# fakerlove1/HPFG

Hardware: AMD Instinct MI355X
Metric: labeled+unlabeled images/sec/node, U-Net 224x224 ACDC-shaped (Mean-Teacher step) (higher is better)
Workload: dtype bf16x3 (fp32 storage; products as split-bf16 MFMA hi*hi+hi*lo+lo*hi, fp32 accumulate); 1 GPU; mean_teacher_unet_224x224 (BASELINE configs[1]): U-Net 1ch->4cls, 8 labelled + 8 unlabelled per GPU, student fwd+bwd + train-mode teacher fwd + CE/Dice/MSE + SGD + EMA; size=224, hipgraph=True, sync_bn=False, parallelism=dp1, math=bf16x3

## Files before the change

hpfg_amd/_lib.py:

```python
from __future__ import annotations

import ctypes as C
import os
import threading

_HERE = os.path.dirname(os.path.abspath(__file__))
LIB_PATH = os.path.join(_HERE, "lib", "libhpfg_hip.so")

BN_MEAN, BN_RSTD, BN_SCALE, BN_SHIFT, BN_K1, BN_K2, BN_K3, BN_SPARE, BN_ROWS = range(9)
ACT_NONE, ACT_PLAIN, ACT_STRIDED, ACT_BNACT, ACT_BNACT_POOL, ACT_UP2X, ACT_DZ, ACT_SPLIT16, ACT_UPBWD = range(9)
OPT_CONV_THIN, OPT_FIRST_MFMA, OPT_FIRST_WGRAD, OPT_NARROW_DEEP = 0, 1, 2, 3
LOSS_NSUM = 32
LOSS_MAX_CLASSES = 16
ACC_MAX_SHARDS = 8
VERSION = 139
RESIZE_TAPS = 36
SURFACE_SEGS = 32
MATH_F32, MATH_BF16X3 = 0, 1


class HipLibraryError(RuntimeError):
    pass


class Act(C.Structure):
    _fields_ = [("z", C.c_void_p), ("bn", C.c_void_p), ("aux", C.c_void_p), ("mode", C.c_int32), ("C", C.c_int32),
                ("Hs", C.c_int32), ("Ws", C.c_int32), ("pstride", C.c_int32), ("aux_pstride", C.c_int32),
                ("bn_stride", C.c_int32), ("bn_coff", C.c_int32), ("sn", C.c_int32), ("sc", C.c_int32), ("sy", C.c_int32),
                ("sx", C.c_int32), ("drop_p", C.c_float), ("drop_seed", C.c_uint32), ("drop_mask", C.c_void_p), ("seed_dev", C.c_void_p),
                ("bn_acc", C.c_void_p), ("bn_gamma", C.c_void_p), ("bn_beta", C.c_void_p), ("bn_count", C.c_float), ("bn_eps", C.c_float),
                ("bn_shards", C.c_int32), ("reserved1", C.c_int32)]


class ConvArgs(C.Structure):
    _fields_ = [("a0", Act), ("a1", Act), ("wpk", C.c_void_p), ("bias", C.c_void_p), ("out", C.c_void_p),
                ("stat_partials", C.c_void_p), ("out_pstride", C.c_int32), ("Cout", C.c_int32), ("CoutPad", C.c_int32),
                ("N", C.c_int32), ("H", C.c_int32), ("W", C.c_int32), ("taps", C.c_int32), ("math", C.c_int32),
                ("bwd_stats", C.c_int32), ("bwd_of", Act), ("out2", C.c_void_p), ("out_split", C.c_int32), ("out2_pstride", C.c_int32),
                ("stat_acc", C.c_void_p), ("stat_shards", C.c_int32), ("reserved2", C.c_int32), ("stage_out", C.c_void_p), ("side_sums", C.c_void_p)]


class WgradArgs(C.Structure):
    _fields_ = [("a0", Act), ("a1", Act), ("g", Act), ("slab", C.c_void_p), ("dw_oihw", C.c_void_p), ("Cin", C.c_int32),
                ("CinPad", C.c_int32), ("Cout", C.c_int32), ("CoutPad", C.c_int32), ("N", C.c_int32), ("H", C.c_int32),
                ("W", C.c_int32), ("taps", C.c_int32), ("S", C.c_int32), ("math", C.c_int32), ("defer_reduce", C.c_int32)]


class PeerX(C.Structure):
    _fields_ = [("mbox", C.c_void_p * 8), ("epoch", C.c_void_p), ("err", C.c_void_p), ("world", C.c_int32), ("rank", C.c_int32),
                ("slot", C.c_int32), ("cap", C.c_int32), ("slot_bytes", C.c_int64)]


class PeerBuf(C.Structure):
    _fields_ = [("win", C.c_void_p * 8), ("epoch", C.c_void_p), ("err", C.c_void_p), ("world", C.c_int32), ("rank", C.c_int32),
                ("slice", C.c_int64), ("n", C.c_int64), ("stride", C.c_int64)]


class FusedBwdArgs(C.Structure):
    _fields_ = [("d", ConvArgs), ("xa0", Act), ("xa1", Act), ("slab", C.c_void_p), ("Cin", C.c_int32), ("CinPad", C.c_int32),
                ("Cout", C.c_int32), ("CoutPad", C.c_int32)]


class AugSample(C.Structure):
    _fields_ = [("img_off", C.c_int64), ("lab_off", C.c_int64), ("h", C.c_int32), ("w", C.c_int32), ("mode", C.c_int32), ("k", C.c_int32),
                ("axis", C.c_int32), ("tab_off", C.c_int32), ("m00", C.c_double), ("m01", C.c_double), ("m10", C.c_double),
                ("m11", C.c_double), ("off_y", C.c_double), ("off_x", C.c_double)]


class BnAccDesc(C.Structure):
    _fields_ = [("acc", C.c_void_p), ("gamma", C.c_void_p), ("beta", C.c_void_p), ("running_mean", C.c_void_p), ("running_var", C.c_void_p),
                ("bn", C.c_void_p), ("C", C.c_int32), ("count", C.c_float), ("shards", C.c_int32), ("reserved", C.c_int32)]


class BnAccBwdDesc(C.Structure):
    _fields_ = [("acc", C.c_void_p), ("gamma", C.c_void_p), ("bn", C.c_void_p), ("dgamma", C.c_void_p), ("dbeta", C.c_void_p),
                ("C", C.c_int32), ("count", C.c_float), ("shards", C.c_int32), ("reserved", C.c_int32)]


class SlabDesc(C.Structure):
    _fields_ = [("slab", C.c_void_p), ("dw_oihw", C.c_void_p), ("S", C.c_int32), ("taps", C.c_int32), ("Cin", C.c_int32),
                ("CinPad", C.c_int32), ("Cout", C.c_int32), ("CoutPad", C.c_int32)]


class PackDesc(C.Structure):
    _fields_ = [("w_oihw", C.c_void_p), ("b", C.c_void_p), ("wpk_fwd", C.c_void_p), ("wpk_dgrad", C.c_void_p),
                ("bias_pad", C.c_void_p), ("wpk16_fwd", C.c_void_p), ("wpk16_dgrad", C.c_void_p), ("Cout", C.c_int32), ("Cin", C.c_int32),
                ("CoutPad", C.c_int32), ("CinPad", C.c_int32), ("taps", C.c_int32), ("kc", C.c_int32)]


class LossArgs(C.Structure):
    _fields_ = [("logits", C.c_void_p), ("t_logits", C.c_void_p), ("labels0", C.c_void_p), ("labels1", C.c_void_p),
                ("coef", C.c_void_p), ("partials", C.c_void_p), ("sums", C.c_void_p), ("out", C.c_void_p),
                ("dlogits", C.c_void_p), ("N", C.c_int32), ("n_lab", C.c_int32), ("H", C.c_int32), ("W", C.c_int32),
                ("C", C.c_int32), ("world", C.c_int32), ("input_is_prob", C.c_int32), ("teacher_is_prob", C.c_int32),
                ("t_unlab_only", C.c_int32), ("reserved0", C.c_int32), ("cons_mask", C.c_void_p)]


class PredBlocks(C.Structure):
    _fields_ = [("p", C.c_void_p * 8), ("n_blocks", C.c_int32), ("per_block", C.c_int32)]


_i, _l, _f, _d, _p, _u32 = C.c_int, C.c_long, C.c_float, C.c_double, C.c_void_p, C.c_uint32

PROTOTYPES = {
    "hpfg_version": (_i, []),
    "hpfg_last_error": (C.c_char_p, []),
    "hpfg_set_option": (_i, [_i, _i]),
    "hpfg_conv3x3_first_fwd": (_i, [C.POINTER(Act), _p, _p, _p, _p, _i, _i, _i, _i, _i, _p]),
    "hpfg_conv_fwd": (_i, [C.POINTER(ConvArgs), _p]),
    "hpfg_conv_stat_blocks": (_i, [_i, _i, _i]),
    "hpfg_conv_stat_rows": (_i, [C.POINTER(ConvArgs)]),
    "hpfg_bn_fwd_finalize": (_i, [_p, _i, _p, _d, _p, _p, _p, _p, _f, _f, _p, _i, _p]),
    "hpfg_reduce_partials": (_i, [_p, _i, _i, _p, _p]),
    "hpfg_conv_kc": (_i, [_i, _i, _i]),
    "hpfg_wpk16_elems": (_l, [_i, _i, _i, _i]),
    "hpfg_pack_weights": (_i, [_p, C.POINTER(PackDesc), _i, _p]),
    "hpfg_pack_weights_bump": (_i, [_p, C.POINTER(PackDesc), _i, _p, _i, _p, _i, _p, _l, _p]),
    "hpfg_conv3x3_first_fwd_acc": (_i, [C.POINTER(Act), _p, _p, _p, _p, _p, _i, _i, _i, _i, _i, _i, _p]),
    "hpfg_bn_acc_finalize": (_i, [_p, C.POINTER(BnAccDesc), _i, _f, _f, _p]),
    "hpfg_bn_acc_bwd_finalize": (_i, [_p, C.POINTER(BnAccBwdDesc), _i, _p]),
    "hpfg_bn_bwd_reduce_acc": (_i, [C.POINTER(Act), _i, _i, _i, _p, _i, _p]),
    "hpfg_bn_bwd_reduce_pool_acc": (_i, [C.POINTER(Act), _p, _i, _i, _i, _i, _p, _i, _p]),
    "hpfg_act_materialize": (_i, [C.POINTER(Act), C.POINTER(Act), _i, _i, _i, _p, _p]),
    "hpfg_dropout_mask": (_i, [_p, _l, _f, _u32, _p, _p]),
    "hpfg_bn_eval_table": (_i, [_p, _p, _p, _p, _f, _p, _i, _p]),
    "hpfg_bn_bwd_reduce": (_i, [C.POINTER(Act), _i, _i, _i, _p, _p]),
    "hpfg_bn_bwd_reduce_pool": (_i, [C.POINTER(Act), _p, _i, _i, _i, _i, _p, _p]),
    "hpfg_bn_bwd_pool_blocks": (_i, [_i, _i, _i, _i]),
    "hpfg_bn_bwd_blocks": (_i, [_i, _i, _i, _i]),
    "hpfg_bn_bwd_finalize": (_i, [_p, _i, _p, _d, _p, _p, _p, _p, _i, _f, _p]),
    "hpfg_wgrad": (_i, [C.POINTER(WgradArgs), _p]),
    "hpfg_fused_bwd": (_i, [C.POINTER(FusedBwdArgs), _p]),
    "hpfg_fused_bwd_grid": (_i, [C.POINTER(FusedBwdArgs)]),
    "hpfg_peer_slot_bytes": (_l, [_i, _i]),
    "hpfg_peer_alloc": (_i, [C.c_size_t, C.POINTER(C.c_void_p)]),
    "hpfg_peer_free": (_i, [_p]),
    "hpfg_peer_handle": (_i, [_p, C.c_char_p]),
    "hpfg_peer_open": (_i, [C.c_char_p, C.POINTER(C.c_void_p)]),
    "hpfg_peer_close": (_i, [_p]),
    "hpfg_word_add": (_i, [_p, _i, _p]),
    "hpfg_peer_buf_slice": (_l, [_i, _l]),
    "hpfg_peer_buf_bytes": (_l, [_i, _l]),
    "hpfg_peer_allreduce_f32": (_i, [C.POINTER(PeerBuf), _p, _p]),
    "hpfg_bn_fwd_finalize_x": (_i, [_p, _i, C.POINTER(PeerX), _d, _p, _p, _p, _p, _f, _f, _p, _i, _p]),
    "hpfg_bn_bwd_finalize_x": (_i, [_p, _i, C.POINTER(PeerX), _d, _p, _p, _p, _p, _i, _f, _p]),
    "hpfg_seg_loss_partials_x": (_i, [C.POINTER(LossArgs), C.POINTER(PeerX), _p]),
    "hpfg_slab_reduce_multi": (_i, [_p, C.POINTER(SlabDesc), _i, _p]),
    "hpfg_wgrad_splits": (_i, [_i, _i, _i, _i, _i, _i]),
    "hpfg_wgrad_slab_floats": (_l, [_i, _i, _i, _i, _i, _i]),
    "hpfg_channel_sum": (_i, [_p, _i, _l, _i, _p, _p, _p]),
    "hpfg_channel_sum_partials": (_i, [_p, _i, _l, _i, _p, _p]),
    "hpfg_channel_sum_blocks": (_i, [_l, _i]),
    "hpfg_conv_first_rows": (_i, [_i, _i, _i]),
    "hpfg_confusion_counts": (_i, [_p, _p, _l, _i, _p, _p]),
    "hpfg_resize_cubic": (_i, [_p, _i, _i, _i, _p, _i, _i, _p, _p, _p, _l, _p]),
    "hpfg_resize_cubic_scratch_bytes": (_l, [_i, _i, _i, _i, _i]),
    "hpfg_surface_counts": (_i, [_p, _p, _i, _i, _i, _i, _i, _p, _p]),
    "hpfg_surface_distances": (_i, [_p, _p, _i, _i, _i, _i, _i, _p, _p, _l, _p]),
    "hpfg_surface_workspace_bytes": (_l, [_i, _l]),
    "hpfg_surface_sums": (_i, [_p, _l, _i, _p, _p, _p]),
    "hpfg_box_masks": (_i, [_p, _i, _i, _i, _i, _i, _p, _p]),
    "hpfg_augment_batch": (_i, [_p, _p, _p, _p, _i, _i, _i, _p, _p, _p]),
    "hpfg_timestamp": (_i, [_p, _p]),
    "hpfg_ln_fwd": (_i, [_p, _p, _p, _p, _p, _p, _l, _i, _p]),
    "hpfg_ln_bwd": (_i, [_p, _p, _p, _p, _p, _p, _p, _p, _p, _l, _i, _p]),
    "hpfg_ln_bwd_blocks": (_i, [_l]),
    "hpfg_attn_fwd": (_i, [_p, _p, _p, _i, _i, _i, _i, _f, _p]),
    "hpfg_attn_bwd": (_i, [_p, _p, _p, _p, _p, _p, _i, _i, _i, _i, _f, _p]),
    "hpfg_dwgelu_fwd": (_i, [_p, _p, _p, _p, _i, _i, _i, _i, _p]),
    "hpfg_dwgelu_bwd": (_i, [_p, _p, _p, _p, _p, _p, _p, _p, _p, _i, _i, _i, _i, _p]),
    "hpfg_dwgelu_bwd_blocks": (_i, [_i, _i, _i]),
    "hpfg_resize_bilinear_fwd": (_i, [_p, _p, _i, _i, _i, _i, _i, _i, _p]),
    "hpfg_resize_sum_fwd": (_i, [_p, C.POINTER(C.c_void_p), C.POINTER(C.c_int), C.POINTER(C.c_int), _i, _p, _i, _i, _i, _i, _p]),
    "hpfg_resize_bilinear_bwd": (_i, [_p, _p, _i, _i, _i, _i, _i, _i, _p]),
    "hpfg_residual_scale": (_i, [_p, _p, _p, _p, _i, _l, _p]),
    "hpfg_scale_rows": (_i, [_p, _p, _p, _i, _l, _p]),
    "hpfg_im2col_nhwc": (_i, [_p, _p, _i, _i, _i, _i, _i, _i, _p]),
    "hpfg_col2im_nhwc": (_i, [_p, _p, _i, _i, _i, _i, _i, _i, _p]),
    "hpfg_linear_wgrad": (_i, [_p, _p, _p, _p, _l, _i, _i, _p]),
    "hpfg_linear_wgrad_splits": (_i, [_l, _i, _i]),
    "hpfg_tok_col_stats": (_i, [_p, _l, _i, _p, _p, _p]),
    "hpfg_tok_stat_blocks": (_i, [_l]),
    "hpfg_bnrelu_apply": (_i, [_p, _p, _p, _p, _p, _p, _f, _l, _p, _l, _i, _p]),
    "hpfg_bnrelu_bwd": (_i, [_p, _p, _p, _p, _p, _p, _p, _f, _l, _p, _p, _p, _l, _i, _p]),
    "hpfg_noise_add": (_i, [_p, _p, _p, _l, _l, _f, _f, _f, _p]),
    "hpfg_uncertainty_mask": (_i, [C.POINTER(PredBlocks), _i, _i, _i, _i, _i, _p, _p, _p, _p]),
    "hpfg_mix_samples": (_i, [_p, _p, _p, _p, _i, _l, _p]),
    "hpfg_softmax_mix": (_i, [_p, _p, _p, _p, _i, _i, _i, _i, _p]),
    "hpfg_pool_scatter_add": (_i, [C.POINTER(Act), _p, _i, _p, _i, _i, _i, _i, _p]),
    "hpfg_upsample2x_bwd": (_i, [_p, _i, _p, _i, _i, _i, _i, _p]),
    "hpfg_upsample2x_bwd_sums": (_i, [_p, _i, _p, _i, _i, _i, _i, _p, _p]),
    "hpfg_upsample2x_bwd_blocks": (_i, [_i, _i, _i, _i]),
    "hpfg_loss_blocks": (_i, [_i, _i, _i]),
    "hpfg_loss_nsum": (_i, [_i]),
    "hpfg_seg_loss_partials": (_i, [C.POINTER(LossArgs), _p]),
    "hpfg_seg_loss_finalize": (_i, [C.POINTER(LossArgs), _p]),
    "hpfg_seg_loss_bwd": (_i, [C.POINTER(LossArgs), _p, _p]),
    "hpfg_argmax_labels": (_i, [_p, _i, _i, _i, _i, _p, _p, _p, _p]),
    "hpfg_cutmix_blend": (_i, [_p, _p, _p, _p, _l, _p]),
    "hpfg_sgd_step": (_i, [_p, _p, _p, _l, _p, _f, _f, _f, _p]),
    "hpfg_adamw_step": (_i, [_p, _p, _p, _p, _l, _p, _p, _f, _f, _f, _f, _f, _p]),
    "hpfg_ema_update": (_i, [_p, _p, _l, _p, _p]),
    "hpfg_sgd_ema_step": (_i, [_p, _p, _p, _l, _p, _f, _f, _f, _p, _l, _p, _p]),
    "hpfg_attn_mfma_fwd": (_i, [_p, _p, _p, _i, _i, _i, _i, _f, _p]),
    "hpfg_attn_mfma_bwd": (_i, [_p, _p, _p, _p, _p, _p, _i, _i, _i, _i, _f, _p]),
    "hpfg_attn_mfma_blocks": (_i, [_i]),
    "hpfg_attn_mfma_fwd_hd": (_i, [_p, _p, _p, _i, _i, _i, _i, _i, _f, _p]),
    "hpfg_attn_mfma_bwd_hd": (_i, [_p, _p, _p, _p, _p, _p, _i, _i, _i, _i, _i, _f, _p]),
    "hpfg_attn_mfma_scratch_floats": (_l, [_i, _i, _i, _i]),
    "hpfg_attn_keys_max": (_i, []),
    "hpfg_attn_keys_fwd": (_i, [_p, _p, _p, _p, _i, _i, _i, _i, _i, _f, _i, _p]),
    "hpfg_attn_keys_bwd": (_i, [_p, _p, _p, _p, _p, _p, _p, _p, _i, _i, _i, _i, _i, _f, _i, _p]),
    "hpfg_attn_keys_scratch_floats": (_l, [_i, _i, _i, _i, _i, _i]),
    "hpfg_attn_window_fwd": (_i, [_p, _p, _p, _i, _i, _i, _i, _i, _i, _i, _f, _i, _p]),
    "hpfg_attn_window_bwd": (_i, [_p, _p, _p, _p, _p, _p, _i, _i, _i, _i, _i, _i, _i, _f, _i, _p]),
    "hpfg_attn_window_scratch_floats": (_l, [_i, _i, _i, _i, _i, _i, _i]),
    "hpfg_gelu_fwd": (_i, [_p, _p, _l, _p]),
    "hpfg_gelu_bwd": (_i, [_p, _p, _p, _l, _p]),
    "hpfg_patch_merge_fwd": (_i, [_p, _p, _i, _i, _i, _i, _p]),
    "hpfg_patch_merge_bwd": (_i, [_p, _p, _i, _i, _i, _i, _p]),
    "hpfg_attn_fwd_hd": (_i, [_p, _p, _p, _i, _i, _i, _i, _i, _f, _p]),
    "hpfg_attn_bwd_hd": (_i, [_p, _p, _p, _p, _p, _p, _i, _i, _i, _i, _i, _f, _p]),
    "hpfg_gemm_f32": (_i, [_p, _l, _l, _p, _l, _l, _p, _l, _i, _i, _i, _p, _i, _i, _p]),
    "hpfg_gemm_f32_splitk": (_i, [_p, _l, _l, _p, _l, _l, _p, _l, _i, _i, _i, _p, _i, _i, _p, _p]),
    "hpfg_gemm_f32_splits": (_i, [_i, _i, _i]),
    "hpfg_gemm_bf16x3": (_i, [_p, _l, _l, _p, _l, _l, _p, _l, _i, _i, _i, _p, _i, _i, _p]),
    "hpfg_gemm_bf16x3_splits": (_i, [_i, _i, _i]),
    "hpfg_gemm_bf16x3_splitk": (_i, [_p, _l, _l, _p, _l, _l, _p, _l, _i, _i, _i, _p, _i, _i, _p, _p]),
    "hpfg_gemm_bf16x3_ok": (_i, [_p, _l, _l, _p, _l, _l, _i, _i, _i]),
    "hpfg_gemm_tn_bf16x3": (_i, [_p, _p, _p, _p, _l, _i, _i, _i, _p]),
    "hpfg_gemm_tn_splits": (_i, [_l, _i, _i]),
    "hpfg_col_sum2": (_i, [_p, _l, _i, _l, _p, _p, _p]),
    "hpfg_col_sum_splits": (_i, [_l]),
    "hpfg_col_sum": (_i, [_p, _l, _i, _l, _p, _p]),
    "hpfg_relu_bwd": (_i, [_p, _p, _l, _p]),
    "hpfg_neck_pool_fwd": (_i, [_p, _i, _i, _i, _i, _i, _i, _p, _p, _p]),
    "hpfg_neck_pool_bwd": (_i, [_p, _p, _i, _i, _i, _i, _i, _p, _p]),
    "hpfg_l2norm_fwd": (_i, [_p, _i, _i, _i, _i, _i, _p, _p, _p]),
    "hpfg_l2norm_bwd": (_i, [_p, _p, _p, _i, _i, _i, _i, _i, _p, _p, _p]),
    "hpfg_ntxent_rows": (_i, [_p, _i, _f, _p, _p, _p]),
}

_lock = threading.Lock()
_lib = None


def load() -> C.CDLL:
    global _lib
    if _lib is not None:
        return _lib
    with _lock:
        if _lib is not None:
            return _lib
        if not os.path.exists(LIB_PATH):
            raise HipLibraryError(
                f"{LIB_PATH} not found: build it with `python -c 'import __graft_entry__ as g; g.build()'` "
                f"or `make -C hpfg_amd/csrc`. There is no CPU fallback for the HIP path.")
        lib = C.CDLL(LIB_PATH)
        for name, (res, args) in PROTOTYPES.items():
            fn = getattr(lib, name)
            fn.restype = res
            fn.argtypes = args
        if lib.hpfg_version() != VERSION:
            raise HipLibraryError(f"libhpfg_hip.so version {lib.hpfg_version()} != binding version {VERSION}; rebuild")
        if os.environ.get("HPFG_FIRST_WGRAD", "1") == "0":
            lib.hpfg_set_option(OPT_FIRST_WGRAD, 0)
        if os.environ.get("HPFG_NARROW_DEEP") is not None:
            lib.hpfg_set_option(OPT_NARROW_DEEP, int(os.environ["HPFG_NARROW_DEEP"]))
        _lib = lib
    return _lib


def check(rc: int, what: str):
    if rc != 0:
        msg = load().hpfg_last_error().decode("utf-8", "replace")
        raise HipLibraryError(f"{what} failed (rc={rc}): {msg}")


def ptr(t):
    return None if t is None else t.data_ptr()


def none_act() -> Act:
    return Act()
```

hpfg_amd/csrc/conv.hip:

```cpp
#include "conv_kernel.h"
#include "conv_bf16_kernel.h"

namespace {

struct HpfgFirstConvArgs {
  HpfgAct x;
  const float* w_oihw;
  const float* bias;
  float* out;
  float* stat_partials;
  long long* stat_acc;
  int stat_shards;
};

inline bool tile_is_big(int H, int W) { return (H % 16 == 0) && (W % 16 == 0); }

__global__ __launch_bounds__(256) HPFG_NO_PK_F32 void conv_first_kernel(HpfgFirstConvArgs q, int N, int H, int W, int Cin, int tiles_x, int tiles_y) {
  constexpr int T = 16, TP = T + 2, CO = 16;
  const HpfgAct& x = q.x;
  const float* __restrict__ w = q.w_oihw;
  const float* __restrict__ bias = q.bias;
  float* __restrict__ out = q.out;
  float* __restrict__ stat = q.stat_partials;
  long long* __restrict__ sacc = q.stat_acc;
  __shared__ float tin[4][TP * TP];
  __shared__ __attribute__((aligned(16))) float wl[9 * 4 * CO];
  __shared__ float red[2][4][CO];
  const int tid = threadIdx.x, lane = tid & 63, wave = tid >> 6;
  const int ntiles = tiles_x * tiles_y, nwork = ntiles * N;
  for (int i = tid; i < 9 * Cin * CO; i += 256) {
    int co = i % CO, r = i / CO, ci = r % Cin, tap = r / Cin;
    wl[i] = w[(co * Cin + ci) * 9 + tap];
  }
  f32x4 bq[4], s1[4], s2[4];
#pragma unroll
  for (int q = 0; q < 4; ++q) {
    bq[q] = *reinterpret_cast<const f32x4*>(bias + 4 * q);
    s1[q] = f32x4{0.f, 0.f, 0.f, 0.f};
    s2[q] = s1[q];
  }
  const int ly = tid / T, lx = tid % T;
  for (int wk = blockIdx.x; wk < nwork; wk += gridDim.x) {
    const int n = wk / ntiles, tile = wk % ntiles;
    const int ty0 = (tile / tiles_x) * T, tx0 = (tile % tiles_x) * T;
    __syncthreads();
    for (int i = tid; i < Cin * TP * TP; i += 256) {
      int ci = i / (TP * TP), pix = i % (TP * TP);
      int gy = ty0 + pix / TP - 1, gx = tx0 + pix % TP - 1;
      float v = 0.f;
      if (gy >= 0 && gy < H && gx >= 0 && gx < W) v = x.z[(long)n * x.sn + (long)ci * x.sc + (long)gy * x.sy + (long)gx * x.sx];
      tin[ci][pix] = v;
    }
    __syncthreads();
    f32x4 acc[4] = {bq[0], bq[1], bq[2], bq[3]};
    for (int ci = 0; ci < Cin; ++ci)
#pragma unroll
      for (int tap = 0; tap < 9; ++tap) {
        const float a = tin[ci][(ly + tap / 3) * TP + lx + tap % 3];
        const f32x4* wr = reinterpret_cast<const f32x4*>(wl + (tap * Cin + ci) * CO);
#pragma unroll
        for (int q = 0; q < 4; ++q) acc[q] += a * wr[q];
      }
    const int gy = ty0 + ly, gx = tx0 + lx;
    if (gy < H && gx < W) {
      f32x4* o = reinterpret_cast<f32x4*>(out + ((long)(n * H + gy) * W + gx) * CO);
#pragma unroll
      for (int q = 0; q < 4; ++q) {
        o[q] = acc[q];
        s1[q] += acc[q];
        s2[q] += acc[q] * acc[q];
      }
    }
  }
  if (stat || sacc) {
#pragma unroll
    for (int q = 0; q < 4; ++q)
#pragma unroll
      for (int j = 0; j < 4; ++j) {
        float v = s1[q][j], v2 = s2[q][j];
#pragma unroll
        for (int o = 32; o >= 1; o >>= 1) {
          v += __shfl_xor(v, o);
          v2 += __shfl_xor(v2, o);
        }
        if (lane == 0) {
          red[0][wave][4 * q + j] = v;
          red[1][wave][4 * q + j] = v2;
        }
      }
    __syncthreads();
    if (tid < 2 * CO) {
      int which = tid / CO, co = tid % CO;
      float t = red[which][0][co] + red[which][1][co] + red[which][2][co] + red[which][3][co];
      if (sacc) hpfg_acc_add(sacc, CO, (int)blockIdx.x & (q.stat_shards - 1), which, co, t);
      if (stat) stat[((long)blockIdx.x * 2 + which) * CO + co] = t;
    }
  }
}

template <int CIN>
__global__ __launch_bounds__(256) void conv_first_mfma_kernel(HpfgFirstConvArgs q, int N, int H, int W, int tiles_x, int tiles_y) {
  constexpr int T = 16, TP = T + 2, CO = 16, NPIX = TP * TP, KT = 9 * CIN, KS = (KT + 3) / 4, NLD = (CIN * NPIX + 255) / 256;
  const HpfgAct& x = q.x;
  const float* __restrict__ w = q.w_oihw;
  float* __restrict__ out = q.out;
  float* __restrict__ stat = q.stat_partials;
  long long* __restrict__ sacc = q.stat_acc;
  __shared__ float tin[CIN * NPIX];
  __shared__ float red[2][4][CO];
  const int tid = threadIdx.x, lane = tid & 63, wave = tid >> 6;
  const int ntiles = tiles_x * tiles_y, nwork = ntiles * N;
  const int co_a = lane & 15, kq = lane >> 4;
  float wa[KS];
  int boff[KS];
#pragma unroll
  for (int s_ = 0; s_ < KS; ++s_) {
    const int k = 4 * s_ + kq, ci = k / 9, tap = k - 9 * ci;
    wa[s_] = k < KT ? w[co_a * KT + k] : 0.f;
    boff[s_] = k < KT ? ci * NPIX + (tap / 3) * TP + (lane & 15) + tap % 3 : 0;
  }
  const f32x4 b4 = *reinterpret_cast<const f32x4*>(q.bias + 4 * kq);
  f32x4 s1[4], s2[4];
#pragma unroll
  for (int r = 0; r < 4; ++r) {
    s1[r] = f32x4{0.f, 0.f, 0.f, 0.f};
    s2[r] = s1[r];
  }
  int pci[NLD], ppy[NLD], ppx[NLD];
#pragma unroll
  for (int i = 0; i < NLD; ++i) {
    const int e = tid + 256 * i, pix = e % NPIX;
    pci[i] = e / NPIX;
    ppy[i] = pix / TP - 1;
    ppx[i] = pix % TP - 1;
  }
  int n = 0, ty0 = 0, tx0 = 0;
  auto coords = [&](int wk) {
    n = wk / ntiles;
    const int tile = wk - n * ntiles, tyi = tile / tiles_x;
    ty0 = tyi * T;
    tx0 = (tile - tyi * tiles_x) * T;
  };
  auto fetch = [&](float (&v)[NLD]) {
    const float* xb = x.z + (long)n * x.sn;
#pragma unroll
    for (int i = 0; i < NLD; ++i) {
      const int gy = ty0 + ppy[i], gx = tx0 + ppx[i];
      v[i] = (tid + 256 * i < CIN * NPIX && gy >= 0 && gy < H && gx >= 0 && gx < W) ? xb[(long)pci[i] * x.sc + (long)gy * x.sy + (long)gx * x.sx] : 0.f;
    }
  };
  float v[NLD];
  int wk = blockIdx.x;
  if (wk < nwork) {
    coords(wk);
    fetch(v);
  }
#pragma unroll 1
  for (; wk < nwork; wk += gridDim.x) {
    const int cn = n, cy0 = ty0, cx0 = tx0;
    __syncthreads();
#pragma unroll
    for (int i = 0; i < NLD; ++i)
      if (tid + 256 * i < CIN * NPIX) tin[tid + 256 * i] = v[i];
    __syncthreads();
    if (wk + (int)gridDim.x < nwork) {
      coords(wk + gridDim.x);
      fetch(v);
    }
    const int gx = cx0 + (lane & 15);
    float* orow = out + ((long)(cn * H + cy0 + 4 * wave) * W + gx) * CO + 4 * kq;
#pragma unroll
    for (int r = 0; r < 4; ++r) {
      const int ly = 4 * wave + r;
      f32x4 acc = b4;
#pragma unroll
      for (int s_ = 0; s_ < KS; ++s_) {
        float bv = tin[ly * TP + boff[s_]];
        if (s_ == KS - 1 && 4 * s_ + kq >= KT) bv = 0.f;
        acc = __builtin_amdgcn_mfma_f32_16x16x4f32(wa[s_], bv, acc, 0, 0, 0);
      }
      if (cy0 + ly < H && gx < W) *reinterpret_cast<f32x4*>(orow + (long)r * W * CO) = acc;
      s1[r] += acc;
      s2[r] += acc * acc;
    }
  }
  if (stat || sacc) {
    const f32x4 t1 = (s1[0] + s1[2]) + (s1[1] + s1[3]), t2 = (s2[0] + s2[2]) + (s2[1] + s2[3]);
#pragma unroll
    for (int j = 0; j < 4; ++j) {
      float a1 = t1[j], a2 = t2[j];
#pragma unroll
      for (int o = 8; o >= 1; o >>= 1) {
        a1 += __shfl_xor(a1, o);
        a2 += __shfl_xor(a2, o);
      }
      if ((lane & 15) == 0) {
        red[0][wave][4 * kq + j] = a1;
        red[1][wave][4 * kq + j] = a2;
      }
    }
    __syncthreads();
    if (tid < 2 * CO) {
      const int which = tid / CO, co = tid % CO;
      const float t = red[which][0][co] + red[which][1][co] + red[which][2][co] + red[which][3][co];
      if (sacc) hpfg_acc_add(sacc, CO, (int)blockIdx.x & (q.stat_shards - 1), which, co, t);
      if (stat) stat[((long)blockIdx.x * 2 + which) * CO + co] = t;
    }
  }
}

inline int conv_first_grid(int N, int H, int W) {
  const long nwork = (long)N * ((H + 15) / 16) * ((W + 15) / 16);
  return (int)(nwork < 1024 ? nwork : 1024);
}

}

extern "C" int hpfg_conv_stat_blocks(int N, int H, int W) {
  if (tile_is_big(H, W)) return (N * (H / 16) * (W / 16) + 7) / 8 * 8;
  const int a = N * ((H + 7) / 8) * ((W + 7) / 8), b = N * ((H + 3) / 4) * ((W + 15) / 16);
  return a > b ? a : b;
}

extern "C" int hpfg_conv_first_rows(int N, int H, int W) { return conv_first_grid(N, H, W); }

static int conv_fwd_impl(const HpfgConvArgs* a, void* stream, int* rows_only);

extern "C" int hpfg_conv_fwd(const HpfgConvArgs* a, void* stream) { return conv_fwd_impl(a, stream, nullptr); }

extern "C" int hpfg_conv_stat_rows(const HpfgConvArgs* a) {
  int rows = -1;
  int rc = conv_fwd_impl(a, nullptr, &rows);
  return rc ? -1 : rows;
}

static int conv_fwd_impl(const HpfgConvArgs* a, void* stream, int* rows_only) {
  HPFG_ARG_CHECK(a && a->wpk && a->out, "conv_fwd: null pointer");
  HPFG_ARG_CHECK(a->taps == 9 || a->taps == 1, "conv_fwd: taps must be 1 or 9 (got %d)", a->taps);
  HPFG_ARG_CHECK(a->CoutPad % 16 == 0 && a->Cout <= a->CoutPad && a->Cout > 0, "conv_fwd: bad Cout %d / pad %d", a->Cout, a->CoutPad);
  HPFG_ARG_CHECK(a->N > 0 && a->H > 0 && a->W > 0 && a->N < 65536, "conv_fwd: bad N/H/W");
  HPFG_ARG_CHECK(a->a0.mode != HPFG_ACT_NONE && a->a0.C > 0, "conv_fwd: a0 empty");
  HPFG_ARG_CHECK(a->a1.mode == HPFG_ACT_NONE || a->a0.C % 16 == 0, "conv_fwd: concat needs a0.C %% 16 == 0");
  HPFG_ARG_CHECK(a->out_split ? (a->out_pstride >= a->out_split) : (a->out_pstride >= a->Cout), "conv_fwd: out_pstride too small");
  HPFG_ARG_CHECK(a->out_split == 0 || (a->out2 && a->out_split % 16 == 0 && a->out_split < a->Cout && a->out2_pstride >= a->Cout - a->out_split &&
                                       !a->bwd_stats),
                 "conv_fwd: out_split needs out2, a multiple of 16 below Cout, and no bwd_stats");
  HPFG_ARG_CHECK(!a->stat_acc || ((a->math & 0xff) == HPFG_MATH_BF16X3 && a->Cout == a->CoutPad && a->stat_shards >= 1 &&
                                  a->stat_shards <= HPFG_ACC_MAX_SHARDS && (a->stat_shards & (a->stat_shards - 1)) == 0),
                 "conv_fwd: stat_acc is a bf16x3 forward feature (Cout == CoutPad, stat_shards a power of two <= %d)", HPFG_ACC_MAX_SHARDS);
  for (const HpfgAct* s : {&a->a0, &a->a1}) {
    if (!s->bn_acc) continue;
    HPFG_ARG_CHECK((a->math & 0xff) == HPFG_MATH_BF16X3 && (s->mode == HPFG_ACT_BNACT || s->mode == HPFG_ACT_BNACT_POOL || s->mode == HPFG_ACT_DZ) &&
                       s->bn_gamma && (s->bn_beta || s->mode == HPFG_ACT_DZ) && s->bn_count >= 1.f && s->bn_count <= 16777216.f && s->C <= 256 && s->bn_shards >= 1 &&
                       s->bn_shards <= HPFG_ACC_MAX_SHARDS,
                   "conv_fwd: bn_acc needs a BNACT / BNACT_POOL / DZ source of the bf16x3 kernels with gamma (beta), a count of at most 2^24 (a float holds N*H*W exactly up to there) and at most 256 channels");
  }
  HPFG_ARG_CHECK((a->math & 0xff) != HPFG_MATH_BF16X3 || !(a->a0.mode == HPFG_ACT_BNACT || a->a0.mode == HPFG_ACT_BNACT_POOL || a->a0.mode == HPFG_ACT_DZ) ||
                     a->a0.C <= 256,
                 "conv_fwd(bf16x3): a BatchNorm'd source has at most 256 channels (got %d)", a->a0.C);
  const bool upb = a->a0.mode == HPFG_ACT_UPBWD;
  HPFG_ARG_CHECK(!upb || ((a->math & 0xff) == HPFG_MATH_BF16X3 && a->taps == 1 && a->a1.mode == HPFG_ACT_NONE && a->a0.C % 8 == 0 && a->a0.pstride % 4 == 0 &&
                          a->a0.Hs == a->H && a->a0.Ws == a->W && a->H <= 16383 && a->W <= 16383 && (long)a->N * 4 * a->H * a->W * a->a0.pstride < (1L << 31)),
                 "conv_fwd: an UPBWD source belongs to the 1x1 bf16x3 dgrad (channels a multiple of 8, pixel stride of 4, Hs x Ws == H x W)");
  HPFG_ARG_CHECK(!a->side_sums || upb, "conv_fwd: side_sums goes with an UPBWD source");
  HPFG_ARG_CHECK(!a->stage_out || upb || ((a->math & 0xff) == HPFG_MATH_BF16X3 && a->taps == 9 && hpfg_kind_of(a->a0, a->a1) > HPFG_KIND_PLAIN &&
                                    (a->a0.C + a->a1.C) % 8 == 0 && (a->H % 16 || a->W % 16)),
                 "conv_fwd: stage_out is a feature of the 3x3 bf16x3 kernels (non-PLAIN source, channels a multiple of 8, H or W not a multiple of 16)");
  hipStream_t st = (hipStream_t)stream;
  if (a->bwd_stats) {
    const int kind = hpfg_kind_of(a->a0, a->a1);
    HPFG_ARG_CHECK((a->math & 0xff) == HPFG_MATH_BF16X3 && (kind == HPFG_KIND_DZ || kind == HPFG_KIND_PLAIN || (kind == HPFG_KIND_UPB && a->bwd_stats == 1)),
                   "conv_fwd: bwd_stats is a dgrad feature of the bf16x3 kernels (DZ, PLAIN or UPBWD source)");
    HPFG_ARG_CHECK((a->stat_partials || a->stat_acc) && a->bwd_of.z && a->bwd_of.bn && !a->bias,
                   "conv_fwd: bwd_stats needs stat_partials or stat_acc, bwd_of.z / .bn and no bias");
    const int up = a->bwd_stats == 2 ? 2 : 1;
    HPFG_ARG_CHECK(a->bwd_stats == 1 || a->bwd_stats == 2, "conv_fwd: bwd_stats must be 0, 1 or 2");
    HPFG_ARG_CHECK(a->bwd_of.C == a->Cout && a->Cout == a->CoutPad && a->bwd_of.Hs == up * a->H && a->bwd_of.Ws == up * a->W && a->bwd_of.pstride % 4 == 0,
                   "conv_fwd: bwd_of must describe a layer with C == Cout == CoutPad (%d/%d/%d) at the output size (twice it for bwd_stats == 2)",
                   a->bwd_of.C, a->Cout, a->CoutPad);
    HPFG_ARG_CHECK(a->bwd_stats == 1 || (a->taps == 9 && (a->H % 16 || a->W % 16) && a->bwd_of.aux && a->bwd_of.aux_pstride % 4 == 0 && a->bwd_of.drop_p == 0.f && !a->out_split),
                   "conv_fwd: bwd_stats == 2 (max-pool backward in the epilogue) needs a 3x3 dgrad at a size that is not a multiple of 16, bwd_of.aux (the gradient so far) and no dropout behind bwd_of");
  }
  if ((a->math & 0xff) == HPFG_MATH_BF16X3) {
    {
      const int r = hpfg_conv_thin_try(*a, st, rows_only);
      if (r != HPFG_THIN_NONE) return r;
    }
    switch (hpfg_kind_of(a->a0, a->a1)) {
      case HPFG_KIND_PLAIN: return hpfg_conv16_launch_plain(*a, st, rows_only);
      case HPFG_KIND_BNACT: return hpfg_conv16_launch_bnact(*a, st, rows_only);
      case HPFG_KIND_POOL: return hpfg_conv16_launch_pool(*a, st, rows_only);
      case HPFG_KIND_CAT: return hpfg_conv16_launch_cat(*a, st, rows_only);
      case HPFG_KIND_DZ: return hpfg_conv16_launch_dz(*a, st, rows_only);
      case HPFG_KIND_UPB: return hpfg_conv16_launch_upb(*a, st, rows_only);
      default: break;
    }
    hpfg_set_error("conv_fwd(bf16x3): unsupported source combination (a0.mode=%d, a1.mode=%d)", a->a0.mode, a->a1.mode);
    return -1;
  }
  if (rows_only) {
    const int tl = tile_is_big(a->H, a->W) ? 16 : 8;
    *rows_only = a->N * ((a->H + tl - 1) / tl) * ((a->W + tl - 1) / tl);
    return 0;
  }
  switch (hpfg_kind_of(a->a0, a->a1)) {
    case HPFG_KIND_PLAIN: return hpfg_conv_launch_plain(*a, st);
    case HPFG_KIND_BNACT: return hpfg_conv_launch_bnact(*a, st);
    case HPFG_KIND_POOL: return hpfg_conv_launch_pool(*a, st);
    case HPFG_KIND_CAT: return hpfg_conv_launch_cat(*a, st);
    case HPFG_KIND_DZ: return hpfg_conv_launch_dz(*a, st);
    default: break;
  }
  hpfg_set_error("conv_fwd: unsupported source combination (a0.mode=%d, a1.mode=%d)", a->a0.mode, a->a1.mode);
  return -1;
}

static int conv_first_impl(const HpfgFirstConvArgs* q, int N, int H, int W, int Cin, int Cout, void* stream) {
  HPFG_ARG_CHECK(Cin >= 1 && Cin <= 4 && Cout == 16, "conv_first: needs Cin<=4, Cout==16 (got %d,%d)", Cin, Cout);
  HPFG_ARG_CHECK(q->x.z && q->w_oihw && q->bias && q->out, "conv_first: null pointer");
  HPFG_ARG_CHECK(q->x.mode == HPFG_ACT_STRIDED, "conv_first: input must be a STRIDED source");
  HPFG_ARG_CHECK((q->stat_partials == nullptr && q->stat_acc == nullptr) || tile_is_big(H, W), "conv_first: BN sums need H,W multiples of 16 (got %dx%d)", H, W);
  int tx = (W + 15) / 16, ty = (H + 15) / 16;
  const dim3 g1(conv_first_grid(N, H, W));
  if (q->stat_acc) HPFG_ACC_CHECK(g1.x, q->stat_shards, "conv_first");
  if ((Cin == 1 || Cin == 3) && hpfg_opt(HPFG_OPT_FIRST_MFMA) != 0) {
    if (Cin == 1) hipLaunchKernelGGL((conv_first_mfma_kernel<1>), g1, dim3(256), 0, (hipStream_t)stream, *q, N, H, W, tx, ty);
    else hipLaunchKernelGGL((conv_first_mfma_kernel<3>), g1, dim3(256), 0, (hipStream_t)stream, *q, N, H, W, tx, ty);
    return hpfg_launch_status("conv_first_mfma_kernel");
  }
  hipLaunchKernelGGL(conv_first_kernel, g1, dim3(256), 0, (hipStream_t)stream, *q, N, H, W, Cin, tx, ty);
  return hpfg_launch_status("conv_first_kernel");
}

extern "C" int hpfg_conv3x3_first_fwd(const HpfgAct* x, const float* w_oihw, const float* bias, float* out, float* stat_partials,
                                      int N, int H, int W, int Cin, int Cout, void* stream) {
  HPFG_ARG_CHECK(x, "conv_first: null pointer");
  HpfgFirstConvArgs a = {*x, w_oihw, bias, out, stat_partials, nullptr, 1};
  return conv_first_impl(&a, N, H, W, Cin, Cout, stream);
}

extern "C" int hpfg_conv3x3_first_fwd_acc(const HpfgAct* x, const float* w_oihw, const float* bias, float* out, float* stat_partials, long long* stat_acc,
                                          int stat_shards, int N, int H, int W, int Cin, int Cout, void* stream) {
  HPFG_ARG_CHECK(x && stat_acc, "conv_first_acc: null pointer");
  HPFG_ARG_CHECK(stat_shards >= 1 && stat_shards <= HPFG_ACC_MAX_SHARDS && (stat_shards & (stat_shards - 1)) == 0, "conv_first_acc: bad shard count %d", stat_shards);
  HpfgFirstConvArgs a = {*x, w_oihw, bias, out, stat_partials, stat_acc, stat_shards};
  return conv_first_impl(&a, N, H, W, Cin, Cout, stream);
}
```

hpfg_amd/csrc/misc.hip:

```cpp
#include <stdarg.h>
#include <string.h>
#include "stage.h"

static thread_local char g_err[512] = "";
extern "C" void hpfg_set_error(const char* fmt, ...) {
  va_list ap;
  va_start(ap, fmt);
  vsnprintf(g_err, sizeof(g_err), fmt, ap);
  va_end(ap);
}
extern "C" const char* hpfg_last_error(void) { return g_err; }
extern "C" int hpfg_version(void) { return HPFG_VERSION; }

static int g_opt[HPFG_OPT_COUNT] = {1, 1, 1, 128};
int hpfg_opt(int which) { return which >= 0 && which < HPFG_OPT_COUNT ? g_opt[which] : 0; }
extern "C" int hpfg_set_option(int which, int value) {
  HPFG_ARG_CHECK(which >= 0 && which < HPFG_OPT_COUNT, "set_option: unknown option %d", which);
  const int old = g_opt[which];
  g_opt[which] = value;
  return old;
}

namespace {

__global__ __launch_bounds__(256) void pack_weights_kernel(const HpfgPackDesc* __restrict__ table, long long* __restrict__ counters, int n_counters,
                                                           int* __restrict__ seed_word, int seed_add, long long* __restrict__ zero, long n_zero) {
  if (blockIdx.x == 0 && blockIdx.y == 0) {
    for (int i = threadIdx.x; i < n_counters; i += 256) counters[i] += 1;
    if (threadIdx.x == 0 && seed_word && seed_add) *seed_word = (*seed_word + seed_add) & 0x7FFFFFFF;
  }
  for (long i = ((long)blockIdx.y * gridDim.x + blockIdx.x) * 256 + threadIdx.x; i < n_zero; i += (long)gridDim.x * gridDim.y * 256) zero[i] = 0;
  const HpfgPackDesc d = table[blockIdx.y];
  const long total = (long)d.taps * d.CinPad * d.CoutPad;
  const int nt_f = d.CoutPad / 16, nch_f = d.CinPad / 16;
  const int nt_d = d.CinPad / 16, nch_d = d.CoutPad / 16;
  for (long i = blockIdx.x * 256L + threadIdx.x; i < total; i += (long)gridDim.x * 256) {
    int ks = (int)(i & 3), lane = (int)((i >> 2) & 63);
    long r = i >> 8;
    if (d.wpk_fwd) {
      int nt = (int)(r % nt_f), ch = (int)((r / nt_f) % nch_f), tap = (int)(r / ((long)nt_f * nch_f));
      int co = nt * 16 + (lane & 15), ci = ch * 16 + ks * 4 + (lane >> 4);
      d.wpk_fwd[i] = (co < d.Cout && ci < d.Cin) ? d.w_oihw[((long)co * d.Cin + ci) * d.taps + tap] : 0.f;
    }
    if (d.wpk_dgrad) {
      int nt = (int)(r % nt_d), ch = (int)((r / nt_d) % nch_d), tap = (int)(r / ((long)nt_d * nch_d));
      int co = ch * 16 + ks * 4 + (lane >> 4), ci = nt * 16 + (lane & 15);
      d.wpk_dgrad[i] = (co < d.Cout && ci < d.Cin) ? d.w_oihw[((long)co * d.Cin + ci) * d.taps + (d.taps - 1 - tap)] : 0.f;
    }
    if (i < d.CoutPad) d.bias_pad[i] = (i < d.Cout && d.b) ? d.b[i] : 0.f;
  }
  const int ksteps = d.taps == 1 ? 1 : (d.kc == 32 ? 9 : 5);
  for (int dir = 0; dir < 2; ++dir) {
    __bf16* out = reinterpret_cast<__bf16*>(dir == 0 ? d.wpk16_fwd : d.wpk16_dgrad);
    if (!out) continue;
    const int Kch = dir == 0 ? d.Cin : d.Cout;
    const int ntn = (dir == 0 ? d.CoutPad : d.CinPad) / 16;
    const int nchunks = (Kch + d.kc - 1) / d.kc;
    const long tot = (long)nchunks * ksteps * ntn * 512;
    for (long i = blockIdx.x * 256L + threadIdx.x; i < tot; i += (long)gridDim.x * 256) {
      const int j = (int)(i & 7), lane = (int)((i >> 3) & 63);
      const long r = i >> 9;
      const int nt = (int)(r % ntn), ks = (int)(r / ntn);
      const int chunk = ks / ksteps, s = ks % ksteps;
      const int kl = 8 * (lane >> 4) + j;
      int tap, kch;
      if (d.taps == 1) { tap = 0; kch = chunk * 32 + kl; }
      else if (d.kc == 32) { tap = s; kch = chunk * 32 + kl; }
      else { tap = 2 * s + (kl >> 4); kch = chunk * 16 + (kl & 15); }
      const int nch = nt * 16 + (lane & 15);
      float w = 0.f;
      if (tap < d.taps && kch < Kch) {
        if (dir == 0) { if (nch < d.Cout) w = d.w_oihw[((long)nch * d.Cin + kch) * d.taps + tap]; }
        else { if (nch < d.Cin) w = d.w_oihw[((long)kch * d.Cin + nch) * d.taps + (d.taps - 1 - tap)]; }
      }
      const __bf16 hi = (__bf16)w;
      const __bf16 lo = (__bf16)(w - (float)hi);
      const long base = ((long)ks * ntn + nt) * 2;
      out[(base + 0) * 512 + lane * 8 + j] = hi;
      out[(base + 1) * 512 + lane * 8 + j] = lo;
    }
  }
}

__global__ __launch_bounds__(256) void materialize_kernel(HpfgAct a0, HpfgAct a1, int N, int H, int W, float* __restrict__ out) {
  const int Ct = a0.C + a1.C, Q = (Ct + 3) / 4;
  const ActCtx c0 = make_ctx(a0), c1 = make_ctx(a1);
  const long total = (long)N * H * W * Q;
  for (long i = blockIdx.x * 256L + threadIdx.x; i < total; i += (long)gridDim.x * 256) {
    int q = (int)(i % Q);
    long pix = i / Q;
    int x = (int)(pix % W), y = (int)((pix / W) % H), n = (int)(pix / ((long)W * H));
    f32x4 v = cat_load4(a0, c0, a1, c1, n, y, x, q * 4);
#pragma unroll
    for (int j = 0; j < 4; ++j)
      if (q * 4 + j < Ct) out[pix * Ct + q * 4 + j] = v[j];
  }
}

__global__ __launch_bounds__(256) void dropout_mask_kernel(uint8_t* __restrict__ out, long n, uint32_t thresh, uint32_t seed0,
                                                           const uint32_t* __restrict__ seed_dev) {
  const uint32_t seed = seed0 + (seed_dev ? *seed_dev : 0u);
  for (long i = blockIdx.x * 256L + threadIdx.x; i < n; i += (long)gridDim.x * 256) out[i] = hpfg_keep((uint32_t)i, seed, thresh) ? 1 : 0;
}

__global__ __launch_bounds__(256) void pool_scatter_kernel(HpfgAct s, const float* __restrict__ dP, int dp_ps, float* __restrict__ dA, int da_ps,
                                                           int N, int Hp, int Wp) {
  const int Q = s.C / 4;
  const long total = (long)N * Hp * Wp * Q;
  for (long i = blockIdx.x * 256L + threadIdx.x; i < total; i += (long)gridDim.x * 256) {
    int q = (int)(i % Q);
    long pp = i / Q;
    int xp = (int)(pp % Wp), yp = (int)((pp / Wp) % Hp), n = (int)(pp / ((long)Wp * Hp));
    int c = q * 4;
    f32x4 sc = *reinterpret_cast<const f32x4*>(s.bn + HPFG_BN_SCALE * s.bn_stride + s.bn_coff + c);
    f32x4 sh = *reinterpret_cast<const f32x4*>(s.bn + HPFG_BN_SHIFT * s.bn_stride + s.bn_coff + c);
    long p00 = (long)(n * s.Hs + 2 * yp) * s.Ws + 2 * xp;
    long pos[4] = {p00, p00 + 1, p00 + s.Ws, p00 + s.Ws + 1};
    f32x4 zz[4];
#pragma unroll
    for (int k = 0; k < 4; ++k) zz[k] = *reinterpret_cast<const f32x4*>(s.z + pos[k] * s.pstride + c);
    f32x4 g = *reinterpret_cast<const f32x4*>(dP + pp * dp_ps + c);
    f32x4 da[4];
#pragma unroll
    for (int k = 0; k < 4; ++k) da[k] = *reinterpret_cast<const f32x4*>(dA + pos[k] * da_ps + c);
#pragma unroll
    for (int j = 0; j < 4; ++j) {
      float best = lrelu(zz[0][j] * sc[j] + sh[j]);
      int bi = 0;
#pragma unroll
      for (int k = 1; k < 4; ++k) {
        float v = lrelu(zz[k][j] * sc[j] + sh[j]);
        if (v > best) {
          best = v;
          bi = k;
        }
      }
#pragma unroll
      for (int k = 0; k < 4; ++k) da[k][j] += bi == k ? g[j] : 0.f;
    }
#pragma unroll
    for (int k = 0; k < 4; ++k) *reinterpret_cast<f32x4*>(dA + pos[k] * da_ps + c) = da[k];
  }
}

constexpr int UPB_MAXDIM = 512, UPB_TAPS = HPFG_UPB_TAPS;
__global__ __launch_bounds__(256) __attribute__((amdgpu_waves_per_eu(2, 3))) void upsample_bwd_kernel(const float* __restrict__ dUp, int dup_ps, float* __restrict__ dU, int N, int Hl, int Wl,
                                                           int C, float* __restrict__ csum, int xcd_aware) {
  __shared__ short t_idx[UPB_MAXDIM][UPB_TAPS];
  __shared__ float t_w[UPB_MAXDIM][UPB_TAPS];
  __shared__ float red[256 * 4];
  for (int e = threadIdx.x; e < Hl + Wl; e += 256) {
    int idx[8], cnt;
    float wgt[8];
    if (e < Hl) hpfg_up_taps(e, Hl, idx, wgt, cnt);
    else hpfg_up_taps(e - Hl, Wl, idx, wgt, cnt);
    if (cnt > UPB_TAPS) cnt = UPB_TAPS;
    for (int k = 0; k < UPB_TAPS; ++k) {
      t_idx[e][k] = (short)(k < cnt ? idx[k] : idx[cnt - 1]);
      t_w[e][k] = k < cnt ? wgt[k] : 0.f;
    }
  }
  __syncthreads();
  const int Q = C / 4, Ho = 2 * Hl, Wo = 2 * Wl;
  const long total = (long)N * Hl * Wl * Q;
  f32x4 csum4 = {0.f, 0.f, 0.f, 0.f};
  const int nxcd = (xcd_aware && gridDim.x % 8 == 0) ? 8 : 1;
  const long gx = gridDim.x / nxcd, xj = blockIdx.x / nxcd;
  const long span = ((total + nxcd - 1) / nxcd + 255) / 256 * 256;
// ... 464 lines not shown
```

hpfg_amd/engine.py:

```python
from __future__ import annotations

import ctypes as C
import itertools
import os
from dataclasses import dataclass
from typing import Dict, List, Optional

import torch

from . import _lib as L

SEED_BUMP = -1

WIDTHS = (16, 32, 64, 128, 256)
ENC_DROPOUT = (0.05, 0.1, 0.2, 0.3, 0.5)
BN_EPS, BN_MOMENTUM = 1e-5, 0.1


ACC, LOCAL, ALLREDUCE, PEER, EVAL = "acc", "local", "allreduce", "peer", "eval"


def bn_route(train: bool, math: int, bn_acc_on: bool, peer: bool, world: int, force_sync: bool) -> str:
    if not train:
        return EVAL
    sync = world > 1 or force_sync
    if bn_acc_on and math == L.MATH_BF16X3 and not peer and not sync:
        return ACC
    if sync:
        return PEER if peer else ALLREDUCE
    return LOCAL


def _pad16(c: int) -> int:
    return (c + 15) // 16 * 16


def _carve(flat: torch.Tensor, sizes: Dict[str, int]) -> Dict[str, torch.Tensor]:
    ends = list(itertools.accumulate(sizes.values()))
    return {name: flat[e - n:e] for (name, n), e in zip(sizes.items(), ends)}


class DescTable:

    def __init__(self, descs: C.Array, dev: torch.device):
        self.host = descs
        self.dev = torch.frombuffer(bytearray(bytes(descs)), dtype=torch.uint8).to(dev)
        self._base, self._size = self.dev.data_ptr(), C.sizeof(descs._type_)

    def sub(self, lo: int, hi: int):
        return self._base + lo * self._size, (self.host._type_ * (hi - lo)).from_buffer(self.host, lo * self._size), hi - lo


@dataclass
class ConvSpec:
    name: str
    bn: Optional[str]
    cin: int
    cout: int
    taps: int
    h: int
    w: int
    drop_p: float = 0.0
    idx: int = 0
    cin_pad: int = 0
    cout_pad: int = 0

    def __post_init__(self):
        self.cin_pad, self.cout_pad = _pad16(self.cin), _pad16(self.cout)


def enc_prefix(lvl: int) -> str:
    return "encoder.in_conv.conv_conv" if lvl == 0 else f"encoder.down{lvl}.maxpool_conv.1.conv_conv"


def build_specs(in_ch: int, ncls: int, H: int, W: int) -> Dict[str, ConvSpec]:
    specs: Dict[str, ConvSpec] = {}

    def add(s: ConvSpec):
        s.idx = len(specs)
        specs[s.name] = s

    cprev = in_ch
    for lvl, c in enumerate(WIDTHS):
        p, h, w = enc_prefix(lvl), H >> lvl, W >> lvl
        add(ConvSpec(f"{p}.0", f"{p}.1", cprev, c, 9, h, w, ENC_DROPOUT[lvl]))
        add(ConvSpec(f"{p}.4", f"{p}.5", c, c, 9, h, w))
        cprev = c
    for k in range(1, 5):
        c1, c2 = WIDTHS[5 - k], WIDTHS[4 - k]
        hl, wl = H >> (5 - k), W >> (5 - k)
        add(ConvSpec(f"decoder.up{k}.conv1x1", None, c1, c2, 1, hl, wl))
        p = f"decoder.up{k}.conv.conv_conv"
        add(ConvSpec(f"{p}.0", f"{p}.1", 2 * c2, c2, 9, 2 * hl, 2 * wl))
        add(ConvSpec(f"{p}.4", f"{p}.5", c2, c2, 9, 2 * hl, 2 * wl))
    add(ConvSpec("decoder.out_conv", None, WIDTHS[0], ncls, 9, H, W))
    return specs


class MarkLog:

    def __init__(self, dev: torch.device, capacity: int = 2048):
        self.buf = torch.zeros(capacity, dtype=torch.int64, device=dev)
        self.spans: List[tuple] = []
        self.n = 0
        self.lib = L.load()

    def stamp(self, stream: int) -> int:
        k = self.n
        if k >= self.buf.numel():
            raise RuntimeError("MarkLog: out of slots")
        self.n += 1
        L.check(self.lib.hpfg_timestamp(self.buf.data_ptr() + 8 * k, stream), "timestamp")
        return k

    def bracket(self, tag: str, stream: int, launch):
        a = self.stamp(stream)
        launch()
        self.spans.append((tag, a, self.stamp(stream)))

    def calib(self, stream: int):
        a = self.stamp(stream)
        self.spans.append(("calib", a, self.stamp(stream)))

    def read_us(self) -> List[tuple]:
        t = self.buf[: self.n].cpu().numpy()
        return [(tag, float(int(t[b]) - int(t[a])) / 100.0) for tag, a, b in self.spans]


class UNetEngine:

    def __init__(self, params: Dict[str, torch.Tensor], buffers: Dict[str, torch.Tensor], grads: Dict[str, torch.Tensor],
                 in_ch: int, ncls: int, N: int, H: int, W: int, device: torch.device):
        assert H % 16 == 0 and W % 16 == 0, "U-Net input must be a multiple of 16 (4 poolings)"
        self.lib = L.load()
        self.dev = device
        self.N, self.H, self.W, self.in_ch, self.ncls = N, H, W, in_ch, ncls
        self.params, self.buffers, self.grads = params, buffers, grads
        self.specs = build_specs(in_ch, ncls, H, W)
        self.order = list(self.specs.values())
        f32 = dict(dtype=torch.float32, device=device)
        self.z: Dict[str, torch.Tensor] = {s.name: torch.empty(N, s.h, s.w, s.cout, **f32) for s in self.order if s.name != "decoder.out_conv"}
        self.bn: Dict[str, torch.Tensor] = {s.name: torch.zeros(L.BN_ROWS, s.cout, **f32) for s in self.order if s.bn}
        nb = max(self.lib.hpfg_conv_stat_blocks(N, s.h, s.w) * 2 * s.cout_pad for s in self.order if s.bn)
        nb = max(nb, max(self.lib.hpfg_bn_bwd_blocks(N, s.h, s.w, s.cout) * 2 * s.cout for s in self.order if s.bn))
        nb = max(nb, max(self.lib.hpfg_bn_bwd_pool_blocks(N, s.h // 2, s.w // 2, s.cout) * 2 * s.cout for s in self.order if s.bn))
        self.partials = torch.empty(nb, **f32)
        self.sums = torch.empty(2 * 256, dtype=torch.float64, device=device)
        self.packed = [s for s in self.order if s.idx > 0]
        self.wpk_f = {s.name: torch.empty(s.taps * s.cin_pad * s.cout_pad, **f32) for s in self.packed}
        self.wpk_d = {s.name: torch.empty(s.taps * s.cin_pad * s.cout_pad, **f32) for s in self.packed}
        self.bias_pad = {s.name: torch.empty(s.cout_pad, **f32) for s in self.packed}
        self.kc = {s.name: self.lib.hpfg_conv_kc(s.h, s.w, s.taps) for s in self.packed}
        self.wpk16_f = {s.name: torch.empty(self.lib.hpfg_wpk16_elems(s.cin, s.cout_pad, s.taps, self.kc[s.name]), dtype=torch.bfloat16, device=device)
                        for s in self.packed}
        self.wpk16_d = {s.name: torch.empty(self.lib.hpfg_wpk16_elems(s.cout, s.cin_pad, s.taps, self.kc[s.name]), dtype=torch.bfloat16, device=device)
                        for s in self.packed}
        self._pack_tables: Dict[tuple, DescTable] = {}
        self.bn_layers = [s for s in self.order if s.bn]
        self._bn_idx = {s.name: i for i, s in enumerate(self.bn_layers)}
        self._n_enc_bn = sum(1 for s in self.bn_layers if s.name.startswith("encoder."))
        self.bn_acc_on = os.environ.get("HPFG_BN_ACC", "1") != "0"
        self.acc_shards = {s.name: L.ACC_MAX_SHARDS for s in self.bn_layers}
        assert all(s.cout == s.cout_pad for s in self.bn_layers)
        acc_words = {s.name: self.acc_shards[s.name] * 4 * s.cout for s in self.bn_layers}
        self.acc_all = torch.zeros(sum(acc_words.values()), dtype=torch.int64, device=device)
        self.acc_of = _carve(self.acc_all, acc_words)
        self.fwd_route, self._acc_dirty = EVAL, False
        self._acc_tables: Dict[bool, DescTable] = {}
        self.pack_overlap = False
        self.after_layer = None
        self.accb_all = torch.zeros_like(self.acc_all)
        self.accb_of = _carve(self.accb_all, acc_words)
        self.bwd_route, self._accb_dirty = LOCAL, False
        self._accb_table: Optional[DescTable] = None
        self.seed_dev = torch.zeros(1, dtype=torch.int32, device=device)
        self.bump_counters: Optional[torch.Tensor] = None
        self.base_seed = 0x1234567
        self.dropout_on = False
        self._stage_inputs = False
        self.bwd_ready = False
        self.x: Optional[torch.Tensor] = None
        self.world = 1
        self.gtmp, self.direct = None, False
        self._bwd_alloc_key: Optional[tuple] = None
        self.dA, self.dA_ps = {}, {}
        self.dcat, self.dup, self.dU, self.dP = {}, {}, {}, {}
        self.slab_of, self.csum_part, self.csum_rows = {}, {}, {}
        self.slabs: Optional[DescTable] = None
        self.bias_layers = [s for s in self.order if not s.bn]
        self._n_enc_desc = sum(1 for s in self.order if s.name.startswith("encoder."))
        self._n_thin_enc_desc = sum(1 for s in self.order if s.name.startswith("encoder.in_conv") or s.name.startswith("encoder.down1"))
        self.fuse_bwd_stats = 1
        self._fused_rows: Dict[str, int] = {}
        self.fused_bwd = os.environ.get("HPFG_FUSED_BWD", "1") == "1"
        self.pool_fuse = True
        self._pool_done: set = set()
        self.dz_side = True
        self.act_side = True
        self.upb_fuse = os.environ.get("HPFG_UPB_FUSE", "1") == "1"
        self.upb_max_c1 = int(os.environ.get("HPFG_UPB_MAX_C1", "128"))
        self.dzbuf: Dict[str, torch.Tensor] = {}
        self.actbuf: Dict[str, torch.Tensor] = {}
        self._act_live: set = set()
        self.defer_wgrad = False
        self._deferred: Optional[list] = None
        self._csum_pending: Optional[torch.Tensor] = None
        self.fused_grid: Dict[str, int] = {}
        self._side, self._side_used = None, False
        self.force_sync = False
        self.math = L.MATH_F32
        self.ext_masks: Dict[str, torch.Tensor] = {}
        self.allreduce = None
        self.peer, self.peer_base, self.xepoch = None, 0, None
        self.marks: Optional[MarkLog] = None

    def _stream(self):
        return torch.cuda.current_stream(self.dev).cuda_stream

    def _call(self, fn, *args, tag: Optional[str] = None, stream: Optional[int] = None):
        st = self._stream() if stream is None else stream

        def launch():
            L.check(fn(*args, st), f"{fn.__name__}[{tag}]" if tag else fn.__name__)
        if tag is None or self.marks is None:
            return launch()
        self.marks.bracket(tag, st, launch)

    @property
    def _b16(self) -> bool:
        return self.math == L.MATH_BF16X3

    def _fork_side(self) -> torch.cuda.Stream:
        if self._side is None:
            self._side = torch.cuda.Stream(device=self.dev)
        self._side.wait_stream(torch.cuda.current_stream(self.dev))
        return self._side

    def _join_side(self):
        if self._side_used:
            torch.cuda.current_stream(self.dev).wait_stream(self._side)
            self._side_used = False

    def layer_seed(self, s: ConvSpec) -> int:
        return (self.base_seed * 0x9E3779B1 + 0x85EBCA6B * (s.idx + 1)) & 0xFFFFFFFF

    def _act_bn(self, name: str, mode=L.ACT_BNACT) -> L.Act:
        s = self.specs[name]
        a = L.Act()
        a.z, a.bn, a.mode, a.C = L.ptr(self.z[name]), L.ptr(self.bn[name]), mode, s.cout
        a.Hs, a.Ws, a.pstride, a.bn_stride, a.bn_coff = s.h, s.w, s.cout, s.cout, 0
        if self.fwd_route == ACC and mode in (L.ACT_BNACT, L.ACT_BNACT_POOL):
            a.bn_acc, a.bn_gamma, a.bn_beta = L.ptr(self.acc_of[name]), L.ptr(self.params[f"{s.bn}.weight"]), L.ptr(self.params[f"{s.bn}.bias"])
            a.bn_count, a.bn_eps, a.bn_shards = float(self.N * s.h * s.w), BN_EPS, self.acc_shards[name]
        if mode == L.ACT_BNACT:
            self._act_dropout(a, s)
        return a

    def _act_dropout(self, a: L.Act, s: ConvSpec):
        if s.drop_p > 0 and self.dropout_on:
            a.drop_p, a.drop_seed, a.seed_dev = s.drop_p, self.layer_seed(s), L.ptr(self.seed_dev)
            a.drop_mask = L.ptr(self.ext_masks.get(s.name)) if self.ext_masks else None

    def _act_plain(self, t: torch.Tensor, C_: int, h: int, w: int, pstride: Optional[int] = None, mode=L.ACT_PLAIN) -> L.Act:
        a = L.Act()
        a.z, a.mode, a.C, a.Hs, a.Ws = L.ptr(t), mode, C_, h, w
        a.pstride = C_ if pstride is None else pstride
        if C_ % 4 != 0 and mode == L.ACT_PLAIN:
            a.mode = L.ACT_STRIDED
            a.sn, a.sc, a.sy, a.sx = h * w * a.pstride, 1, w * a.pstride, a.pstride
        return a

    def _act_split(self, t: torch.Tensor, C_: int, h: int, w: int) -> L.Act:
        return self._act_plain(t, C_, h, w, mode=L.ACT_SPLIT16)

    def _act_input(self, x: torch.Tensor) -> L.Act:
        a = L.Act()
        a.z, a.mode, a.C, a.Hs, a.Ws = L.ptr(x), L.ACT_STRIDED, self.in_ch, self.H, self.W
        a.sn, a.sc, a.sy, a.sx = x.stride(0), x.stride(1), x.stride(2), x.stride(3)
        return a

    def _act_dz(self, name: str, dA: torch.Tensor, da_pstride: int) -> L.Act:
        s = self.specs[name]
        a = L.Act()
        a.z, a.bn, a.aux, a.mode, a.C = L.ptr(self.z[name]), L.ptr(self.bn[name]), L.ptr(dA), L.ACT_DZ, s.cout
        a.Hs, a.Ws, a.pstride, a.aux_pstride, a.bn_stride = s.h, s.w, s.cout, da_pstride, s.cout
        if self.bwd_route == ACC:
            a.bn_acc, a.bn_gamma, a.bn_count, a.bn_shards = L.ptr(self.accb_of[name]), L.ptr(self.params[f"{s.bn}.weight"]), float(self.N * s.h * s.w), self.acc_shards[name]
        self._act_dropout(a, s)
        return a

    def input_acts(self, name: str):
        s = self.specs[name]
        none = L.Act()
        if name == "encoder.in_conv.conv_conv.0":
            return self._act_input(self.x), none
        if name == "decoder.out_conv":
            return self._act_bn("decoder.up4.conv.conv_conv.4"), none
        if name.endswith(".4"):
            return self._act_bn(name[:-2] + ".0"), none
        if name.startswith("encoder.down"):
            lvl = int(name[len("encoder.down")])
            return self._act_bn(enc_prefix(lvl - 1) + ".4", L.ACT_BNACT_POOL), none
        k = int(name[len("decoder.up")])
        prev = enc_prefix(4) + ".4" if k == 1 else f"decoder.up{k - 1}.conv.conv_conv.4"
        if name.endswith("conv1x1"):
            return self._act_bn(prev), none
        skip = self._act_bn(enc_prefix(4 - k) + ".4")
        u = self.specs[f"decoder.up{k}.conv1x1"]
        up = self._act_plain(self.z[u.name], u.cout, u.h, u.w, mode=L.ACT_UP2X)
        return skip, up

    def _pack_table(self, math: int, with_dgrad: bool):
        key = (math, with_dgrad)
        if key not in self._pack_tables:
            b16 = math == L.MATH_BF16X3
            descs = (L.PackDesc * len(self.packed))()
            for d, s in zip(descs, self.packed):
                d.w_oihw, d.b = L.ptr(self.params[f"{s.name}.weight"]), L.ptr(self.params[f"{s.name}.bias"])
                d.bias_pad = L.ptr(self.bias_pad[s.name])
                d.wpk_fwd = None if b16 else L.ptr(self.wpk_f[s.name])
                d.wpk_dgrad = None if (b16 or not with_dgrad) else L.ptr(self.wpk_d[s.name])
                d.wpk16_fwd = L.ptr(self.wpk16_f[s.name]) if b16 else None
                d.wpk16_dgrad = L.ptr(self.wpk16_d[s.name]) if (b16 and with_dgrad) else None
                d.kc = self.kc[s.name]
                d.Cout, d.Cin, d.CoutPad, d.CinPad, d.taps = s.cout, s.cin, s.cout_pad, s.cin_pad, s.taps
            self._pack_tables[key] = DescTable(descs, self.dev)
        return self._pack_tables[key]

    def pack(self, with_dgrad: bool = True, counters: Optional[torch.Tensor] = None, seed_add: int = 0):
        dev, host, n = self._pack_table(self.math, with_dgrad).sub(0, len(self.packed))
        if counters is not None:
            assert counters.dtype == torch.int64 and counters.is_contiguous() and counters.device == self.dev
        self._call(self.lib.hpfg_pack_weights_bump, dev, host, n, L.ptr(counters), counters.numel() if counters is not None else 0, L.ptr(self.seed_dev), int(seed_add),
                   None, 0, tag="pack_weights")

    def _finalize_bwd_all(self, lo: int, hi: int):
        if self.bwd_route != ACC or hi <= lo:
            return
        if self._accb_table is None:
            descs = (L.BnAccBwdDesc * len(self.bn_layers))()
            for d, s in zip(descs, self.bn_layers):
                d.acc, d.gamma, d.bn = L.ptr(self.accb_of[s.name]), L.ptr(self.params[f"{s.bn}.weight"]), L.ptr(self.bn[s.name])
                d.dgamma, d.dbeta = L.ptr(self.grads[f"{s.bn}.weight"]), L.ptr(self.grads[f"{s.bn}.bias"])
                d.C, d.count, d.shards = s.cout, float(self.N * s.h * s.w), self.acc_shards[s.name]
            self._accb_table = DescTable(descs, self.dev)
        dev, host, n = self._accb_table.sub(lo, hi)
        self._call(self.lib.hpfg_bn_acc_bwd_finalize, dev, host, n, tag="bn_bfin_all")

    def _finalize_all(self, track: bool):
        if track not in self._acc_tables:
            descs = (L.BnAccDesc * len(self.bn_layers))()
            for d, s in zip(descs, self.bn_layers):
                d.acc, d.gamma, d.beta = L.ptr(self.acc_of[s.name]), L.ptr(self.params[f"{s.bn}.weight"]), L.ptr(self.params[f"{s.bn}.bias"])
                d.running_mean = L.ptr(self.buffers[f"{s.bn}.running_mean"]) if track else None
                d.running_var = L.ptr(self.buffers[f"{s.bn}.running_var"]) if track else None
                d.bn, d.C, d.count, d.shards = L.ptr(self.bn[s.name]), s.cout, float(self.N * s.h * s.w), self.acc_shards[s.name]
            self._acc_tables[track] = DescTable(descs, self.dev)
        dev, host, n = self._acc_tables[track].sub(0, len(self.bn_layers))
        self._call(self.lib.hpfg_bn_acc_finalize, dev, host, n, BN_MOMENTUM, BN_EPS, tag="bn_fin_all")

    def _finalize_bn(self, s: ConvSpec, nblk: int, track: bool):
        rm, rv = (L.ptr(self.buffers[f"{s.bn}.running_{k}"]) if track else None for k in ("mean", "var"))
        tail = (float(self.N * s.h * s.w * self.world), L.ptr(self.params[f"{s.bn}.weight"]), L.ptr(self.params[f"{s.bn}.bias"]), rm, rv,
                BN_MOMENTUM, BN_EPS, L.ptr(self.bn[s.name]), s.cout)
        if self.fwd_route == PEER:
            px = self.peer.peer_desc(self.peer_base + 2 * self._bn_idx[s.name], self.xepoch)
            self._call(self.lib.hpfg_bn_fwd_finalize_x, L.ptr(self.partials), nblk, C.byref(px), *tail, tag="bn_fin:" + s.name)
        elif self.fwd_route == ALLREDUCE:
            sums = self.sums[: 2 * s.cout_pad]
            self._call(self.lib.hpfg_reduce_partials, L.ptr(self.partials), nblk, s.cout_pad, L.ptr(sums))
            self.allreduce(sums)
            self._call(self.lib.hpfg_bn_fwd_finalize, None, 0, L.ptr(sums), *tail)
        else:
            self._call(self.lib.hpfg_bn_fwd_finalize, L.ptr(self.partials), nblk, None, *tail, tag="bn_fin:" + s.name)

    def forward(self, x: torch.Tensor, train: bool = True, dropout: Optional[bool] = None, track_running: bool = True,
                seed_step: Optional[int] = None, needs_grad: bool = True) -> torch.Tensor:
        pack_args = self._fwd_begin(x, train, dropout, seed_step, needs_grad)
        logits = torch.empty(self.N, self.H, self.W, self.ncls, dtype=torch.float32, device=self.dev)
        for i, s in enumerate(self.order):
            if i == 0 and pack_args is not None:
                main = torch.cuda.current_stream(self.dev)
                with torch.cuda.stream(self._fork_side()):
                    self.pack(**pack_args)
                self._fwd_layer(s, logits, track_running)
                main.wait_stream(self._side)
                continue
            self._fwd_layer(s, logits, track_running)
            if self.after_layer is not None and i == self.after_layer[0]:
                self.after_layer[1]()
        if self.fwd_route == ACC:
            self._finalize_all(track_running)
            self._acc_dirty = False
        self.bwd_ready = bool(train and needs_grad)
        return logits

    def _fwd_begin(self, x: torch.Tensor, train: bool, dropout: Optional[bool], seed_step: Optional[int], needs_grad: bool) -> Optional[dict]:
        assert x.is_cuda and x.dtype == torch.float32 and tuple(x.shape) == (self.N, self.in_ch, self.H, self.W), (x.shape, x.dtype, x.device)
        self.x = x
        self._act_live = set()
        self._stage_inputs = bool(train and needs_grad and self.act_side and self._b16)
        self.dropout_on = train if dropout is None else dropout
        if seed_step is not None and seed_step != SEED_BUMP:
            self.seed_dev.fill_(int(seed_step) & 0x7FFFFFFF)
        counters, self.bump_counters = self.bump_counters, None
        self.fwd_route = bn_route(train, self.math, self.bn_acc_on, self.peer is not None, self.world, self.force_sync)
        if self.fwd_route == ACC:
            if self._acc_dirty:
                self.acc_all.zero_()
            self._acc_dirty = True
        pack_args = dict(with_dgrad=bool(train and needs_grad), counters=counters, seed_add=1 if seed_step == SEED_BUMP else 0)
        if not (self.pack_overlap and train):
            self.pack(**pack_args)
            pack_args = None
        if self.marks is not None:
            self.marks.calib(self._stream())
        if self.fwd_route == PEER:
            self.peer.bump(self.xepoch, self._stream())
        return pack_args

    def _fwd_layer(self, s: ConvSpec, logits: torch.Tensor, track_running: bool):
        out = logits if s.name == "decoder.out_conv" else self.z[s.name]
        want_stats = bool(s.bn) and self.fwd_route != EVAL
        acc = want_stats and self.fwd_route == ACC
        if s.idx == 0:
            a0, _ = self.input_acts(s.name)
            w, b = L.ptr(self.params[f"{s.name}.weight"]), L.ptr(self.params[f"{s.name}.bias"])
            if acc:
                self._call(self.lib.hpfg_conv3x3_first_fwd_acc, C.byref(a0), w, b, L.ptr(out), None, L.ptr(self.acc_of[s.name]), self.acc_shards[s.name],
                           self.N, s.h, s.w, s.cin, s.cout, tag="fwd:" + s.name)
            else:
                self._call(self.lib.hpfg_conv3x3_first_fwd, C.byref(a0), w, b, L.ptr(out), L.ptr(self.partials) if want_stats else None,
                           self.N, s.h, s.w, s.cin, s.cout, tag="fwd:" + s.name)
            nblk = self.lib.hpfg_conv_first_rows(self.N, s.h, s.w)
        else:
            ca = L.ConvArgs()
            ca.a0, ca.a1 = self.input_acts(s.name)
            ca.math = self.math
            ca.wpk = L.ptr(self.wpk16_f[s.name]) if self._b16 else L.ptr(self.wpk_f[s.name])
            ca.bias, ca.out = L.ptr(self.bias_pad[s.name]), L.ptr(out)
            ca.out_pstride, ca.Cout, ca.CoutPad = s.cout, s.cout, s.cout_pad
            ca.N, ca.H, ca.W, ca.taps = self.N, s.h, s.w, s.taps
            if acc:
                ca.stat_acc, ca.stat_shards = L.ptr(self.acc_of[s.name]), self.acc_shards[s.name]
            elif want_stats:
                ca.stat_partials = L.ptr(self.partials)
            if self._stage_inputs and self._side_layer(s) and s.cin % 8 == 0 and ca.a0.mode != L.ACT_PLAIN:
                ca.stage_out = L.ptr(self._side_buf(self.actbuf, s, s.cin))
                self._act_live.add(s.name)
            self._call(self.lib.hpfg_conv_fwd, C.byref(ca), tag="fwd:" + s.name)
            if want_stats and not acc:
                nblk = self.lib.hpfg_conv_stat_rows(C.byref(ca))
        if s.bn:
            if self.fwd_route == EVAL:
                self._call(self.lib.hpfg_bn_eval_table, L.ptr(self.params[f"{s.bn}.weight"]), L.ptr(self.params[f"{s.bn}.bias"]), L.ptr(self.buffers[f"{s.bn}.running_mean"]),
                           L.ptr(self.buffers[f"{s.bn}.running_var"]), BN_EPS, L.ptr(self.bn[s.name]), s.cout)
            elif self.fwd_route != ACC:
                self._finalize_bn(s, nblk, track_running)

    def materialize(self, name: str, mode=L.ACT_BNACT) -> torch.Tensor:
        s = self.specs[name]
        a = self._act_bn(name, mode)
        h, w = (s.h // 2, s.w // 2) if mode == L.ACT_BNACT_POOL else (s.h, s.w)
        out = torch.empty(self.N, h, w, s.cout, dtype=torch.float32, device=self.dev)
        self._call(self.lib.hpfg_act_materialize, C.byref(a), None, self.N, h, w, L.ptr(out))
        return out

    def materialize_input(self, name: str) -> torch.Tensor:
        s = self.specs[name]
        a0, a1 = self.input_acts(name)
        out = torch.empty(self.N, s.h, s.w, s.cin, dtype=torch.float32, device=self.dev)
        self._call(self.lib.hpfg_act_materialize, C.byref(a0), C.byref(a1), self.N, s.h, s.w, L.ptr(out))
        return out

    def _alloc_bwd(self):
        key = (self.math, self.fused_bwd, self.upb_fuse)
        if self._bwd_alloc_key == key:
            return
        self._bwd_alloc_key = key
        f32 = dict(dtype=torch.float32, device=self.dev)
        N, sp = self.N, self.specs
        self.dA, self.dA_ps, self.dcat, self.dup = {}, {}, {}, {}
        for k in range(1, 5):
            s = sp[f"decoder.up{k}.conv.conv_conv.0"]
            skip = enc_prefix(4 - k) + ".4"
            cw = s.cin // 2 if s.cin // 2 * 4 < 128 else s.cin
            self.dcat[k] = torch.empty(N, s.h, s.w, cw, **f32)
            if cw < s.cin:
                self.dup[k] = torch.empty(N, s.h, s.w, cw, **f32)
            self.dA[skip], self.dA_ps[skip] = self.dcat[k], cw
        for s in self.order:
            if s.bn and s.name not in self.dA:
                self.dA[s.name] = torch.empty(N, s.h, s.w, s.cout, **f32)
                self.dA_ps[s.name] = s.cout
        self.dU = {k: torch.empty(N, s.h, s.w, s.cout, **f32) for k, s in ((k, sp[f"decoder.up{k}.conv1x1"]) for k in range(1, 5))}
        self.dP = {lvl: torch.empty(N, s.h, s.w, s.cin, **f32) for lvl, s in ((lvl, sp[enc_prefix(lvl) + ".0"]) for lvl in range(1, 5))}
        sizes = {s.name: self.lib.hpfg_wgrad_slab_floats(N, s.h, s.w, s.cin_pad, s.cout_pad, s.taps) for s in self.order}
        self.fused_grid = {}
        if self.fused_bwd and self._b16:
            for s in self.order:
                if s.taps != 9:
                    continue
                fa = L.FusedBwdArgs()
                fa.xa0, fa.xa1 = self.input_acts(s.name)
                fa.d.a0.mode = L.ACT_DZ if s.bn else L.ACT_PLAIN
                fa.d.out = None if s.idx == 0 else L.ptr(self.partials)
                fa.d.N, fa.d.H, fa.d.W, fa.d.taps, fa.d.math = N, s.h, s.w, 9, self.math
                fa.Cin, fa.CinPad, fa.Cout, fa.CoutPad = s.cin, s.cin_pad, s.cout, s.cout_pad
                grid = self.lib.hpfg_fused_bwd_grid(C.byref(fa))
                if grid > 0:
                    self.fused_grid[s.name] = grid
                    sizes[s.name] = max(sizes[s.name], grid * 9 * s.cin_pad * s.cout_pad)
        self.slab_all = torch.empty(sum(sizes.values()), **f32)
        self.slab_of = _carve(self.slab_all, sizes)
        self.csum_rows = {s.name: ((self._upb_rows(s) if self._upb_on(s) else self.lib.hpfg_upsample2x_bwd_blocks(N, s.h, s.w, s.cout)) if s.taps == 1
                                   else self.lib.hpfg_channel_sum_blocks(N * s.h * s.w, s.cout)) for s in self.bias_layers}
        self.csum_part = {s.name: torch.empty(self.csum_rows[s.name] * s.cout, **f32) for s in self.bias_layers}
        descs = (L.SlabDesc * (len(self.order) + len(self.bias_layers)))()
        for d, s in zip(descs, self.order):
            d.slab, d.dw_oihw = L.ptr(self.slab_of[s.name]), L.ptr(self.grads[f"{s.name}.weight"])
            d.S = self.fused_grid.get(s.name) or self.lib.hpfg_wgrad_splits(N, s.h, s.w, s.cin_pad, s.cout_pad, s.taps)
            d.taps, d.Cin, d.CinPad, d.Cout, d.CoutPad = s.taps, s.cin, s.cin_pad, s.cout, s.cout_pad
        for j, s in enumerate(self.bias_layers):
            d = descs[len(self.order) + j]
            d.slab, d.dw_oihw = L.ptr(self.csum_part[s.name]), L.ptr(self.grads[f"{s.name}.bias"])
            d.S = self.csum_rows[s.name]
            d.taps, d.Cin, d.CinPad, d.Cout, d.CoutPad = 1, 1, 1, s.cout, s.cout
        self.slabs = DescTable(descs, self.dev)

    def _bn_backward(self, s: ConvSpec, pooled_grad: Optional[torch.Tensor] = None):
        g = self._act_dz(s.name, self.dA[s.name], self.dA_ps[s.name])
        nblk = self._fused_rows.pop(s.name, None)
        if nblk is not None:
            assert pooled_grad is None
        elif self.bwd_route == ACC:
            acc, sh = L.ptr(self.accb_of[s.name]), self.acc_shards[s.name]
            if pooled_grad is not None:
                self._call(self.lib.hpfg_bn_bwd_reduce_pool_acc, C.byref(g), L.ptr(pooled_grad), s.cout, self.N, s.h // 2, s.w // 2, acc, sh, tag="bn_red:" + s.name)
            else:
                self._call(self.lib.hpfg_bn_bwd_reduce_acc, C.byref(g), self.N, s.h, s.w, acc, sh, tag="bn_red:" + s.name)
        elif pooled_grad is not None:
            nblk = self.lib.hpfg_bn_bwd_pool_blocks(self.N, s.h // 2, s.w // 2, s.cout)
            self._call(self.lib.hpfg_bn_bwd_reduce_pool, C.byref(g), L.ptr(pooled_grad), s.cout, self.N, s.h // 2, s.w // 2, L.ptr(self.partials), tag="bn_red:" + s.name)
        else:
            nblk = self.lib.hpfg_bn_bwd_blocks(self.N, s.h, s.w, s.cout)
            self._call(self.lib.hpfg_bn_bwd_reduce, C.byref(g), self.N, s.h, s.w, L.ptr(self.partials), tag="bn_red:" + s.name)
        if self.bwd_route == ACC:
            return g
        tail = (float(self.N * s.h * s.w * self.world), L.ptr(self.params[f"{s.bn}.weight"]), L.ptr(self.bn[s.name]), L.ptr(self.grads[f"{s.bn}.weight"]),
                L.ptr(self.grads[f"{s.bn}.bias"]), s.cout)
        if self.bwd_route == PEER:
            px = self.peer.peer_desc(self.peer_base + 2 * self._bn_idx[s.name] + 1, self.xepoch)
            self._call(self.lib.hpfg_bn_bwd_finalize_x, L.ptr(self.partials), nblk, C.byref(px), *tail, 1.0 / self.world, tag="bn_bfin:" + s.name)
        elif self.bwd_route == ALLREDUCE:
            sums = self.sums[: 2 * s.cout]
            self._call(self.lib.hpfg_reduce_partials, L.ptr(self.partials), nblk, s.cout, L.ptr(sums))
            self.allreduce(sums)
            self._call(self.lib.hpfg_bn_bwd_finalize, None, 0, L.ptr(sums), *tail, 1.0 / self.world)
        else:
            self._call(self.lib.hpfg_bn_bwd_finalize, L.ptr(self.partials), nblk, None, *tail, 1.0, tag="bn_bfin:" + s.name)
        return g

    def _wgrad_dgrad(self, s: ConvSpec, g: L.Act, dgrad_out: torch.Tensor, stats_for: Optional[str] = None, out2: Optional[torch.Tensor] = None,
                     pool_of: Optional[str] = None):
        if s.name in self.fused_grid:
            return self._fused_bwd(s, g, dgrad_out, stats_for, out2)
        dz, gw = None, g
        if self.dz_side and self._b16 and self._side_layer(s) and g.mode == L.ACT_DZ and s.cout % 8 == 0:
            dz = self._side_buf(self.dzbuf, s, s.cout)
            gw = self._act_split(dz, s.cout, s.h, s.w)
        if self._deferred is None and dz is None:
            self._wgrad(s, g)
        self._dgrad(s, g, dgrad_out, stats_for, out2, stage_out=dz, pool_of=pool_of)
        if self._deferred is not None:
            self._deferred.append((s, gw))
        elif dz is not None:
            self._wgrad(s, gw)

    def _upb_on(self, su: ConvSpec) -> bool:
        return bool(self.upb_fuse and self._b16 and su.taps == 1 and su.cout % 8 == 0 and su.cin <= self.upb_max_c1)

# ... 198 lines not shown
```

hpfg_amd/model/unet.py:

```python
from __future__ import annotations

from collections import OrderedDict
from typing import Dict, List, Optional, Tuple

import torch
import torch.nn as nn

import os

from .. import _lib as L
from .. import engine as E
from .. import heads

WIDTHS = E.WIDTHS

_INSTANCES = [0]


def reset_dropout_streams(count: int = 0) -> None:
    _INSTANCES[0] = int(count)


def _fresh_dropout_seed() -> int:
    _INSTANCES[0] += 1
    h = (0x1234567 + _INSTANCES[0] * 0x9E3779B1 + (torch.initial_seed() & 0xFFFFFFFF) * 0x85EBCA6B) & 0xFFFFFFFF
    h ^= h >> 15
    h = (h * 0x85EBCA6B) & 0xFFFFFFFF
    h ^= h >> 13
    return h & 0x7FFFFFFF


def _block(cin: int, cout: int) -> nn.Module:
    m = nn.Module()
    m.conv_conv = nn.ModuleDict(OrderedDict([
        ("0", nn.Conv2d(cin, cout, 3, padding=1)), ("1", nn.BatchNorm2d(cout)),
        ("4", nn.Conv2d(cout, cout, 3, padding=1)), ("5", nn.BatchNorm2d(cout))]))
    return m


def _down(cin: int, cout: int) -> nn.Module:
    m = nn.Module()
    m.maxpool_conv = nn.ModuleDict(OrderedDict([("1", _block(cin, cout))]))
    return m


def _up(c1: int, c2: int) -> nn.Module:
    m = nn.Module()
    m.conv1x1 = nn.Conv2d(c1, c2, 1)
    m.conv = _block(2 * c2, c2)
    return m


def _neck(cin: int, hid: int, out: int = 128) -> nn.Module:
    m = nn.Module()
    m.mlp = nn.ModuleDict(OrderedDict([("0", nn.Linear(cin, hid)), ("2", nn.Linear(hid, out))]))
    m.mlp_conv = nn.ModuleDict(OrderedDict([("0", nn.Conv2d(cin, hid, 1)), ("2", nn.Conv2d(hid, out, 1))]))
    return m


class _UNetFn(torch.autograd.Function):

    @staticmethod
    def forward(ctx, anchor: torch.Tensor, x: torch.Tensor, net: "UNet", want_feat: bool, needs_grad: bool):
        eng = net._acquire_engine(x)
        if getattr(net, "_bn_bump_pending", False):
            eng.bump_counters, net._bn_bump_pending = net._flat_long, False
        logits = eng.forward(x, train=net.training, track_running=True, seed_step=net._next_seed() if net.training else None, needs_grad=needs_grad)
        ctx.net, ctx.eng, ctx.want_feat = net, eng, want_feat
        out = logits.permute(0, 3, 1, 2)
        if want_feat:
            feat = eng.materialize(E.enc_prefix(4) + ".4").permute(0, 3, 1, 2)
            return out, feat
        return out, logits.new_empty(0)

    @staticmethod
    def backward(ctx, dlogits, dfeat):
        net, eng = ctx.net, ctx.eng
        dl = dlogits.permute(0, 2, 3, 1)
        if not dl.is_contiguous():
            dl = dl.contiguous()
        df = None
        if ctx.want_feat and dfeat is not None:
            df = dfeat.permute(0, 2, 3, 1).contiguous()
        dp = net.dp
        cb = None
        nested = getattr(dp, "p2p_grads", False) and not getattr(net, "_alone", False)
        if dp is not None and dp.active and getattr(dp, "overlap", False) and eng.direct and not nested:
            cb = lambda i: dp.launch_bucket(net.grad_bucket(i))
            net._buckets_launched = True
        eng.backward(dl, df, cb)
        net._accumulate_grads(eng)
        return None, None, None, None, None


class UNet(nn.Module):
    def __init__(self, in_channels: int = 1, num_classes: int = 4):
        super().__init__()
        self.in_channels, self.num_classes = in_channels, num_classes
        enc = nn.Module()
        enc.in_conv = _block(in_channels, WIDTHS[0])
        for k in range(1, 5):
            setattr(enc, f"down{k}", _down(WIDTHS[k - 1], WIDTHS[k]))
        dec = nn.Module()
        for k in range(1, 5):
            setattr(dec, f"up{k}", _up(WIDTHS[5 - k], WIDTHS[4 - k]))
        dec.out_conv = nn.Conv2d(WIDTHS[0], num_classes, 3, padding=1)
        self.encoder, self.decoder = enc, dec
        self._init_runtime()

    def _init_runtime(self):
        self._flat: Optional[torch.Tensor] = None
        self._flat_grad: Optional[torch.Tensor] = None
        self._flat_buf: Optional[torch.Tensor] = None
        self._flat_long: Optional[torch.Tensor] = None
        self._engines: Dict[Tuple, List[E.UNetEngine]] = {}
        self._anchor: Optional[torch.Tensor] = None
        self._seed_counter = 0
        self.dropout_seed = _fresh_dropout_seed()
        self.dp = None
        self.math = os.environ.get("HPFG_MATH", "bf16x3")
        self.external_dropout_masks = None
        self._flatten()

    def _float_buffers(self):
        return [(n, b) for n, b in self.named_buffers() if b.is_floating_point()]

    def _flatten(self):
        ps = list(self.named_parameters())
        if not ps:
            return
        dev = ps[0][1].device
        with torch.no_grad():
            flat = torch.cat([p.detach().reshape(-1).float() for _, p in ps]).to(dev)
            flat_grad = torch.zeros_like(flat)
            off = 0
            self._offsets: Dict[str, Tuple[int, int]] = {}
            for n, p in ps:
                k = p.numel()
                p.data = flat[off:off + k].view(p.shape)
                p.grad = None
                self._offsets[n] = (off, k)
                off += k
            bs = self._float_buffers()
            fb = torch.cat([b.detach().reshape(-1).float() for _, b in bs]).to(dev)
            off = 0
            for n, b in bs:
                k = b.numel()
                b.data = fb[off:off + k].view(b.shape)
                off += k
            ls = [(n, b) for n, b in self.named_buffers() if b.dtype == torch.long]
            fl = torch.stack([b.detach().reshape(()) for _, b in ls]).to(dev) if ls else torch.zeros(0, dtype=torch.long, device=dev)
            for i, (n, b) in enumerate(ls):
                b.data = fl[i]
        self._flat, self._flat_grad, self._flat_buf, self._flat_long = flat, flat_grad, fb, fl
        self._engines = {}
        self._anchor = torch.zeros(1, device=dev, requires_grad=True)
        self._backbone_numel = sum(p.numel() for n, p in ps if n.startswith("encoder.") or n.startswith("decoder."))
        self._encoder_numel = sum(p.numel() for n, p in ps if n.startswith("encoder."))

    def _is_flat(self) -> bool:
        ps = list(self.parameters())
        if self._flat is None or not ps:
            return False
        first, last = ps[0], ps[-1]
        return (first.data_ptr() == self._flat.data_ptr() and
                last.data_ptr() == self._flat.data_ptr() + (self._flat.numel() - last.numel()) * 4)

    def _ensure_flat(self):
        if not self._is_flat():
            self._flatten()

    def _apply(self, fn, *a, **k):
        out = super()._apply(fn, *a, **k)
        self._flatten()
        return out

    def __deepcopy__(self, memo):
        cls = self.__class__
        new = cls.__new__(cls)
        nn.Module.__init__(new)
        import copy
        for k, v in self.__dict__.items():
            if k in ("_flat", "_flat_grad", "_flat_buf", "_flat_long", "_engines", "_anchor", "dp"):
                continue
            new.__dict__[k] = copy.deepcopy(v, memo)
        new.dp = self.dp
        new.dropout_seed = _fresh_dropout_seed()
        new._flat = new._flat_grad = new._flat_buf = new._flat_long = None
        new._engines, new._anchor = {}, None
        new._flatten()
        return new

    def load_state_dict(self, *a, **k):
        out = super().load_state_dict(*a, **k)
        self._ensure_flat()
        return out

    @property
    def flat_params(self) -> torch.Tensor:
        self._ensure_flat()
        return self._flat

    @property
    def flat_grads(self) -> torch.Tensor:
        self._ensure_flat()
        return self._flat_grad

    def grad_bucket(self, i: int) -> torch.Tensor:
        return self._flat_grad[self._encoder_numel:] if i == 0 else self._flat_grad[:self._encoder_numel]

    def backbone_numel(self) -> int:
        return self._backbone_numel

    def attach_grad_views(self):
        for n, p in self.named_parameters():
            if p.requires_grad:
                off, k = self._offsets[n]
                g = self._flat_grad[off:off + k].view(p.shape)
                if p.grad is None or p.grad.data_ptr() != g.data_ptr():
                    p.grad = g

    def zero_flat_grad(self):
        if getattr(self, "direct_grads", False):
            return
        self._flat_grad.zero_()

    def _next_seed(self):
        if getattr(self, "_graph_seed_mode", False):
            self._graph_fwds = getattr(self, "_graph_fwds", 0) + 1
            return E.SEED_BUMP
        self._seed_counter += 1
        return self._seed_counter

    def bump_graph_seed(self):
        self._seed_counter += getattr(self, "_fwds_per_replay", 0)

    def _acquire_engine(self, x: torch.Tensor) -> E.UNetEngine:
        if not x.is_cuda:
            raise RuntimeError("hpfg_amd.UNet runs on the HIP library only: move the input to the GPU (no CPU fallback)")
        self._ensure_flat()
        if x.device != self._flat.device:
            raise RuntimeError(f"input on {x.device} but parameters on {self._flat.device}")
        key = (tuple(x.shape), x.device.index)
        pool = self._engines.setdefault(key, [])
        direct = bool(getattr(self, "direct_grads", False))
        eng = next((e for e in pool if not e.bwd_ready and e.direct == direct), None)
        if eng is None and len(pool) >= 4:
            eng = next((e for e in pool if e.direct == direct), None)
        if eng is None:
            named = dict(self.named_parameters())
            params = {n: p.data for n, p in named.items()}
            bufs = {n: b.data for n, b in self.named_buffers()}
            gtmp = self._flat_grad if direct else torch.zeros_like(self._flat)
            grads = {n: gtmp[o:o + k].view(named[n].shape) for n, (o, k) in self._offsets.items()}
            eng = E.UNetEngine(params, bufs, grads, self.in_channels, self.num_classes, x.shape[0], x.shape[2], x.shape[3], x.device)
            eng.gtmp = gtmp
            eng.direct = direct
            pool.append(eng)
        rank = self.dp.rank if self.dp is not None else 0
        eng.base_seed = (self.dropout_seed + 0x632BE5AB * rank) & 0x7FFFFFFF
        eng.math = L.MATH_BF16X3 if self.math == "bf16x3" else L.MATH_F32
        eng.defer_wgrad = bool(getattr(self, "defer_wgrad", False))
        eng.pack_overlap = bool(getattr(self, "_alone", False))
        eng.after_layer = getattr(self, "_after_layer", None)
        ext = self.external_dropout_masks
        if isinstance(ext, (list, tuple)):
            k = getattr(self, "_ext_mask_idx", 0)
            self._ext_mask_idx = k + 1
            ext = ext[k % len(ext)] if len(ext) else None
        eng.ext_masks = ext or {}
        if self.dp is not None and getattr(self.dp, "sync_bn", True):
            eng.world, eng.allreduce = self.dp.world_size, self.dp.allreduce_sum
            eng.force_sync = bool(getattr(self.dp, "force_sync", False))
            if getattr(self.dp, "p2p", False) and eng.peer is None:
                eng.peer, eng.peer_base = self.dp, self.dp.alloc_slots(2 * 18)
                eng.xepoch = torch.zeros(1, dtype=torch.int32, device=x.device)
        return eng

    def _accumulate_grads(self, eng: E.UNetEngine):
        if eng.direct:
            self.attach_grad_views()
            return
        n = self._backbone_numel
        first = next(iter(self.parameters()))
        if first.grad is None:
            self._flat_grad[:n].copy_(eng.gtmp[:n])
        else:
            self._flat_grad[:n].add_(eng.gtmp[:n])
        self.attach_grad_views()

    def _prepare_head_grads(self):
        n = self._backbone_numel
        heads_ = [p for nme, p in self.named_parameters() if not (nme.startswith("encoder.") or nme.startswith("decoder."))]
        if heads_ and heads_[0].requires_grad and (heads_[0].grad is None or heads_[0].grad.data_ptr() != self._flat_grad.data_ptr() + 4 * n):
            self._flat_grad[n:].zero_()
            for nme, p in self.named_parameters():
                if not (nme.startswith("encoder.") or nme.startswith("decoder.")):
                    off, k = self._offsets[nme]
                    p.grad = self._flat_grad[off:off + k].view(p.shape)

    def _bump_bn_counters(self):
        self._bn_bump_pending = True

    def _run(self, x: torch.Tensor, want_feat: bool):
        self._ensure_flat()
        if self.training:
            self._bump_bn_counters()
        trainable = next(iter(self.parameters())).requires_grad
        anchor = self._anchor if trainable else self._anchor.detach()
        return _UNetFn.apply(anchor, x.float(), self, want_feat, bool(trainable and torch.is_grad_enabled()))

    def forward(self, x: torch.Tensor) -> torch.Tensor:
        return self._run(x, False)[0]


class UNet_Plus(UNet):
    def __init__(self, in_channels: int = 1, num_classes: int = 4):
        nn.Module.__init__(self)
        self.in_channels, self.num_classes = in_channels, num_classes
        tmp = UNet.__new__(UNet)
        UNet.__init__(tmp, in_channels, num_classes)
        self.encoder, self.decoder = tmp.encoder, tmp.decoder
        self.dense_projection_high = _neck(WIDTHS[-1], 2048)
        self.dense_projection_head = _neck(num_classes, 1024)
        self._init_runtime()

    def val(self, x):
        return self._run(x, False)[0]

    def forward(self, x):
        self._prepare_head_grads()
        logits, feat = self._run(x, True)
        if getattr(self, "skip_necks", False):
            return logits, None, None
        direct = bool(getattr(self, "direct_grads", False)) and torch.is_grad_enabled()
        high = heads.projection_neck(self.dense_projection_high, feat, direct=direct)
        head = heads.projection_neck(self.dense_projection_head, logits, direct=direct)
        return logits, high, head
```

hpfg_amd/train.py:

```python
from __future__ import annotations

import contextlib
import ctypes as C
import math
import os
from typing import Dict, Optional

import numpy as np
import torch

from . import _lib as L
from .utils import (BoxMaskGenerator, build_lr_scheduler, build_optimizer, ema_alpha, linear_rampup, seg_loss, sigmoid_rampup,
                    update_ema_variables, update_ema_variables_backbone)
from .utils.loss import _nhwc
from .utils.optim import FusedSGD

S_LR1, S_LR2, S_ALPHA, S_THRESH, S_COEF_A, S_COEF_B = 0, 1, 2, 3, 8, 16


class StepScalars:

    SLOTS = 8

    def __init__(self, dev):
# ... 93 lines not shown
        self.host_scalars(cur_itrs, **kw)
        self.sc.push()
        r = self.device_step(*inputs)
        self.after()
        return r

    def device_step(self, *inputs):
        r = self.device_fwd_bwd(*inputs)
        self.exchange()
        self.device_update()
        return r

    def exchange(self):
        self._reduce_grads(*self.trainable)

    def device_update(self):
        for o in self.optimizers:
            o.step(push_lr=False) if hasattr(o, "push_lr") else o.step()

    def after(self):
        for s in self.lr_schedulers:
            s.step()

    def _cons_w(self, cur_itrs, cons_w=None, rampup=sigmoid_rampup):
        a = self.args
        return a.consistency * rampup(cur_itrs // 150, a.consistency_rampup) if cons_w is None else cons_w

    def _mark(self, i):
        if self.marks is not None:
            L.check(L.load().hpfg_timestamp(self.marks.data_ptr() + 8 * i, torch.cuda.current_stream(self.dev).cuda_stream), "timestamp")

    def _side2(self):
        if self.side2 is None:
            self.side2 = torch.cuda.Stream(device=self.dev)
        return self.side2

    @contextlib.contextmanager
    def _fork(self, stream):
        stream.wait_stream(torch.cuda.current_stream(self.dev))
        with torch.cuda.stream(stream):
            yield

    def _join(self, stream, *outs):
        cur = torch.cuda.current_stream(self.dev)
        cur.wait_stream(stream)
        for o in outs:
            for t_ in (o if isinstance(o, (tuple, list)) else (o,)):
                for u in (t_ if isinstance(t_, (tuple, list)) else (t_,)):
                    if torch.is_tensor(u):
                        u.record_stream(cur)

    def _teacher_forward(self, x, forked: bool = False):
        with (torch.cuda.stream(self.side) if forked else self._fork(self.side)), torch.no_grad():
            self._mark(2)
            out = self.ema_model(x)
            self._mark(3)
        return out

    def _backward(self, loss, stream):
        for o in self.optimizers:
            o.zero_grad()
        loss.backward()
        self._join(stream)

    def _attach(self, model, alone: bool = False):
        model.dp = self.dp
        model._alone = bool(alone)
        if alone:
            model.defer_wgrad = True
        if any(p.requires_grad for p in model.parameters()):
            model.direct_grads = True

    def _loss_backward(self, res):
        if getattr(self, "_g1", None) is None or self._g1.device != res.device:
            self._g1 = torch.zeros(res.numel(), dtype=res.dtype, device=res.device)
            self._g1[0] = 1.0
        res.backward(self._g1)

    def _reduce_grads(self, *models):
        if self.dp is not None and (self.dp.world_size > 1 or self.dp.force_sync):
            p2p = getattr(self.dp, "p2p_grads", False)
            red = self.dp.peer_allreduce_sum if p2p else self.dp.allreduce_sum
            for m in models:
                if getattr(m, "_buckets_launched", False):
                    m._buckets_launched = False
                    self.dp.join_buckets()
                elif hasattr(m, "flat_grads") and not hasattr(m, "_hpfg_generic_flat"):
                    red(m.flat_grads)
                elif getattr(m, "_hpfg_flat_optimizer", None) is not None:
                    opt = m._hpfg_flat_optimizer
                    assert opt.external_gather, "a flat-buffer optimizer under data parallel must be registered with _StepBase._own_gather"
                    red(opt.gather_flat_grads())
                else:
                    gs = [p.grad for p in m.parameters() if p.grad is not None]
                    flat = torch.cat([g.reshape(-1) for g in gs])
                    red(flat)
                    o = 0
                    for g in gs:
                        g.copy_(flat[o:o + g.numel()].view_as(g))
                        o += g.numel()

    def _own_gather(self, *optimizers):
        active = self.dp is not None and (self.dp.world_size > 1 or self.dp.force_sync)
        for o in optimizers:
            if hasattr(o, "external_gather"):
                o.external_gather = bool(active)

    def _set_grad_scale(self, *optimizers):
        if self.dp is not None and not getattr(self.dp, "sync_bn", True):
            for o in optimizers:
                o.grad_scale = 1.0 / self.dp.world_size

    @staticmethod
    def _lr(opt):
        lr = opt.param_groups[0]["lr"]
        return 0.0 if torch.is_tensor(lr) else float(lr)


class SupervisedStep(_StepBase):
    def __init__(self, model, args, dp=None):
        super().__init__(args, dp, [model])
        self.sc.host[S_COEF_A:S_COEF_A + 2] = torch.tensor([0.5, 0.5])

    def host_scalars(self, cur_itrs):
        self.sc.host[S_LR1] = self._lr(self.optimizer)

    def device_fwd_bwd(self, img, label):
        out = self.model(img)
        res = seg_loss(out, label, coef=self.sc.view(S_COEF_A, 8), dp=self.dp)
        self.optimizer.zero_grad()
        self._loss_backward(res)
        return {"loss": res[0].detach(), "logits": out.detach(), "parts": res.detach()}

    def step(self, img, label, cur_itrs):
        return self.eager_step((img, label), cur_itrs)


class _TeacherStudentStep(_StepBase):

    def __init__(self, model, ema_model, args, dp=None):
        super().__init__(args, dp, [model], ema_model)

    def host_scalars(self, cur_itrs, cons_w=None):
        w = self._cons_w(cur_itrs, cons_w)
        h = self.sc.host
        h[S_LR1] = self._lr(self.optimizer)
        h[S_ALPHA] = ema_alpha(cur_itrs, self.args.ema_decay)
        h[S_COEF_A:S_COEF_A + 5] = torch.tensor([0.5, 0.5, 0.0, 0.0, w])
        return w

    def device_update(self):
        fs, ft = getattr(self.model, "flat_params", None), getattr(self.ema_model, "flat_params", None)
        if isinstance(self.optimizer, FusedSGD) and fs is not None and ft is not None and fs.numel() == ft.numel() and fs.is_cuda:
            self.optimizer.step(push_lr=False, ema=(ft, fs.numel(), self.sc.view(S_ALPHA)))
        else:
            self.optimizer.step(push_lr=False)
            update_ema_variables(self.model, self.ema_model, self.args.ema_decay, 0, alpha_dev=self.sc.view(S_ALPHA))


class MeanTeacherStep(_TeacherStudentStep):
    def __init__(self, model, ema_model, args, dp=None):
        super().__init__(model, ema_model, args, dp)
        self.teacher_after = 7

    def device_fwd_bwd(self, label_img, target_label, unlabel_img):
        nl = label_img.shape[0]
        x = cat_batch(label_img, unlabel_img)
        self._mark(0)
        ev = torch.cuda.Event()
        ev.record(torch.cuda.current_stream(self.dev))
        self._mark(1)
        box = []

        def teacher():
            with torch.cuda.stream(self.side), torch.no_grad():
                self.side.wait_event(ev)
                self._mark(2)
                box.append(self.ema_model(x))
                self._mark(3)

        self.model._after_layer = (self.teacher_after, teacher)
        try:
            out = self.model(x)
        finally:
            self.model._after_layer = None
        if not box:
            teacher()
        t_out = box[0]
        self._mark(4)
        self._join(self.side, t_out)
        self._mark(5)
        res = seg_loss(out, target_label, nl, coef=self.sc.view(S_COEF_A, 8), teacher_logits=t_out, dp=self.dp)
        self.optimizer.zero_grad()
        self._loss_backward(res)
        self._mark(6)
        return {"loss": res[0].detach(), "parts": res.detach(), "logits": out.detach(), "t_logits": t_out}

    def device_update(self):
        super().device_update()
        self._mark(7)

    def step(self, label_img, target_label, unlabel_img, cur_itrs, cons_w=None):
        return self.eager_step((label_img, target_label, unlabel_img), cur_itrs, cons_w=cons_w)


def mix_samples(a: torch.Tensor, b: torch.Tensor, f: torch.Tensor) -> torch.Tensor:
    a, b, f = a.contiguous(), b.contiguous(), f.reshape(-1).float().contiguous()
    out = torch.empty_like(a)
    L.check(L.load().hpfg_mix_samples(L.ptr(a), L.ptr(b), L.ptr(f), L.ptr(out), a.shape[0], a[0].numel(),
                                      torch.cuda.current_stream(a.device).cuda_stream), "mix_samples")
    return out


def softmax_mix(t0: torch.Tensor, t1: torch.Tensor, f: torch.Tensor) -> torch.Tensor:
    x0, x1 = _nhwc(t0.detach()), _nhwc(t1.detach())
    n, H, W, Cc = x0.shape
    out = torch.empty(n, H, W, Cc, dtype=torch.float32, device=x0.device)
    L.check(L.load().hpfg_softmax_mix(L.ptr(x0), L.ptr(x1), L.ptr(f.reshape(-1).float().contiguous()), L.ptr(out), n, H, W, Cc,
                                      torch.cuda.current_stream(x0.device).cuda_stream), "softmax_mix")
    return out.permute(0, 3, 1, 2)


class ICTStep(_TeacherStudentStep):

    def draw_mix_factors(self, unlabel_bs: int, rng=None) -> torch.Tensor:
        rng = np.random if rng is None else rng
        a = float(getattr(self.args, "ict_alpha", 0.2))
        return torch.tensor(rng.beta(a, a, size=(unlabel_bs // 2, 1, 1, 1)), dtype=torch.float)

    def device_step(self, label_img, target_label, unlabel_img, mix_factors):
        nl, nu = label_img.shape[0], unlabel_img.shape[0]
        u0, u1 = unlabel_img[:nu // 2], unlabel_img[nu // 2:]
        f = mix_factors.to(label_img.device)
        x = torch.cat([label_img, mix_samples(u0, u1, f)], 0)
        with torch.no_grad():
            t0 = self.ema_model(u0.contiguous())
            t1 = self.ema_model(u1.contiguous())
        out = self.model(x)
        tp = softmax_mix(t0, t1, f)
        res = seg_loss(out, target_label, nl, coef=self.sc.view(S_COEF_A, 8), teacher_prob=tp, dp=self.dp)
        self.optimizer.zero_grad()
        self._loss_backward(res)
        self.exchange()
        self.device_update()
        return {"loss": res[0].detach(), "parts": res.detach(), "logits": out.detach(), "t_prob": tp}

    def step(self, label_img, target_label, unlabel_img, cur_itrs, mix_factors=None, cons_w=None):
        if mix_factors is None:
            mix_factors = self.draw_mix_factors(unlabel_img.shape[0])
        return self.eager_step((label_img, target_label, unlabel_img, mix_factors), cur_itrs, cons_w=cons_w)


def noise_add(x: torch.Tensor, noise: torch.Tensor, scale: float = 0.1, lo: float = -0.2, hi: float = 0.2) -> torch.Tensor:
    x, noise = x.contiguous(), noise.float().contiguous()
    if noise.numel() % x.numel():
        raise ValueError("noise must hold a whole number of copies of x")
    out = torch.empty_like(noise)
    L.check(L.load().hpfg_noise_add(L.ptr(x), L.ptr(noise), L.ptr(out), x.numel(), noise.numel(), scale, lo, hi,
                                    torch.cuda.current_stream(x.device).cuda_stream), "noise_add")
    return out


def uncertainty_mask(pred_blocks, n_images: int, threshold_dev: torch.Tensor, want_uncertainty: bool = False):
    xs = [_nhwc(b.detach().float()) for b in pred_blocks]
    per, H, W, Cc = xs[0].shape
    if any(tuple(x.shape) != (per, H, W, Cc) for x in xs) or (len(xs) * per) % n_images:
        raise ValueError("prediction blocks must have one shape and hold T*n_images predictions")
    T = len(xs) * per // n_images
    pb = L.PredBlocks()
    for i, x in enumerate(xs):
        pb.p[i] = x.data_ptr()
    pb.n_blocks, pb.per_block = len(xs), per
    dev = xs[0].device
    mask = torch.empty(n_images, 1, H, W, dtype=torch.float32, device=dev)
    unc = torch.empty(n_images, 1, H, W, dtype=torch.float32, device=dev) if want_uncertainty else None
    L.check(L.load().hpfg_uncertainty_mask(C.byref(pb), T, n_images, H, W, Cc, L.ptr(threshold_dev), L.ptr(mask), L.ptr(unc),
                                           torch.cuda.current_stream(dev).cuda_stream), "uncertainty_mask")
    return (mask, unc) if want_uncertainty else mask


class UAMTStep(_TeacherStudentStep):

    T = 8

    def host_scalars(self, cur_itrs, cons_w=None):
        w = super().host_scalars(cur_itrs, cons_w)
        self.sc.host[S_THRESH] = (0.75 + 0.25 * sigmoid_rampup(cur_itrs, self.args.total_itrs)) * math.log(2)
        return w

    def draw_noise(self, unlabel_img):
        n0 = torch.randn_like(unlabel_img)
        rest = [torch.randn(2 * unlabel_img.shape[0], *unlabel_img.shape[1:], device=unlabel_img.device) for _ in range(self.T // 2)]
        return n0, rest

    def device_step(self, label_img, target_label, unlabel_img, noise0, noises):
        nl, nu = label_img.shape[0], unlabel_img.shape[0]
        out = self.model(cat_batch(label_img, unlabel_img))
        with torch.no_grad():
            ema_out = self.ema_model(noise_add(unlabel_img, noise0))
            preds = [self.ema_model(noise_add(unlabel_img, nz)) for nz in noises]
        mask = uncertainty_mask(preds, nu, self.sc.view(S_THRESH))
        res = seg_loss(out, target_label, nl, coef=self.sc.view(S_COEF_A, 8), teacher_logits=ema_out, cons_mask=mask, dp=self.dp)
        self.optimizer.zero_grad()
        self._loss_backward(res)
        self.exchange()
        self.device_update()
        return {"loss": res[0].detach(), "parts": res.detach(), "logits": out.detach(), "mask": mask, "t_logits": ema_out.detach()}

    def step(self, label_img, target_label, unlabel_img, cur_itrs, noise=None, cons_w=None):
        n0, rest = self.draw_noise(unlabel_img) if noise is None else noise
        return self.eager_step((label_img, target_label, unlabel_img, n0, rest), cur_itrs, cons_w=cons_w)


class CPSStep(_StepBase):
    def __init__(self, model1, model2, args, dp=None):
        super().__init__(args, dp, [model1, model2])

    def host_scalars(self, cur_itrs, cons_w=None):
        w = self._cons_w(cur_itrs, cons_w)
        h = self.sc.host
        h[S_LR1], h[S_LR2] = self._lr(self.optimizer1), self._lr(self.optimizer2)
        h[S_COEF_A:S_COEF_A + 5] = torch.tensor([0.5, 0.5, 0.5 * w, 0.5 * w, 0.0])
        return w

    def device_fwd_bwd(self, label_img, target_label, unlabel_img):
        nl = label_img.shape[0]
        x = cat_batch(label_img, unlabel_img)
        with self._fork(self.side):
            o2 = self.model2(x)
        o1 = self.model1(x)
        self._join(self.side, o2)
        p1 = argmax_labels(o1[nl:])
        p2 = argmax_labels(o2[nl:])
        coef = self.sc.view(S_COEF_A, 8)
        r1 = seg_loss(o1, target_label, nl, coef=coef, pseudo=p2, dp=self.dp)
        r2 = seg_loss(o2, target_label, nl, coef=coef, pseudo=p1, dp=self.dp)
        loss = r1[0] + r2[0]
        self._backward(loss, self.side)
        return {"loss": loss.detach(), "parts1": r1.detach(), "parts2": r2.detach(), "logits1": o1.detach(), "logits2": o2.detach()}

    def step(self, label_img, target_label, unlabel_img, cur_itrs, cons_w=None):
        return self.eager_step((label_img, target_label, unlabel_img), cur_itrs, cons_w=cons_w)


class HPFGStep(_StepBase):
    def __init__(self, model1, model2, ema_model, args, dp=None):
        from .model.segformer import SegFormer_Plus
        from .utils import Dense_Loss
        from .utils.optim import FusedAdamW, flatten_parameters
        plus = [isinstance(m, SegFormer_Plus) for m in (model1, model2, ema_model)]
        if any(plus):
            if not all(plus):
                raise NotImplementedError("HPFGStep: mixed U-Net / SegFormer_Plus networks are not built (the three networks must be of one kind)")
            if dp is not None:
                raise NotImplementedError("HPFGStep: data parallel (dp is not None) with SegFormer_Plus networks is not built")
            for m in (model1, model2, ema_model):
                flatten_parameters(m)
        self.reference_call_order = all(plus)
        super().__init__(args, dp, [model1, model2], ema_model)
        if hasattr(model1, "dense_projection_high"):
            model1.skip_necks = True
            if isinstance(self.optimizer1, (FusedSGD, FusedAdamW)):
                self.optimizer1.active_numel = model1.backbone_numel()
        self.dense_loss = Dense_Loss(args.batch_size + args.unlabel_batch_size, self.dev)
        self.dense_loss.dp = dp
        self.mask_generator = BoxMaskGenerator(prop_range=(0.25, 0.5), n_boxes=4, random_aspect_ratio=True, prop_by_area=True,
                                               within_bounds=True, invert=True)
        self._w = 0.0

    def host_scalars(self, cur_itrs):
        w = self._cons_w(cur_itrs, rampup=linear_rampup)
        h = self.sc.host
        h[S_LR1], h[S_LR2] = self._lr(self.optimizer1), self._lr(self.optimizer2)
        h[S_ALPHA] = ema_alpha(cur_itrs, self.args.ema_decay)
        h[S_COEF_A:S_COEF_A + 5] = torch.tensor([0.5, 0.5, 0.0, 7.0 * w, 0.0])
        h[S_COEF_B:S_COEF_B + 5] = torch.tensor([0.5, 0.5, 0.0, 0.0, 0.0 if cur_itrs < 1000 else w])
        h[3] = w
        self._w = w
        return w

    def _student_args(self):
        return getattr(self.args, "model1", self.args), getattr(self.args, "model2", self.args)

    def make_cutmix_mask(self, n, shape, rng=None, device=None):
        if device is not None:
            return self.mask_generator.generate_params_device(n_masks=n, mask_shape=shape, device=device, rng=rng)
        m = self.mask_generator.generate_params(n_masks=n, mask_shape=shape, rng=rng)
        return torch.tensor(m, dtype=torch.float)

    def device_fwd_bwd(self, label_img, target_label, label_img1, target_label1, img_unlabel, cutmix_mask):
        nl = label_img.shape[0]
        mix_un = cutmix_blend(label_img1, img_unlabel, cutmix_mask)
        batch_mix = torch.cat([label_img, mix_un], 0)
        with self._fork(self._side2()):
            o1, _, _ = self.model1(batch_mix)
        volume = cat_batch(label_img, img_unlabel)
        if self.reference_call_order:
            self.side.wait_stream(torch.cuda.current_stream(self.dev))
            o2, h1, h2 = self.model2(volume)
            ot, th1, th2 = self._teacher_forward(volume, forked=True)
        else:
            ot, th1, th2 = self._teacher_forward(volume)
            o2, h1, h2 = self.model2(volume)
        self._join(self.side, ot, th1, th2)
        self._join(self.side2, o1)
        batch_mix.record_stream(self.side2)
        pseudo = argmax_labels(ot[nl:], target_label1, cutmix_mask[:, 0])
        r1 = seg_loss(o1, target_label, nl, coef=self.sc.view(S_COEF_A, 8), pseudo=pseudo, dp=self.dp)
        r2 = seg_loss(o2, target_label, nl, coef=self.sc.view(S_COEF_B, 8), teacher_logits=ot, dp=self.dp)
        contrast = self.dense_loss(h1, th1) + self.dense_loss(h2, th2)
        loss = r1[0] + r2[0] + self.sc.view(3)[0] * contrast
        self._backward(loss, self.side2)
        return {"loss": loss.detach(), "parts1": r1.detach(), "parts2": r2.detach(), "contrast": contrast.detach(),
                "logits1": o1.detach(), "logits2": o2.detach(), "t_logits": ot}

    def device_update(self):
        super().device_update()
        a = self.sc.view(S_ALPHA)
        update_ema_variables_backbone(self.model1, self.model2, self.args.ema_decay, 0, alpha_dev=a)
        update_ema_variables(self.model2, self.ema_model, self.args.ema_decay, 0, alpha_dev=a)

    def step(self, label_img, target_label, label_img1, target_label1, img_unlabel, cutmix_mask, cur_itrs):
        return self.eager_step((label_img, target_label, label_img1, target_label1, img_unlabel, cutmix_mask), cur_itrs)


class S4CVNetStep(_StepBase):

    def __init__(self, model1, model2, ema_model, args, dp=None):
        super().__init__(args, dp, [model1, model2], ema_model)

    def host_scalars(self, cur_itrs):
        w = self._cons_w(cur_itrs, rampup=linear_rampup)
        h = self.sc.host
        h[S_LR1], h[S_LR2] = self._lr(self.optimizer1), self._lr(self.optimizer2)
        h[S_ALPHA] = ema_alpha(cur_itrs, self.args.ema_decay)
        h[S_COEF_A:S_COEF_A + 5] = torch.tensor([0.5, 0.5, 0.0, 7.0 * w, 0.0 if cur_itrs < 1000 else w])
        return w

    def draw_noise(self, unlabel_img):
        return torch.randn_like(unlabel_img)

    def device_fwd_bwd(self, label_img, target_label, unlabel_img, noise):
        nl = label_img.shape[0]
        x = cat_batch(label_img, unlabel_img)
        ot = self._teacher_forward(noise_add(unlabel_img, noise))
        with self._fork(self._side2()):
            o1 = self.model1(x)
        o2 = self.model2(x)
        self._join(self.side2, o1)
        self._join(self.side, ot)
        p1 = argmax_labels(o1[nl:])
        p2 = argmax_labels(o2[nl:])
        coef = self.sc.view(S_COEF_A, 8)
        r1 = seg_loss(o1, target_label, nl, coef=coef, pseudo=p2, teacher_logits=ot, dp=self.dp)
        r2 = seg_loss(o2, target_label, nl, coef=coef, pseudo=p1, teacher_logits=ot, dp=self.dp)
        loss = r1[0] + r2[0]
        self._backward(loss, self.side2)
        return {"loss": loss.detach(), "parts1": r1.detach(), "parts2": r2.detach(), "logits1": o1.detach(), "logits2": o2.detach(), "t_logits": ot}

    def device_update(self):
        super().device_update()
        update_ema_variables(self.model2, self.ema_model, self.args.ema_decay, 0, alpha_dev=self.sc.view(S_ALPHA))

    def step(self, label_img, target_label, unlabel_img, cur_itrs, noise=None):
        if noise is None:
            noise = self.draw_noise(unlabel_img)
        return self.eager_step((label_img, target_label, unlabel_img, noise), cur_itrs)


class GraphNotCapturable(RuntimeError):
    """GraphedStep's refusal BEFORE anything is captured (a step with host-launched collectives between its kernels): the one condition a
    driver loop answers by staying eager.  Anything raised DURING a capture (an argument check, a workspace that is too small) is a real
    failure and propagates."""


class GraphedStep:

    def __init__(self, step_obj, example_inputs, warmup: int = 3, alias_inputs: bool = False, before_capture=None):
        self.s = step_obj
        dp0 = getattr(step_obj, "dp", None)
        host_gather = isinstance(step_obj, HPFGStep) and not getattr(dp0, "p2p_grads", False)
        if dp0 is not None and getattr(dp0, "sync_bn", True) and (dp0.world_size > 1 or dp0.force_sync) and (not getattr(dp0, "p2p", False) or host_gather):
            raise GraphNotCapturable("GraphedStep: a step with collectives between its kernels (data parallel with sync_bn=True) is not captured into a "
                               "hipGraph; run it eager, enable the peer mailbox exchange (DataParallelContext.enable_peer_exchange: the sums then cross "
                               "the ranks inside the kernels), or use sync_bn=False (per-rank BatchNorm: collectives only between graphs)")
        self.alias = bool(alias_inputs)
        self.static = list(example_inputs) if self.alias else [t.clone() for t in example_inputs]
        self.graph = torch.cuda.CUDAGraph()
        self._seed_words = []
        side = torch.cuda.Stream()
        side.wait_stream(torch.cuda.current_stream())
        with torch.cuda.stream(side):
            for i in range(warmup):
                self.s.eager_step(self.static, i + 1)
        torch.cuda.current_stream().wait_stream(side)
        torch.cuda.synchronize()
        if before_capture is not None:
            before_capture()
        if dp0 is not None:
            dp0._loss_call = 0
        dp = getattr(step_obj, "dp", None)
        self.split = bool(dp is not None and (dp.world_size > 1 or dp.force_sync) and not getattr(dp, "p2p_grads", False))
        if self.split and not hasattr(step_obj, "device_fwd_bwd"):
            raise GraphNotCapturable(f"GraphedStep: {type(step_obj).__name__} has no device_fwd_bwd / exchange / device_update split, so its gradient "
                               "exchange would be captured into the graph; run it eager under data parallel")
        self._freeze_seed_updates(True)
        try:
            self._capture(dp, mode_split=self.split)
        finally:
            self._freeze_seed_updates(False)
            if dp is not None:
                dp.bucket_hook = None

    def _capture(self, dp, mode_split: bool):
        if self.split:
            self.graph_b = torch.cuda.CUDAGraph()
            self.graphs, self.bucket_after = [self.graph], []
            overlap = (bool(getattr(dp, "overlap", False))
                       and sum(1 for m in self.s.models if any(p.requires_grad for p in m.parameters())) == 1)
            if overlap:
                mode = "relaxed"
                pad = torch.zeros(1, device=self.static[0].device)
                cap = torch.cuda.Stream()
                torch.cuda.synchronize()
                cap.wait_stream(torch.cuda.current_stream())

                def hook(t):
                    self.graphs[-1].capture_end()
                    self.bucket_after.append(t)
                    g2 = torch.cuda.CUDAGraph()
                    g2.capture_begin(pool=self.graph.pool(), capture_error_mode=mode)
                    self.graphs.append(g2)
                    pad.add_(1.0)

                with torch.cuda.stream(cap):
                    self.graph.capture_begin(capture_error_mode=mode)
                    dp.bucket_hook = hook
                    try:
                        self.out = self.s.device_fwd_bwd(*self.static)
                    finally:
                        dp.bucket_hook = None
                        self.graphs[-1].capture_end()
                torch.cuda.current_stream().wait_stream(cap)
                for m in self.s.models:
                    m._buckets_launched = False
            else:
                prev, dp.overlap = getattr(dp, "overlap", False), False
                try:
                    with torch.cuda.graph(self.graph, capture_error_mode="thread_local"):
                        self.out = self.s.device_fwd_bwd(*self.static)
                finally:
                    dp.overlap = prev
            with torch.cuda.graph(self.graph_b, pool=self.graph.pool(), capture_error_mode="thread_local"):
                self.s.device_update()
        else:
            with torch.cuda.graph(self.graph, capture_error_mode="thread_local"):
                self.out = self.s.device_step(*self.static)

    def _freeze_seed_updates(self, capturing: bool):
        for m in self.s.models:
            m._graph_seed_mode = capturing
            if capturing:
                m._graph_fwds = 0
            else:
                m._fwds_per_replay = getattr(m, "_graph_fwds", 0)

    def step(self, inputs, cur_itrs, **kw):
        for dst, src in zip(self.static, inputs):
            if dst is not src:
                dst.copy_(src, non_blocking=_async_ok(src))
        self.s.host_scalars(cur_itrs, **kw)
        self.s.sc.push()
        for m in self.s.models:
            m.bump_graph_seed()
        if self.split:
            dp = self.s.dp
            for i, g in enumerate(self.graphs):
                g.replay()
                if i < len(self.bucket_after):
                    dp.launch_bucket(self.bucket_after[i])
            if self.bucket_after:
                dp.join_buckets()
            else:
                self.s.exchange()
            self.graph_b.replay()
        else:
            self.graph.replay()
        self.s.after()
        return self.out


class CTCTStep(CPSStep):

    def host_scalars(self, cur_itrs, cons_w=None):
        w = self._cons_w(cur_itrs, cons_w)
        h = self.sc.host
        h[S_LR1], h[S_LR2] = self._lr(self.optimizer1), self._lr(self.optimizer2)
        h[S_COEF_A:S_COEF_A + 5] = torch.tensor([0.5, 0.5, 0.0, w, 0.0])
        return w


def _cycle(loader):
    it = iter(loader)
    while True:
        try:
            yield next(it)
        except StopIteration:
            it = iter(loader)
            yield next(it)


class ScalarLog:

    def __init__(self, dev, width: int, emit, writer=None, every: int = 50):
        self.dev, self.width, self.emit, self.writer = dev, int(width), emit, writer
        self.every = max(1, int(every))
        self.buf = torch.zeros(self.every, self.width, dtype=torch.float32, device=dev)
        self.pending, self.history = [], []
        self.check = None

    def add(self, itr: int, vecs, host: Dict[str, float]):
        k, o = len(self.pending), 0
        for v in vecs:
            v = v.detach().reshape(-1)
            self.buf[k, o:o + v.numel()].copy_(v, non_blocking=True)
            o += v.numel()
        assert o <= self.width
        self.pending.append((int(itr), dict(host)))
        if len(self.pending) == self.every:
            self.flush()

    def flush(self):
        if not self.pending:
            return
        rows = self.buf[:len(self.pending)].cpu()
        if self.check is not None:
            self.check()
        for (itr, host), row in zip(self.pending, rows):
            named = self.emit([float(x) for x in row], host)
            self.history.append((itr, named))
            if self.writer is not None:
                for name, val in named.items():
                    self.writer.add_scalar(name, val, itr)
        self.pending = []

    def losses(self) -> torch.Tensor:
        self.flush()
        vals = [next((v for n, v in named.items() if n.endswith("/loss")), float("nan")) for _, named in self.history]
        return torch.tensor(vals, dtype=torch.float32, device=self.dev)


def _async_ok(src: torch.Tensor) -> bool:
    return src.is_cuda or src.is_pinned()


class _LoopRunner:

    def __init__(self, st, args, width: int, emit, vec_keys, host_fn):
        self.st, self.args, self.vec_keys, self.host_fn = st, args, vec_keys, host_fn
        self.dev = torch.device(args.device)
        self.slog = ScalarLog(self.dev, width, emit, getattr(args, "writer", None), int(getattr(args, "log_every", 50) or 50))
        self.graph_ok = bool(getattr(args, "hipgraph", True)) and os.environ.get("HPFG_LOOP_GRAPH", "1") == "1"
        self.runner, self.n = None, 0
        dp = getattr(args, "dp", None)
        if dp is not None:
            self.slog.check = dp.check_peer_errors

    def _to_dev(self, t):
        t = t.to(self.dev, non_blocking=_async_ok(t))
        return t.float() if t.is_floating_point() and t.dtype != torch.float32 else t

    def __call__(self, inputs, cur_itrs: int, **kw):
        self.n += 1
        r = None
        if self.graph_ok and self.n >= 2:
            if self.runner is None:
                dev_in = [self._to_dev(t) for t in inputs]
                try:
                    self.runner = GraphedStep(self.st, dev_in, warmup=0)
                except GraphNotCapturable as e:
                    logger = getattr(self.args, "logger", None)
                    if logger is not None:
                        logger.warning(f"hipGraph capture unavailable ({e}); running eager")
                    self.graph_ok = False
            if self.runner is not None and all(tuple(a.shape) == tuple(b.shape) for a, b in zip(inputs, self.runner.static)):
                r = self.runner.step(list(inputs), cur_itrs, **kw)
        if r is None:
            r = self.st.eager_step((self._to_dev(t) for t in inputs), cur_itrs, **kw)
        self.slog.add(cur_itrs, [r[k] for k in self.vec_keys], self.host_fn())
        return r

    def drive(self, loader, inputs_of, test_loader, evals):
        args, cur_itrs = self.args, 0
        for _ in range(args.total_itrs // len(loader) + 1):
            for batch in loader:
                cur_itrs += 1
                self(inputs_of(batch), cur_itrs)
                _check_peers(args, cur_itrs)
                if test_loader is not None and cur_itrs % args.step_size == 0:
                    for best, model, optimizer, lr_scheduler, name in evals:
                        best(model, optimizer, lr_scheduler, test_loader, cur_itrs, name)
                if cur_itrs > args.total_itrs:
                    _check_peers(args, cur_itrs, final=True)
                    return self.slog.losses()
        _check_peers(args, cur_itrs, final=True)
        return self.slog.losses()


def _with_labels(label_loader, extra=None):
    labels = _cycle(label_loader)

    def inputs_of(batch):
        unlabel_img, _ = batch
        label_img, target_label = next(labels)
        return [label_img, target_label, unlabel_img] + (list(extra(unlabel_img)) if extra is not None else [])

    return inputs_of


def _sup_of(row, o=0):
    return 0.5 * (row[o + 1] + row[o + 2])


def eval_hd95_route(args):
    v = getattr(args, "eval_hd95", None)
    if v is None or v is False:
        return False
# ... 189 lines not shown
```

hpfg_amd/utils/optim.py:

```python
from __future__ import annotations

import torch

from .. import _lib as L
from .scheduler import CosineWarmupLR_Scheduler, Medical_LR, PolyLR


class FusedSGD(torch.optim.Optimizer):
    def __init__(self, model, lr=0.01, momentum=0.0, weight_decay=0.0):
        self.model = model
        params = [p for p in model.parameters() if p.requires_grad]
        super().__init__(params, dict(lr=lr, momentum=momentum, weight_decay=weight_decay))
        flat = model.flat_params
        self._mom = torch.zeros_like(flat)
        self._lr_host = torch.zeros(1, dtype=torch.float32).pin_memory() if torch.cuda.is_available() else torch.zeros(1)
        self._lr_dev = torch.zeros(1, dtype=torch.float32, device=flat.device)
        self.grad_scale = 1.0
        self.active_numel = None

    def zero_grad(self, set_to_none: bool = False):
        if hasattr(self.model, "_hpfg_generic_flat"):
            for p in self.model.parameters():
                p.grad = None
            return
        self.model.zero_flat_grad()
        self.model.attach_grad_views()

    def push_lr(self):
        self._lr_host[0] = float(self.param_groups[0]["lr"])
        self._lr_dev.copy_(self._lr_host, non_blocking=True)

    @torch.no_grad()
    def step(self, closure=None, push_lr: bool = True, ema=None):
        g = self.param_groups[0]
        if hasattr(self.model, "_hpfg_generic_flat"):
            gather_flat_grads(self.model, self.active_numel)
        flat, grad = self.model.flat_params, self.model.flat_grads
        if self._mom.data_ptr() == 0 or self._mom.numel() != flat.numel() or self._mom.device != flat.device:
            self._mom = torch.zeros_like(flat)
        if push_lr:
            self.push_lr()
        st = torch.cuda.current_stream(flat.device).cuda_stream
        n_sgd = flat.numel() if self.active_numel is None else int(self.active_numel)
        if ema is not None:
            t, n_ema, alpha_dev = ema
            assert t.is_cuda and t.dtype == torch.float32 and t.numel() == flat.numel() and 0 <= n_ema <= n_sgd
            L.check(L.load().hpfg_sgd_ema_step(L.ptr(flat), L.ptr(grad), L.ptr(self._mom), n_sgd, L.ptr(self._lr_dev), float(g["momentum"]),
                                               float(g["weight_decay"]), float(self.grad_scale), L.ptr(t), int(n_ema), L.ptr(alpha_dev), st),
                    "sgd_ema_step")
            return
        L.check(L.load().hpfg_sgd_step(L.ptr(flat), L.ptr(grad), L.ptr(self._mom), n_sgd, L.ptr(self._lr_dev), float(g["momentum"]),
                                       float(g["weight_decay"]), float(self.grad_scale), st), "sgd_step")

    def state_dict(self):
        d = super().state_dict()
        d["flat_momentum"] = self._mom
        return d

    def load_state_dict(self, sd):
        sd = dict(sd)
        mom = sd.pop("flat_momentum", None)
        super().load_state_dict(sd)
        if mom is not None:
            self._mom.copy_(mom)


def flatten_parameters(model):
    if hasattr(model, "flat_params"):
        return
    ps = [p for p in model.parameters()]
    dev = ps[0].device
    n = sum(p.numel() for p in ps)
    flat = torch.empty(n, dtype=torch.float32, device=dev)
    grad = torch.zeros(n, dtype=torch.float32, device=dev)
    o = 0
    with torch.no_grad():
        for p in ps:
            k = p.numel()
            flat[o:o + k].copy_(p.detach().reshape(-1))
            p.data = flat[o:o + k].view(p.shape)
            o += k
    model.flat_params, model.flat_grads = flat, grad
    model._hpfg_generic_flat = True


@torch.no_grad()
def gather_flat_grads(model, active_numel=None):
    ps, k = [], 0
    for p in model.parameters():
        if active_numel is not None and k >= active_numel:
            break
        ps.append(p)
        k += p.numel()
    assert active_numel is None or k == active_numel, "active_numel must end on a parameter boundary"
    out = model.flat_grads if active_numel is None else model.flat_grads[:k]
    torch.cat([(p.grad if p.grad is not None else torch.zeros_like(p)).reshape(-1) for p in ps], out=out)
    return model.flat_grads


class FusedAdamW(torch.optim.Optimizer):

    def __init__(self, model, lr=1e-3, weight_decay=1e-2, betas=(0.9, 0.999), eps=1e-8):
        flatten_parameters(model)
        self.model = model
        super().__init__([p for p in model.parameters() if p.requires_grad], dict(lr=lr, weight_decay=weight_decay, betas=betas, eps=eps))
        flat = model.flat_params
        self._m, self._v = torch.zeros_like(flat), torch.zeros_like(flat)
        self._step_dev = torch.zeros(1, dtype=torch.float32, device=flat.device)
        self._lr_host = torch.zeros(1, dtype=torch.float32).pin_memory()
        self._lr_dev = torch.zeros(1, dtype=torch.float32, device=flat.device)
        self.grad_scale = 1.0
        self.external_gather = False
        self.active_numel = None
        model._hpfg_flat_optimizer = self

    def zero_grad(self, set_to_none: bool = True):
        for p in self.model.parameters():
            p.grad = None

    def gather_flat_grads(self):
        return gather_flat_grads(self.model, self.active_numel)

    def push_lr(self):
        self._lr_host[0] = float(self.param_groups[0]["lr"])
        self._lr_dev.copy_(self._lr_host, non_blocking=True)

    @torch.no_grad()
    def step(self, closure=None, push_lr: bool = True):
        g = self.param_groups[0]
        flat = self.model.flat_params
        grad = self.model.flat_grads if self.external_gather else self.gather_flat_grads()
        if push_lr:
            self.push_lr()
        st = torch.cuda.current_stream(flat.device).cuda_stream
        n = flat.numel() if self.active_numel is None else int(self.active_numel)
        L.check(L.load().hpfg_adamw_step(L.ptr(flat), L.ptr(grad), L.ptr(self._m), L.ptr(self._v), n, L.ptr(self._lr_dev), L.ptr(self._step_dev),
                                         float(g["betas"][0]), float(g["betas"][1]), float(g["eps"]), float(g["weight_decay"]), float(self.grad_scale), st),
                "adamw_step")

    def state_dict(self):
        d = super().state_dict()
        d["flat_m"], d["flat_v"], d["step"] = self._m, self._v, self._step_dev
        return d

    def load_state_dict(self, sd):
        sd = dict(sd)
        m, v, st = sd.pop("flat_m", None), sd.pop("flat_v", None), sd.pop("step", None)
        super().load_state_dict(sd)
        if m is not None:
            self._m.copy_(m)
        if v is not None:
            self._v.copy_(v)
        if st is not None:
            self._step_dev.copy_(torch.as_tensor(st, dtype=torch.float32).reshape(1))


def build_optimizer(args, model):
    if args.opt == "sgd":
        if hasattr(model, "flat_params") and model.flat_params.is_cuda:
            return FusedSGD(model, lr=args.lr, momentum=args.momentum, weight_decay=args.weight_decay)
        return torch.optim.SGD(model.parameters(), lr=args.lr, momentum=args.momentum, weight_decay=args.weight_decay)
    if args.opt == "adamW":
        params = list(model.parameters())
        if params and params[0].is_cuda:
            return FusedAdamW(model, lr=args.lr, weight_decay=args.weight_decay)
        return torch.optim.AdamW(params, lr=args.lr, weight_decay=args.weight_decay)
    if args.opt == "adam":
        return torch.optim.Adam(model.parameters(), lr=args.lr, weight_decay=args.weight_decay)
    raise ValueError("get_optimizer error")


def build_lr_scheduler(args, optimizer):
    if args.sched == "cosine":
        return CosineWarmupLR_Scheduler(optimizer=optimizer, base_lr=args.lr, warmup_epochs=args.warmup_epochs, warmup_lr=args.warmup_lr,
                                        final_lr=args.min_lr, iter_per_epoch=args.step_size, num_epochs=args.total_itrs // args.step_size)
    if args.sched == "poly":
        return PolyLR(optimizer, max_iters=args.total_itrs, power=0.1, min_lr=args.min_lr)
    if args.sched == "medical":
        return Medical_LR(optimizer=optimizer, base_lr=args.lr, max_iterations=args.total_itrs)
    raise ValueError("get_lr_scheduler error")
```

hpfg_amd/utils/utils.py:

```python
from __future__ import annotations

import math
import os
import shutil

import numpy as np
import torch
import yaml


class AttrDict(dict):

    def __init__(self, d=None, **kw):
        super().__init__()
        for k, v in dict(d or {}, **kw).items():
            self[k] = v

    def __setitem__(self, k, v):
        if isinstance(v, dict) and not isinstance(v, AttrDict):
            v = AttrDict(v)
        super().__setitem__(k, v)

    def __getattr__(self, k):
        try:
            return self[k]
        except KeyError as e:
            raise AttributeError(k) from e

    __setattr__ = __setitem__


def loadyaml(file_path):
    if file_path is None:
        print("file path is empty")
        return None
    try:
        with open(file_path, "r", encoding="utf-8") as f:
            return AttrDict(yaml.safe_load(f))
    except IOError as e:
        print(e)
        return None


def mk_path(path, remove=False):
    try:
        if not os.path.exists(path):
            os.makedirs(path)
        elif remove:
            shutil.rmtree(path, ignore_errors=True)
    except Exception as e:
        print(e)


def sigmoid_rampup(current, rampup_length):
    if rampup_length == 0:
        return 1.0
    current = float(np.clip(current, 0.0, rampup_length))
    phase = 1.0 - current / rampup_length
    return float(math.exp(-5.0 * phase * phase))


def linear_rampup(current, rampup_length):
    assert current >= 0 and rampup_length >= 0
    return 1.0 if current >= rampup_length else current / rampup_length


def get_current_consistency_weight(epoch, args):
    return args.consistency * sigmoid_rampup(epoch, args.consistency_rampup)


def ema_alpha(global_step: int, alpha: float) -> float:
    return min(1 - 1 / (global_step + 1), alpha)


def _flat_pair(model, ema_model):
    fp = getattr(model, "flat_params", None)
    fe = getattr(ema_model, "flat_params", None)
    if fp is None or fe is None or fp.numel() != fe.numel() or not fp.is_cuda:
        return None
    return fp, fe


_alpha_cache = {}


def _alpha_dev(dev, alpha: float) -> torch.Tensor:
    t = _alpha_cache.get(dev)
    if t is None:
        t = _alpha_cache[dev] = torch.zeros(1, dtype=torch.float32, device=dev)
    t.fill_(alpha)
    return t


def update_ema_variables(model, ema_model, alpha, global_step, alpha_dev: torch.Tensor = None, numel: int = None):
    from .. import _lib as L
    pair = _flat_pair(model, ema_model)
    if pair is None:
        raise RuntimeError("update_ema_variables needs two hpfg_amd U-Nets on the GPU (no CPU fallback)")
    src, dst = pair
    n = src.numel() if numel is None else numel
    a = alpha_dev if alpha_dev is not None else _alpha_dev(src.device, ema_alpha(global_step, alpha))
    L.check(L.load().hpfg_ema_update(L.ptr(dst), L.ptr(src), n, L.ptr(a), torch.cuda.current_stream(src.device).cuda_stream), "ema_update")


def update_ema_variables_backbone(model, ema_model, alpha, global_step, alpha_dev: torch.Tensor = None):
    update_ema_variables(model, ema_model, alpha, global_step, alpha_dev, numel=model.backbone_numel())


class BoxMaskGenerator(object):

    def __init__(self, prop_range, n_boxes=1, random_aspect_ratio=True, prop_by_area=True, within_bounds=True, invert=False):
        if isinstance(prop_range, float):
            prop_range = (prop_range, prop_range)
        self.prop_range, self.n_boxes = prop_range, n_boxes
        self.random_aspect_ratio, self.prop_by_area = random_aspect_ratio, prop_by_area
        self.within_bounds, self.invert = within_bounds, invert

    def draw_rects(self, n_masks, mask_shape, rng=None):
        rng = np.random if rng is None else rng
        lo, hi = self.prop_range
        nb = self.n_boxes
        if self.prop_by_area:
            props = rng.uniform(lo, hi, size=(n_masks, nb))
            zero = props == 0.0
            if self.random_aspect_ratio:
                y_props = np.exp(rng.uniform(low=0.0, high=1.0, size=(n_masks, nb)) * np.log(props))
                x_props = props / y_props
            else:
                y_props = x_props = np.sqrt(props)
            fac = np.sqrt(1.0 / nb)
            y_props, x_props = y_props * fac, x_props * fac
            y_props[zero] = 0
            x_props[zero] = 0
        else:
            if self.random_aspect_ratio:
                y_props = rng.uniform(lo, hi, size=(n_masks, nb))
                x_props = rng.uniform(lo, hi, size=(n_masks, nb))
            else:
                x_props = y_props = rng.uniform(lo, hi, size=(n_masks, nb))
            fac = np.sqrt(1.0 / nb)
            y_props, x_props = y_props * fac, x_props * fac
        shape = np.array(mask_shape)
        sizes = np.round(np.stack([y_props, x_props], axis=2) * shape[None, None, :])
        if self.within_bounds:
            pos = np.round((shape - sizes) * rng.uniform(low=0.0, high=1.0, size=sizes.shape))
            rects = np.append(pos, pos + sizes, axis=2)
        else:
            cen = np.round(shape * rng.uniform(low=0.0, high=1.0, size=sizes.shape))
            rects = np.append(cen - sizes * 0.5, cen + sizes * 0.5, axis=2)
        return rects

    def generate_params(self, n_masks, mask_shape, rng=None):
        rects = self.draw_rects(n_masks, mask_shape, rng)
        masks = np.zeros((n_masks, 1) + tuple(mask_shape)) if self.invert else np.ones((n_masks, 1) + tuple(mask_shape))
        for i, sample in enumerate(rects):
            for y0, x0, y1, x1 in sample:
                sl = (i, 0, slice(int(y0), int(y1)), slice(int(x0), int(x1)))
                masks[sl] = 1 - masks[sl]
        return masks

    def generate_params_device(self, n_masks, mask_shape, device, rng=None):
        import ctypes as C

        import torch

        from .. import _lib as L
        rects = self.draw_rects(n_masks, mask_shape, rng)
        H, W = int(mask_shape[0]), int(mask_shape[1])
        norm = np.zeros((n_masks, self.n_boxes, 4), dtype=np.int32)
        for i, sample in enumerate(rects):
            for b, (y0, x0, y1, x1) in enumerate(sample):
                ys, ye, _ = slice(int(y0), int(y1)).indices(H)
                xs, xe, _ = slice(int(x0), int(x1)).indices(W)
                norm[i, b] = (ys, max(ye, ys), xs, max(xe, xs))
        r = torch.from_numpy(norm).to(device, non_blocking=True)
        out = torch.empty(n_masks, 1, H, W, dtype=torch.float32, device=device)
        L.check(L.load().hpfg_box_masks(L.ptr(r), n_masks, self.n_boxes, H, W, 1 if self.invert else 0, L.ptr(out),
                                        torch.cuda.current_stream(device).cuda_stream), "box_masks")
        return out

    def torch_masks_from_params(self, t_params, mask_shape, torch_device):
        return t_params
```

include/hpfg_hip.h:

```cpp
#ifndef HPFG_HIP_H
#define HPFG_HIP_H

#include <stdint.h>

#ifdef __cplusplus
extern "C" {
#endif

#define HPFG_VERSION 139
enum { HPFG_MATH_F32 = 0, HPFG_MATH_BF16X3 = 1 };

enum { HPFG_BN_MEAN = 0, HPFG_BN_RSTD = 1, HPFG_BN_SCALE = 2, HPFG_BN_SHIFT = 3,
       HPFG_BN_K1 = 4, HPFG_BN_K2 = 5, HPFG_BN_K3 = 6, HPFG_BN_SPARE = 7, HPFG_BN_ROWS = 8 };

enum {
  HPFG_ACT_NONE = 0,
  HPFG_ACT_PLAIN = 1,
  HPFG_ACT_STRIDED = 2,
  HPFG_ACT_BNACT = 3,
  HPFG_ACT_BNACT_POOL = 4,
  HPFG_ACT_UP2X = 5,
  HPFG_ACT_DZ = 6,
  HPFG_ACT_SPLIT16 = 7,
  HPFG_ACT_UPBWD = 8
};

typedef struct HpfgAct {
  const float* z;
  const float* bn;
  const float* aux;
  int32_t mode;
  int32_t C;
  int32_t Hs, Ws;
  int32_t pstride;
  int32_t aux_pstride;
  int32_t bn_stride;
  int32_t bn_coff;
  int32_t sn, sc, sy, sx;
  float drop_p;
  uint32_t drop_seed;
  const uint8_t* drop_mask;
  const uint32_t* seed_dev;
  const long long* bn_acc;
  const float* bn_gamma;
  const float* bn_beta;
  float bn_count;
  float bn_eps;
  int32_t bn_shards;
  int32_t reserved1;
} HpfgAct;

typedef struct HpfgConvArgs {
  HpfgAct a0, a1;
  const float* wpk;
  const float* bias;
  float* out;
  float* stat_partials;
  int32_t out_pstride, Cout, CoutPad;
  int32_t N, H, W;
  int32_t taps;
  int32_t math;
  int32_t bwd_stats;
  HpfgAct bwd_of;
  float* out2;
  int32_t out_split;
  int32_t out2_pstride;
  long long* stat_acc;
  int32_t stat_shards;
  int32_t reserved2;
  float* stage_out;
  float* side_sums;
} HpfgConvArgs;
#define HPFG_ACC_MAX_SHARDS 8
#define HPFG_ACC_WORDS(C, shards) ((shards) * 2 * 2 * (C))

typedef struct HpfgWgradArgs {
  HpfgAct a0, a1;
  HpfgAct g;
  float* slab;
  float* dw_oihw;
  int32_t Cin, CinPad, Cout, CoutPad;
  int32_t N, H, W, taps;
  int32_t S;
  int32_t math;
  int32_t defer_reduce;
} HpfgWgradArgs;

typedef struct HpfgFusedBwdArgs {
  HpfgConvArgs d;
  HpfgAct xa0, xa1;
  float* slab;
  int32_t Cin, CinPad, Cout, CoutPad;
} HpfgFusedBwdArgs;

typedef struct HpfgSlabDesc {
  const float* slab;
  float* dw_oihw;
  int32_t S, taps, Cin, CinPad, Cout, CoutPad;
} HpfgSlabDesc;

typedef struct HpfgPackDesc {
  const float* w_oihw;
  const float* b;
  float* wpk_fwd;
  float* wpk_dgrad;
  float* bias_pad;
  void* wpk16_fwd;
  void* wpk16_dgrad;
  int32_t Cout, Cin, CoutPad, CinPad, taps;
  int32_t kc;
} HpfgPackDesc;

int hpfg_version(void);
const char* hpfg_last_error(void);
enum { HPFG_OPT_CONV_THIN = 0, HPFG_OPT_FIRST_MFMA = 1, HPFG_OPT_FIRST_WGRAD = 2, HPFG_OPT_NARROW_DEEP = 3, HPFG_OPT_COUNT = 4 };
int hpfg_set_option(int which, int value);

int hpfg_conv3x3_first_fwd(const HpfgAct* x, const float* w_oihw, const float* bias, float* out, float* stat_partials,
                           int N, int H, int W, int Cin, int Cout, void* stream);
int hpfg_conv_first_rows(int N, int H, int W);
int hpfg_conv3x3_first_fwd_acc(const HpfgAct* x, const float* w_oihw, const float* bias, float* out, float* stat_partials, long long* stat_acc,
                               int stat_shards, int N, int H, int W, int Cin, int Cout, void* stream);
int hpfg_conv_fwd(const HpfgConvArgs* args, void* stream);
int hpfg_conv_stat_blocks(int N, int H, int W);
int hpfg_conv_stat_rows(const HpfgConvArgs* args);
int hpfg_bn_fwd_finalize(const float* partials, int nblk, const double* sums, double count, const float* gamma, const float* beta,
                         float* running_mean, float* running_var, float momentum, float eps, float* bn, int C, void* stream);
typedef struct HpfgBnAccDesc {
  const long long* acc;
  const float* gamma;
  const float* beta;
  float* running_mean;
  float* running_var;
  float* bn;
  int32_t C;
  float count;
  int32_t shards;
  int32_t reserved;
} HpfgBnAccDesc;
int hpfg_bn_acc_finalize(const HpfgBnAccDesc* table_dev, const HpfgBnAccDesc* table_host, int nlayers, float momentum, float eps, void* stream);
typedef struct HpfgBnAccBwdDesc {
  long long* acc;
  const float* gamma;
  float* bn;
  float* dgamma;
  float* dbeta;
  int32_t C;
  float count;
  int32_t shards;
  int32_t reserved;
} HpfgBnAccBwdDesc;
int hpfg_bn_acc_bwd_finalize(const HpfgBnAccBwdDesc* table_dev, const HpfgBnAccBwdDesc* table_host, int nlayers, void* stream);
int hpfg_bn_bwd_reduce_acc(const HpfgAct* g, int N, int H, int W, long long* acc, int shards, void* stream);
int hpfg_bn_bwd_reduce_pool_acc(const HpfgAct* g, const float* dP, int dp_pstride, int N, int Hp, int Wp, long long* acc, int shards, void* stream);
int hpfg_reduce_partials(const float* partials, int nblk, int C, double* sums, void* stream);
int hpfg_bn_eval_table(const float* gamma, const float* beta, const float* running_mean, const float* running_var, float eps,
                       float* bn, int C, void* stream);
int hpfg_conv_kc(int H, int W, int taps);
long hpfg_wpk16_elems(int Kchannels, int NchannelsPad, int taps, int kc);
int hpfg_pack_weights(const HpfgPackDesc* table_dev, const HpfgPackDesc* table_host, int nlayers, void* stream);
int hpfg_pack_weights_bump(const HpfgPackDesc* table_dev, const HpfgPackDesc* table_host, int nlayers, long long* counters, int n_counters,
                           int32_t* seed_word, int seed_add, long long* zero_words, long n_zero, void* stream);
int hpfg_act_materialize(const HpfgAct* a0, const HpfgAct* a1, int N, int H, int W, float* out, void* stream);
int hpfg_dropout_mask(uint8_t* out, long n_elems, float p, uint32_t seed, const uint32_t* seed_dev, void* stream);

int hpfg_bn_bwd_reduce(const HpfgAct* g , int N, int H, int W, float* partials, void* stream);
int hpfg_bn_bwd_blocks(int N, int H, int W, int C);
int hpfg_bn_bwd_reduce_pool(const HpfgAct* g , const float* dP, int dp_pstride, int N, int Hp, int Wp,
                            float* partials , void* stream);
int hpfg_bn_bwd_pool_blocks(int N, int Hp, int Wp, int C);
int hpfg_bn_bwd_finalize(const float* partials, int nblk, const double* sums, double count, const float* gamma,
                         float* bn, float* dgamma, float* dbeta, int C, float param_grad_scale, void* stream);
int hpfg_wgrad(const HpfgWgradArgs* args, void* stream);
int hpfg_fused_bwd(const HpfgFusedBwdArgs* args, void* stream);
int hpfg_fused_bwd_grid(const HpfgFusedBwdArgs* args);
int hpfg_slab_reduce_multi(const HpfgSlabDesc* table_dev, const HpfgSlabDesc* table_host, int nlayers, void* stream);
int hpfg_wgrad_splits(int N, int H, int W, int CinPad, int CoutPad, int taps);
long hpfg_wgrad_slab_floats(int N, int H, int W, int CinPad, int CoutPad, int taps);
int hpfg_channel_sum(const float* g, int pstride, long npix, int C, float* out, float* scratch, void* stream);
int hpfg_channel_sum_partials(const float* g, int pstride, long npix, int C, float* partials, void* stream);
int hpfg_channel_sum_blocks(long npix, int C);
int hpfg_pool_scatter_add(const HpfgAct* src , const float* dP, int dp_pstride,
                          float* dA, int da_pstride, int N, int Hp, int Wp, void* stream);
int hpfg_upsample2x_bwd(const float* dUp, int dup_pstride, float* dU, int N, int Hl, int Wl, int C, void* stream);
int hpfg_upsample2x_bwd_sums(const float* dUp, int dup_pstride, float* dU, int N, int Hl, int Wl, int C, float* csum_partials, void* stream);
int hpfg_upsample2x_bwd_blocks(int N, int Hl, int Wl, int C);

#define HPFG_PEER_MAX_RANKS 8
#define HPFG_PEER_HANDLE_BYTES 64
#define HPFG_PEER_MAX_SPINS (1L << 22)
typedef struct HpfgPeerX {
  void* mbox[HPFG_PEER_MAX_RANKS];
  const int32_t* epoch;
  int32_t* err;
  int32_t world, rank;
  int32_t slot, cap;
  int64_t slot_bytes;
} HpfgPeerX;
long hpfg_peer_slot_bytes(int world, int cap);
int hpfg_peer_alloc(size_t bytes, void** ptr);
int hpfg_peer_free(void* ptr);
int hpfg_peer_handle(void* ptr, unsigned char* handle64);
int hpfg_peer_open(const unsigned char* handle64, void** ptr);
int hpfg_peer_close(void* ptr);
int hpfg_word_add(int32_t* word, int v, void* stream);
int hpfg_bn_fwd_finalize_x(const float* partials, int nblk, const HpfgPeerX* px, double count, const float* gamma, const float* beta,
                           float* running_mean, float* running_var, float momentum, float eps, float* bn, int C, void* stream);
int hpfg_bn_bwd_finalize_x(const float* partials, int nblk, const HpfgPeerX* px, double count, const float* gamma, float* bn, float* dgamma,
                           float* dbeta, int C, float param_grad_scale, void* stream);

typedef struct HpfgPeerBuf {
  void* win[HPFG_PEER_MAX_RANKS];
  int32_t* epoch;
  int32_t* err;
  int32_t world, rank;
  int64_t slice;
  int64_t n;
  int64_t stride;
} HpfgPeerBuf;
long hpfg_peer_buf_slice(int world, long n);
long hpfg_peer_buf_bytes(int world, long n);
int hpfg_peer_allreduce_f32(const HpfgPeerBuf* pb, float* buf, void* stream);

typedef struct HpfgLossArgs {
  const float* logits;
  const float* t_logits;
  const uint8_t* labels0;
  const uint8_t* labels1;
  const float* coef;
  float* partials;
  float* sums;
  float* out;
  float* dlogits;
  int32_t N, n_lab, H, W, C;
  int32_t world;
  int32_t input_is_prob;
  int32_t teacher_is_prob;
  int32_t t_unlab_only;
  int32_t reserved0;
  const float* cons_mask;
} HpfgLossArgs;
#define HPFG_LOSS_NSUM 32
#define HPFG_LOSS_NSUM_WIDE 104
int hpfg_loss_blocks(int N, int H, int W);
int hpfg_loss_nsum(int C);
int hpfg_seg_loss_partials(const HpfgLossArgs* a, void* stream);
int hpfg_seg_loss_partials_x(const HpfgLossArgs* a, const HpfgPeerX* px, void* stream);
int hpfg_seg_loss_finalize(const HpfgLossArgs* a, void* stream);
int hpfg_seg_loss_bwd(const HpfgLossArgs* a, const float* grad_scale_dev , void* stream);
int hpfg_argmax_labels(const float* logits, int N, int H, int W, int C, const uint8_t* mix_labels, const float* mix_mask,
                       uint8_t* out, void* stream);
int hpfg_confusion_counts(const uint8_t* pred, const uint8_t* gt, long n, int C, unsigned long long* counts, void* stream);
#define HPFG_RESIZE_TAPS 36
int hpfg_resize_cubic(const float* src, int S, int h, int w, float* dst, int H, int W, const float* taps_y, const float* taps_x, void* scratch,
                      long scratch_bytes, void* stream);
long hpfg_resize_cubic_scratch_bytes(int S, int h, int w, int H, int W);
#define HPFG_SURFACE_SEGS 32
int hpfg_surface_counts(const uint8_t* pred, const uint8_t* gt, int S, int h, int w, int C, int ndim, unsigned int* counts, void* stream);
int hpfg_surface_distances(const uint8_t* pred, const uint8_t* gt, int S, int h, int w, int C, int ndim, const unsigned int* counts_host,
                           void* workspace, long workspace_bytes, void* stream);
long hpfg_surface_workspace_bytes(int C, long n_points);
int hpfg_surface_sums(const void* workspace, long workspace_bytes, int C, const unsigned int* counts_host, long long* sums, void* stream);
typedef struct HpfgAugSample {
  int64_t img_off, lab_off;
  int32_t h, w;
  int32_t mode;
  int32_t k, axis;
  int32_t tab_off;
  double m00, m01, m10, m11, off_y, off_x;
} HpfgAugSample;
int hpfg_augment_batch(const float* img_pool, const uint8_t* lab_pool, const HpfgAugSample* samples_dev, const int* tabs_dev, int B, int H, int W,
                       float* out_img, uint8_t* out_lab, void* stream);
int hpfg_box_masks(const int* rects, int n, int n_boxes, int H, int W, int invert, float* out, void* stream);
int hpfg_mix_samples(const float* a, const float* b, const float* f, float* out, int n, long per_sample, void* stream);
int hpfg_softmax_mix(const float* t0, const float* t1, const float* f, float* out_prob, int n, int H, int W, int C, void* stream);
int hpfg_timestamp(unsigned long long* slot, void* stream);
int hpfg_noise_add(const float* x, const float* noise, float* out, long n_src, long n_out, float scale, float lo, float hi, void* stream);
typedef struct HpfgPredBlocks {
  const float* p[8];
  int32_t n_blocks, per_block;
} HpfgPredBlocks;
int hpfg_uncertainty_mask(const HpfgPredBlocks* pb, int T, int S, int H, int W, int C, const float* threshold_dev, float* mask ,
                          float* uncertainty , void* stream);
int hpfg_cutmix_blend(const float* a, const float* b, const float* mask, float* out, long n, void* stream);

int hpfg_ln_fwd(const float* x, const float* gamma, const float* beta, float* y, float* mean, float* rstd, long rows, int C, void* stream);
int hpfg_ln_bwd(const float* x, const float* dy, const float* gamma, const float* mean, const float* rstd, float* dx, float* dgamma, float* dbeta ,
                float* partials , long rows, int C, void* stream);
int hpfg_ln_bwd_blocks(long rows);
int hpfg_attn_fwd(const float* q, const float* kv, float* out, int B, int N, int M, int heads, float scale, void* stream);
int hpfg_attn_bwd(const float* q, const float* kv, const float* dout, float* dq, float* P, float* dS, int B, int N, int M, int heads, float scale,
                  void* stream);
int hpfg_attn_fwd_hd(const float* q, const float* kv, float* out, int B, int N, int M, int heads, int head_dim, float scale, void* stream);
int hpfg_attn_bwd_hd(const float* q, const float* kv, const float* dout, float* dq, float* P, float* dS, int B, int N, int M, int heads, int head_dim,
                     float scale, void* stream);
int hpfg_dwgelu_fwd(const float* x, const float* w9, const float* bias, float* y, int B, int H, int W, int C, void* stream);
int hpfg_dwgelu_bwd(const float* x, const float* w9, const float* bias, const float* dy, float* du , float* dx, float* dw9,
                    float* dbias , float* partials , int B, int H, int W, int C, void* stream);
int hpfg_dwgelu_bwd_blocks(int B, int H, int W);
int hpfg_resize_bilinear_fwd(const float* x, float* y, int B, int h, int w, int H, int W, int C, void* stream);
int hpfg_resize_sum_fwd(const float* base, const float* const* xs, const int* hs, const int* ws, int nsrc, float* y, int B, int H, int W, int C,
                        void* stream);
int hpfg_resize_bilinear_bwd(const float* dy, float* dx, int B, int h, int w, int H, int W, int C, void* stream);
int hpfg_residual_scale(const float* x, const float* y, const float* scale, float* out, int B, long per_sample, void* stream);
int hpfg_scale_rows(const float* d, const float* scale, float* out, int B, long per_sample, void* stream);
int hpfg_gelu_fwd(const float* x, float* y, long n, void* stream);
int hpfg_gelu_bwd(const float* x, const float* dy, float* dx, long n, void* stream);
int hpfg_patch_merge_fwd(const float* x, float* y, int B, int H, int W, int C, void* stream);
int hpfg_patch_merge_bwd(const float* dy, float* dx, int B, int H, int W, int C, void* stream);
int hpfg_im2col_nhwc(const float* x, float* cols, int B, int H, int W, int C, int k, int s, void* stream);
int hpfg_col2im_nhwc(const float* dcols, float* dx, int B, int H, int W, int C, int k, int s, void* stream);
int hpfg_linear_wgrad(const float* dy, const float* x, float* dw, float* partials , long R, int N, int K,
                      void* stream);
int hpfg_linear_wgrad_splits(long R, int N, int K);
int hpfg_tok_col_stats(const float* x, long R, int C, float* partials , float* sums , void* stream);
int hpfg_tok_stat_blocks(long R);
int hpfg_bnrelu_apply(const float* x, const float* mean, const float* rstd, const float* gamma, const float* beta, const float* mask, float inv_keep,
                      long rows_per_image, float* y, long R, int C, void* stream);
int hpfg_bnrelu_bwd(const float* x, const float* dy, const float* mean, const float* rstd, const float* gamma, const float* beta, const float* mask,
                    float inv_keep, long rows_per_image, float* dx, float* partials, float* sums, long R, int C, void* stream);

int hpfg_sgd_step(float* p, const float* g, float* mom, long n, const float* lr_dev, float momentum, float weight_decay,
                  float grad_scale, void* stream);
int hpfg_adamw_step(float* p, const float* g, float* m, float* v, long n, const float* lr_dev, float* step_dev, float beta1, float beta2, float eps,
                    float weight_decay, float grad_scale, void* stream);
int hpfg_ema_update(float* t, const float* s, long n, const float* alpha_dev, void* stream);

int hpfg_sgd_ema_step(float* p, const float* g, float* mom, long n, const float* lr_dev, float momentum, float weight_decay, float grad_scale,
                      float* t, long n_ema, const float* alpha_dev, void* stream);

int hpfg_attn_mfma_fwd(const float* q, const float* kv, float* out, int B, int N, int M, int heads, float scale, void* stream);
int hpfg_attn_mfma_bwd(const float* q, const float* kv, const float* dout, float* dq, float* dkv, float* scratch, int B, int N, int M, int heads,
                       float scale, void* stream);
int hpfg_attn_mfma_blocks(int N);
int hpfg_attn_mfma_fwd_hd(const float* q, const float* kv, float* out, int B, int N, int M, int heads, int head_dim, float scale, void* stream);
int hpfg_attn_mfma_bwd_hd(const float* q, const float* kv, const float* dout, float* dq, float* dkv, float* scratch, int B, int N, int M, int heads,
                          int head_dim, float scale, void* stream);
long hpfg_attn_mfma_scratch_floats(int B, int N, int heads, int head_dim);

int hpfg_attn_keys_max(void);
int hpfg_attn_keys_fwd(const float* q, const float* kv, float* out, float* lse, int B, int N, int M, int heads, int head_dim, float scale, int math,
                       void* stream);
int hpfg_attn_keys_bwd(const float* q, const float* kv, const float* out, const float* lse, const float* dout, float* dq, float* dkv, float* scratch,
                       int B, int N, int M, int heads, int head_dim, float scale, int math, void* stream);
long hpfg_attn_keys_scratch_floats(int B, int N, int M, int heads, int head_dim, int math);

int hpfg_attn_window_fwd(const float* qkv, const float* bias_table, float* out, int B, int H, int W, int heads, int head_dim, int window, int shift,
                         float scale, int math, void* stream);
int hpfg_attn_window_bwd(const float* qkv, const float* bias_table, const float* dout, float* dqkv, float* dbias, float* scratch, int B, int H, int W,
                         int heads, int head_dim, int window, int shift, float scale, int math, void* stream);
long hpfg_attn_window_scratch_floats(int B, int H, int W, int heads, int head_dim, int window, int math);

int hpfg_gemm_f32(const float* A, long sam, long sak, const float* B, long sbk, long sbn, float* C, long ldc, int M, int N, int K,
                  const float* bias, int relu, int accumulate, void* stream);
int hpfg_gemm_f32_splitk(const float* A, long sam, long sak, const float* B, long sbk, long sbn, float* C, long ldc, int M, int N, int K,
                         const float* bias, int relu, int accumulate, float* scratch, void* stream);
int hpfg_gemm_f32_splits(int M, int N, int K);
int hpfg_gemm_bf16x3(const float* A, long sam, long sak, const float* B, long sbk, long sbn, float* C, long ldc, int M, int N, int K,
                     const float* bias, int relu, int accumulate, void* stream);
int hpfg_gemm_bf16x3_splits(int M, int N, int K);
int hpfg_gemm_bf16x3_splitk(const float* A, long sam, long sak, const float* B, long sbk, long sbn, float* Cm, long ldc, int M, int N, int K,
                            const float* bias, int relu, int accumulate, float* scratch, void* stream);
int hpfg_gemm_bf16x3_ok(const float* A, long sam, long sak, const float* B, long sbk, long sbn, int M, int N, int K);
int hpfg_gemm_tn_bf16x3(const float* dy, const float* x, float* dw_db, float* partials, long R, int N, int K, int with_db, void* stream);
int hpfg_gemm_tn_splits(long R, int N, int K);
int hpfg_col_sum(const float* x, long R, int M, long ldx, float* out , void* stream);
int hpfg_col_sum2(const float* x, long R, int M, long ldx, float* out, float* scratch , void* stream);
int hpfg_col_sum_splits(long R);
int hpfg_relu_bwd(float* dy, const float* y, long n, void* stream);
int hpfg_neck_pool_fwd(const float* x, int pstride, int N, int H, int W, int C, int S, float* gap, float* pool, void* stream);
int hpfg_neck_pool_bwd(const float* dgap , const float* dpool , int N, int H, int W, int C, int S,
                       float* dx , void* stream);
int hpfg_l2norm_fwd(const float* x, int G, int D, int S, int sd, int ss, float* u, float* norms , void* stream);
int hpfg_l2norm_bwd(const float* du, const float* u, const float* norms, int G, int D, int S, int sd, int ss,
                    const float* scale , float* dx, void* stream);
int hpfg_ntxent_rows(const float* gram, int n, float temperature, float* loss, float* Q, void* stream);

#ifdef __cplusplus
}
#endif
#endif
```

Baseline: 7966 images/s.

## Fuse SGD+EMA update with bf16 split weight-fragment packing for student and teacher

Adds a fused kernel that performs the SGD momentum step and EMA teacher update per 16x16 weight tile, then writes the packed split-bf16 fwd/dgrad MFMA fragments and padded biases for both the student and teacher engines directly from shared memory. This removes the separate weight-packing passes that previously re-read the fp32 parameters before the next forward and backward. It also folds counter and seed bumps into the first conv kernel through a new bump entry point, which drops small launches. The cost is added complexity: a per-layer descriptor table, gap handling, and staleness tokens that must stay consistent or the engines will use outdated fragments.

Result: faster. 8060 images/s (median of 6 runs) (+1.2%).

```diff
diff --git a/hpfg_amd/_lib.py b/hpfg_amd/_lib.py
--- a/hpfg_amd/_lib.py
+++ b/hpfg_amd/_lib.py
@@ -9,11 +9,11 @@
 
 BN_MEAN, BN_RSTD, BN_SCALE, BN_SHIFT, BN_K1, BN_K2, BN_K3, BN_SPARE, BN_ROWS = range(9)
 ACT_NONE, ACT_PLAIN, ACT_STRIDED, ACT_BNACT, ACT_BNACT_POOL, ACT_UP2X, ACT_DZ, ACT_SPLIT16, ACT_UPBWD = range(9)
-OPT_CONV_THIN, OPT_FIRST_MFMA, OPT_FIRST_WGRAD, OPT_NARROW_DEEP = 0, 1, 2, 3
+OPT_CONV_THIN, OPT_FIRST_MFMA, OPT_FIRST_WGRAD, OPT_NARROW_DEEP, OPT_UPDATE_PACK = 0, 1, 2, 3, 4
 LOSS_NSUM = 32
 LOSS_MAX_CLASSES = 16
 ACC_MAX_SHARDS = 8
-VERSION = 139
+VERSION = 140
 RESIZE_TAPS = 36
 SURFACE_SEGS = 32
 MATH_F32, MATH_BF16X3 = 0, 1
@@ -88,6 +88,12 @@
                 ("CoutPad", C.c_int32), ("CinPad", C.c_int32), ("taps", C.c_int32), ("kc", C.c_int32)]
 
 
+class UpdatePackDesc(C.Structure):
+    _fields_ = [("w_off", C.c_long), ("b_off", C.c_long), ("wpk16_fwd", C.c_void_p), ("wpk16_dgrad", C.c_void_p), ("bias_pad", C.c_void_p),
+                ("t_wpk16_fwd", C.c_void_p), ("t_bias_pad", C.c_void_p), ("Cout", C.c_int32), ("Cin", C.c_int32), ("CoutPad", C.c_int32),
+                ("CinPad", C.c_int32), ("taps", C.c_int32), ("kc", C.c_int32), ("kc_t", C.c_int32), ("reserved", C.c_int32)]
+
+
 class LossArgs(C.Structure):
     _fields_ = [("logits", C.c_void_p), ("t_logits", C.c_void_p), ("labels0", C.c_void_p), ("labels1", C.c_void_p),
                 ("coef", C.c_void_p), ("partials", C.c_void_p), ("sums", C.c_void_p), ("out", C.c_void_p),
@@ -106,6 +112,8 @@
     "hpfg_version": (_i, []),
     "hpfg_last_error": (C.c_char_p, []),
     "hpfg_set_option": (_i, [_i, _i]),
+    "hpfg_get_option": (_i, [_i]),
+    "hpfg_conv3x3_first_fwd_bump": (_i, [C.POINTER(Act), _p, _p, _p, _p, _p, _i, _p, _i, _p, _i, _i, _i, _i, _i, _i, _p]),
     "hpfg_conv3x3_first_fwd": (_i, [C.POINTER(Act), _p, _p, _p, _p, _i, _i, _i, _i, _i, _p]),
     "hpfg_conv_fwd": (_i, [C.POINTER(ConvArgs), _p]),
     "hpfg_conv_stat_blocks": (_i, [_i, _i, _i]),
@@ -202,6 +210,7 @@
     "hpfg_adamw_step": (_i, [_p, _p, _p, _p, _l, _p, _p, _f, _f, _f, _f, _f, _p]),
     "hpfg_ema_update": (_i, [_p, _p, _l, _p, _p]),
     "hpfg_sgd_ema_step": (_i, [_p, _p, _p, _l, _p, _f, _f, _f, _p, _l, _p, _p]),
+    "hpfg_sgd_ema_pack_step": (_i, [_p, _p, _p, _l, _p, _f, _f, _f, _p, _l, _p, _p, C.POINTER(UpdatePackDesc), _i, _p, C.POINTER(C.c_long), _i, _p]),
     "hpfg_attn_mfma_fwd": (_i, [_p, _p, _p, _i, _i, _i, _i, _f, _p]),
     "hpfg_attn_mfma_bwd": (_i, [_p, _p, _p, _p, _p, _p, _i, _i, _i, _i, _f, _p]),
     "hpfg_attn_mfma_blocks": (_i, [_i]),
@@ -267,6 +276,8 @@
             lib.hpfg_set_option(OPT_FIRST_WGRAD, 0)
         if os.environ.get("HPFG_NARROW_DEEP") is not None:
             lib.hpfg_set_option(OPT_NARROW_DEEP, int(os.environ["HPFG_NARROW_DEEP"]))
+        if os.environ.get("HPFG_UPDATE_PACK", "1") == "0":
+            lib.hpfg_set_option(OPT_UPDATE_PACK, 0)
         _lib = lib
     return _lib
 
diff --git a/hpfg_amd/csrc/conv.hip b/hpfg_amd/csrc/conv.hip
--- a/hpfg_amd/csrc/conv.hip
+++ b/hpfg_amd/csrc/conv.hip
@@ -11,7 +11,18 @@
   float* stat_partials;
   long long* stat_acc;
   int stat_shards;
+  long long* counters;
+  int n_counters;
+  int* seed_word;
+  int seed_add;
 };
+
+__device__ __forceinline__ void first_bump(const HpfgFirstConvArgs& q) {
+  if (blockIdx.x == 0) {
+    for (int i = threadIdx.x; i < q.n_counters; i += 256) q.counters[i] += 1;
+    if (threadIdx.x == 0 && q.seed_word && q.seed_add) *q.seed_word = (*q.seed_word + q.seed_add) & 0x7FFFFFFF;
+  }
+}
 
 inline bool tile_is_big(int H, int W) { return (H % 16 == 0) && (W % 16 == 0); }
 
@@ -28,6 +39,7 @@
   __shared__ float red[2][4][CO];
   const int tid = threadIdx.x, lane = tid & 63, wave = tid >> 6;
   const int ntiles = tiles_x * tiles_y, nwork = ntiles * N;
+  first_bump(q);
   for (int i = tid; i < 9 * Cin * CO; i += 256) {
     int co = i % CO, r = i / CO, ci = r % Cin, tap = r / Cin;
     wl[i] = w[(co * Cin + ci) * 9 + tap];
@@ -110,6 +122,7 @@
   __shared__ float red[2][4][CO];
   const int tid = threadIdx.x, lane = tid & 63, wave = tid >> 6;
   const int ntiles = tiles_x * tiles_y, nwork = ntiles * N;
+  first_bump(q);
   const int co_a = lane & 15, kq = lane >> 4;
   float wa[KS];
   int boff[KS];
@@ -335,7 +348,18 @@
 extern "C" int hpfg_conv3x3_first_fwd(const HpfgAct* x, const float* w_oihw, const float* bias, float* out, float* stat_partials,
                                       int N, int H, int W, int Cin, int Cout, void* stream) {
   HPFG_ARG_CHECK(x, "conv_first: null pointer");
-  HpfgFirstConvArgs a = {*x, w_oihw, bias, out, stat_partials, nullptr, 1};
+  HpfgFirstConvArgs a = {*x, w_oihw, bias, out, stat_partials, nullptr, 1, nullptr, 0, nullptr, 0};
+  return conv_first_impl(&a, N, H, W, Cin, Cout, stream);
+}
+
+extern "C" int hpfg_conv3x3_first_fwd_bump(const HpfgAct* x, const float* w_oihw, const float* bias, float* out, float* stat_partials, long long* stat_acc,
+                                           int stat_shards, long long* counters, int n_counters, int32_t* seed_word, int seed_add, int N, int H, int W,
+                                           int Cin, int Cout, void* stream) {
+  HPFG_ARG_CHECK(x, "conv_first_bump: null pointer");
+  HPFG_ARG_CHECK(!stat_acc || (stat_shards >= 1 && stat_shards <= HPFG_ACC_MAX_SHARDS && (stat_shards & (stat_shards - 1)) == 0),
+                 "conv_first_bump: bad shard count %d", stat_shards);
+  HPFG_ARG_CHECK(n_counters >= 0 && (n_counters == 0 || counters) && (seed_add == 0 || seed_word), "conv_first_bump: bad counter arguments");
+  HpfgFirstConvArgs a = {*x, w_oihw, bias, out, stat_partials, stat_acc, stat_acc ? stat_shards : 1, counters, n_counters, seed_word, seed_add};
   return conv_first_impl(&a, N, H, W, Cin, Cout, stream);
 }
 
@@ -343,6 +367,6 @@
                                           int stat_shards, int N, int H, int W, int Cin, int Cout, void* stream) {
   HPFG_ARG_CHECK(x && stat_acc, "conv_first_acc: null pointer");
   HPFG_ARG_CHECK(stat_shards >= 1 && stat_shards <= HPFG_ACC_MAX_SHARDS && (stat_shards & (stat_shards - 1)) == 0, "conv_first_acc: bad shard count %d", stat_shards);
-  HpfgFirstConvArgs a = {*x, w_oihw, bias, out, stat_partials, stat_acc, stat_shards};
+  HpfgFirstConvArgs a = {*x, w_oihw, bias, out, stat_partials, stat_acc, stat_shards, nullptr, 0, nullptr, 0};
   return conv_first_impl(&a, N, H, W, Cin, Cout, stream);
 }
diff --git a/hpfg_amd/csrc/misc.hip b/hpfg_amd/csrc/misc.hip
--- a/hpfg_amd/csrc/misc.hip
+++ b/hpfg_amd/csrc/misc.hip
@@ -12,8 +12,9 @@
 extern "C" const char* hpfg_last_error(void) { return g_err; }
 extern "C" int hpfg_version(void) { return HPFG_VERSION; }
 
-static int g_opt[HPFG_OPT_COUNT] = {1, 1, 1, 128};
+static int g_opt[HPFG_OPT_COUNT] = {1, 1, 1, 128, 1};
 int hpfg_opt(int which) { return which >= 0 && which < HPFG_OPT_COUNT ? g_opt[which] : 0; }
+extern "C" int hpfg_get_option(int which) { return hpfg_opt(which); }
 extern "C" int hpfg_set_option(int which, int value) {
   HPFG_ARG_CHECK(which >= 0 && which < HPFG_OPT_COUNT, "set_option: unknown option %d", which);
   const int old = g_opt[which];
diff --git a/hpfg_amd/csrc/update_pack.hip b/hpfg_amd/csrc/update_pack.hip
--- /dev/null
+++ b/hpfg_amd/csrc/update_pack.hip
@@ -0,0 +1,258 @@
+#include "common.h"
+
+namespace {
+
+constexpr int UP_ROW = 16 * 9 + 1;
+constexpr int UP_MAX_LAYERS = 32, UP_MAX_GAPS = 64;
+constexpr int UP_CHUNK = 1024;
+
+struct UpArgs {
+  float* p;
+  const float* g;
+  float* mom;
+  float* t;
+  long n, n_ema;
+  const float* lr_dev;
+  const float* alpha_dev;
+  float momentum, wd, gscale;
+  const HpfgUpdatePackDesc* table;
+  int nlayers;
+  const long* gaps;
+  int ngaps;
+  int wg0[UP_MAX_LAYERS + 1];
+  int gwg0[UP_MAX_GAPS + 1];
+};
+
+__device__ __forceinline__ void update_math(const UpArgs& a, float w, float g, float m, float tv, float lr, float al, float* b, float* s, float* tn) {
+#pragma clang fp contract(off)
+  float d = g * a.gscale + a.wd * w;
+  *b = a.momentum * m + d;
+  *s = w - lr * *b;
+  *tn = tv * al + *s * (1.f - al);
+}
+
+__device__ __forceinline__ float update_elem(const UpArgs& a, long i, float lr, float al, float* tn) {
+  const bool has_t = a.t && i < a.n_ema;
+  float b, s, tv;
+  update_math(a, a.p[i], a.g[i], a.mom[i], has_t ? a.t[i] : 0.f, lr, al, &b, &s, &tv);
+  a.mom[i] = b;
+  a.p[i] = s;
+  if (has_t) a.t[i] = tv;
+  *tn = has_t ? tv : 0.f;
+  return s;
+}
+
+template <int TAPS>
+__device__ __forceinline__ void update_block(const UpArgs& a, const HpfgUpdatePackDesc& d, int co0, int ci0, float lr, float al, float* sw, float* st) {
+  constexpr int ROW = 16 * TAPS, PER = 16 * ROW / 256;
+  float* __restrict__ p = a.p;
+  const float* __restrict__ g = a.g;
+  float* __restrict__ mom = a.mom;
+  float* __restrict__ t = a.t;
+  long idx[PER];
+  float w[PER], gv[PER], mv[PER], tv[PER];
+#pragma unroll
+  for (int k = 0; k < PER; ++k) {
+    const int e = threadIdx.x + 256 * k, r = e / ROW, q = e % ROW;
+    idx[k] = (co0 + r < d.Cout && ci0 + q / TAPS < d.Cin) ? d.w_off + ((long)(co0 + r) * d.Cin + ci0) * TAPS + q : -1;
+    w[k] = gv[k] = mv[k] = tv[k] = 0.f;
+    if (idx[k] >= 0) {
+      w[k] = p[idx[k]];
+      gv[k] = g[idx[k]];
+      mv[k] = mom[idx[k]];
+      if (t && idx[k] < a.n_ema) tv[k] = t[idx[k]];
+    }
+  }
+#pragma unroll
+  for (int k = 0; k < PER; ++k) {
+    const int e = threadIdx.x + 256 * k, r = e / ROW, q = e % ROW;
+    float b, s = 0.f, tn = 0.f;
+    if (idx[k] >= 0) {
+      update_math(a, w[k], gv[k], mv[k], tv[k], lr, al, &b, &s, &tn);
+      mom[idx[k]] = b;
+      p[idx[k]] = s;
+      if (t && idx[k] < a.n_ema) t[idx[k]] = tn;
+      else tn = 0.f;
+    }
+    sw[r * UP_ROW + q] = s;
+    st[r * UP_ROW + q] = tn;
+  }
+}
+
+__device__ __forceinline__ void update_chunk(const UpArgs& a, long lo, long hi, float lr, float al) {
+  constexpr int PER = UP_CHUNK / 256;
+  float* __restrict__ p = a.p;
+  const float* __restrict__ g = a.g;
+  float* __restrict__ mom = a.mom;
+  float* __restrict__ t = a.t;
+  float w[PER], gv[PER], mv[PER], tv[PER];
+#pragma unroll
+  for (int k = 0; k < PER; ++k) {
+    const long i = lo + threadIdx.x + 256 * k;
+    w[k] = gv[k] = mv[k] = tv[k] = 0.f;
+    if (i < hi) {
+      w[k] = p[i];
+      gv[k] = g[i];
+      mv[k] = mom[i];
+      if (t && i < a.n_ema) tv[k] = t[i];
+    }
+  }
+#pragma unroll
+  for (int k = 0; k < PER; ++k) {
+    const long i = lo + threadIdx.x + 256 * k;
+    if (i < hi) {
+      float b, s, tn;
+      update_math(a, w[k], gv[k], mv[k], tv[k], lr, al, &b, &s, &tn);
+      mom[i] = b;
+      p[i] = s;
+      if (t && i < a.n_ema) t[i] = tn;
+    }
+  }
+}
+
+struct bf16x8 {
+  __bf16 v[8];
+} __attribute__((aligned(16)));
+
+__device__ __forceinline__ void store_split8(__bf16* out, long base, int lane, const float* w8) {
+  bf16x8 hi, lo;
+#pragma unroll
+  for (int j = 0; j < 8; ++j) {
+    const __bf16 h = (__bf16)w8[j];
+    hi.v[j] = h;
+    lo.v[j] = (__bf16)(w8[j] - (float)h);
+  }
+  *reinterpret_cast<bf16x8*>(out + (base + 0) * 512 + lane * 8) = hi;
+  *reinterpret_cast<bf16x8*>(out + (base + 1) * 512 + lane * 8) = lo;
+}
+
+__device__ __forceinline__ void frag_pos(int taps, int kc, int k0, int g, int tap, int* ks, int* lq) {
+  if (taps == 1) {
+    *ks = k0 / 32;
+    *lq = (k0 % 32) / 8 + g;
+  } else if (kc == 32) {
+    *ks = (k0 / 32) * 9 + tap;
+    *lq = (k0 % 32) / 8 + g;
+  } else {
+    *ks = (k0 / 16) * 5 + tap / 2;
+    *lq = (tap & 1) * 2 + g;
+  }
+}
+
+__device__ __forceinline__ void emit_fwd(__bf16* out, const float* sw, int taps, int kc, int co0, int ci0, int CoutPad) {
+  const int ntn = CoutPad / 16;
+  for (int it = threadIdx.x; it < 32 * taps; it += 256) {
+    const int r = it & 15, g = (it >> 4) & 1, tap = it >> 5;
+    float w8[8];
+#pragma unroll
+    for (int j = 0; j < 8; ++j) w8[j] = sw[r * UP_ROW + (g * 8 + j) * taps + tap];
+    int ks, lq;
+    frag_pos(taps, kc, ci0, g, tap, &ks, &lq);
+    store_split8(out, ((long)ks * ntn + co0 / 16) * 2, lq * 16 + r, w8);
+  }
+}
+
+__device__ __forceinline__ void emit_dgrad(__bf16* out, const float* sw, int taps, int kc, int co0, int ci0, int CinPad) {
+  const int ntn = CinPad / 16;
+  for (int it = threadIdx.x; it < 32 * taps; it += 256) {
+    const int c = it & 15, g = (it >> 4) & 1, tap = it >> 5;
+    float w8[8];
+#pragma unroll
+    for (int j = 0; j < 8; ++j) w8[j] = sw[(g * 8 + j) * UP_ROW + c * taps + (taps - 1 - tap)];
+    int ks, lq;
+    frag_pos(taps, kc, co0, g, tap, &ks, &lq);
+    store_split8(out, ((long)ks * ntn + ci0 / 16) * 2, lq * 16 + c, w8);
+  }
+}
+
+__global__ __launch_bounds__(256) HPFG_NO_PK_F32 void sgd_ema_pack_kernel(UpArgs a) {
+  __shared__ float sw[16 * UP_ROW], st[16 * UP_ROW];
+  const float lr = *a.lr_dev, al = a.alpha_dev ? *a.alpha_dev : 0.f;
+  const int b = blockIdx.x;
+  if (b >= a.wg0[UP_MAX_LAYERS]) {
+    const int c = b - a.wg0[UP_MAX_LAYERS];
+    int k = 0, base = 0;
+#pragma unroll
+    for (int i = 1; i < UP_MAX_GAPS; ++i)
+      if (i < a.ngaps && c >= a.gwg0[i]) {
+        k = i;
+        base = a.gwg0[i];
+      }
+    const long lo = a.gaps[2 * k] + (long)(c - base) * UP_CHUNK, end = a.gaps[2 * k + 1];
+    update_chunk(a, lo, lo + UP_CHUNK < end ? lo + UP_CHUNK : end, lr, al);
+    return;
+  }
+  int y = 0, first = 0;
+#pragma unroll
+  for (int i = 1; i < UP_MAX_LAYERS; ++i)
+    if (i < a.nlayers && b >= a.wg0[i]) {
+      y = i;
+      first = a.wg0[i];
+    }
+  const HpfgUpdatePackDesc d = a.table[y];
+  const int taps = d.taps, blk = b - first;
+  const int nib = (d.Cin + 15) / 16;
+  if (blk == 0) {
+    for (int i = threadIdx.x; i < d.CoutPad; i += 256) {
+      float tn = 0.f, s = 0.f;
+      if (i < d.Cout) s = update_elem(a, d.b_off + i, lr, al, &tn);
+      d.bias_pad[i] = s;
+      if (d.t_bias_pad) d.t_bias_pad[i] = tn;
+    }
+  }
+  const int co0 = (blk / nib) * 16, ci0 = (blk % nib) * 16;
+  if (taps == 9) update_block<9>(a, d, co0, ci0, lr, al, sw, st);
+  else update_block<1>(a, d, co0, ci0, lr, al, sw, st);
+  __syncthreads();
+  if (d.wpk16_fwd) emit_fwd(reinterpret_cast<__bf16*>(d.wpk16_fwd), sw, taps, d.kc, co0, ci0, d.CoutPad);
+  if (d.wpk16_dgrad) emit_dgrad(reinterpret_cast<__bf16*>(d.wpk16_dgrad), sw, taps, d.kc, co0, ci0, d.CinPad);
+  if (d.t_wpk16_fwd) emit_fwd(reinterpret_cast<__bf16*>(d.t_wpk16_fwd), st, taps, d.kc_t, co0, ci0, d.CoutPad);
+}
+
+}
+
+extern "C" int hpfg_sgd_ema_pack_step(float* p, const float* g, float* mom, long n, const float* lr_dev, float momentum, float weight_decay,
+                                      float grad_scale, float* t, long n_ema, const float* alpha_dev, const HpfgUpdatePackDesc* table_dev,
+                                      const HpfgUpdatePackDesc* table_host, int nlayers, const long* gaps_dev, const long* gaps_host, int ngaps,
+                                      void* stream) {
+  HPFG_ARG_CHECK(p && g && mom && lr_dev && n > 0, "sgd_ema_pack_step: bad args");
+  HPFG_ARG_CHECK((t == nullptr) == (alpha_dev == nullptr) && t != p && n_ema >= 0 && n_ema <= n && (t || n_ema == 0), "sgd_ema_pack_step: bad teacher args");
+  HPFG_ARG_CHECK(table_dev && table_host && nlayers > 0 && nlayers <= UP_MAX_LAYERS && gaps_dev && gaps_host && ngaps >= 0 && ngaps <= UP_MAX_GAPS,
+                 "sgd_ema_pack_step: bad tables (at most %d layers, %d gaps)", UP_MAX_LAYERS, UP_MAX_GAPS);
+  UpArgs a = {p, g, mom, t, n, n_ema, lr_dev, alpha_dev, momentum, weight_decay, grad_scale, table_dev, nlayers, gaps_dev, ngaps, {0}, {0}};
+  long at = 0, wgs = 0;
+  int k = 0;
+  auto gap_to = [&](long lo) {
+    if (at == lo) return true;
+    if (k >= ngaps || gaps_host[2 * k] != at || gaps_host[2 * k + 1] != lo) return false;
+    ++k;
+    at = lo;
+    return true;
+  };
+  for (int i = 0; i < nlayers; ++i) {
+    const HpfgUpdatePackDesc& d = table_host[i];
+    HPFG_ARG_CHECK(d.Cout > 0 && d.Cin > 0 && d.CinPad % 16 == 0 && d.CoutPad % 16 == 0 && d.Cin <= d.CinPad && d.Cout <= d.CoutPad && (d.taps == 1 || d.taps == 9),
+                   "sgd_ema_pack_step: bad descriptor %d", i);
+    HPFG_ARG_CHECK(d.bias_pad && (d.kc == 32 || (d.kc == 16 && d.taps == 9)) && (!d.t_wpk16_fwd || d.kc_t == 32 || (d.kc_t == 16 && d.taps == 9)),
+                   "sgd_ema_pack_step: bad kc or bias row in descriptor %d", i);
+    HPFG_ARG_CHECK((!d.t_wpk16_fwd && !d.t_bias_pad) || t, "sgd_ema_pack_step: descriptor %d has teacher fragments but there is no teacher", i);
+    const long wn = (long)d.Cout * d.Cin * d.taps;
+    HPFG_ARG_CHECK(d.w_off >= at && gap_to(d.w_off), "sgd_ema_pack_step: weight of descriptor %d is out of order or the gaps do not match", i);
+    at += wn;
+    HPFG_ARG_CHECK(d.b_off >= at && gap_to(d.b_off), "sgd_ema_pack_step: bias of descriptor %d is out of order or the gaps do not match", i);
+    at += d.Cout;
+    HPFG_ARG_CHECK(at <= n && (!(d.t_wpk16_fwd || d.t_bias_pad) || at <= n_ema), "sgd_ema_pack_step: descriptor %d ends behind the updated range", i);
+    a.wg0[i] = (int)wgs;
+    wgs += (long)((d.Cout + 15) / 16) * ((d.Cin + 15) / 16);
+  }
+  HPFG_ARG_CHECK(gap_to(n) && k == ngaps, "sgd_ema_pack_step: descriptors and gaps do not tile the %ld elements", n);
+  for (int i = nlayers; i <= UP_MAX_LAYERS; ++i) a.wg0[i] = (int)wgs;
+  long gw = 0;
+  for (int i = 0; i <= UP_MAX_GAPS; ++i) {
+    a.gwg0[i] = (int)gw;
+    if (i < ngaps) gw += (gaps_host[2 * i + 1] - gaps_host[2 * i] + UP_CHUNK - 1) / UP_CHUNK;
+  }
+  HPFG_ARG_CHECK(wgs + gw < (1L << 30), "sgd_ema_pack_step: too many workgroups");
+  hipLaunchKernelGGL(sgd_ema_pack_kernel, dim3((unsigned)(wgs + gw)), dim3(256), 0, (hipStream_t)stream, a);
+  return hpfg_launch_status("sgd_ema_pack_kernel");
+}
diff --git a/hpfg_amd/engine.py b/hpfg_amd/engine.py
--- a/hpfg_amd/engine.py
+++ b/hpfg_amd/engine.py
@@ -156,6 +156,10 @@
         self.wpk16_d = {s.name: torch.empty(self.lib.hpfg_wpk16_elems(s.cout, s.cin_pad, s.taps, self.kc[s.name]), dtype=torch.bfloat16, device=device)
                         for s in self.packed}
         self._pack_tables: Dict[tuple, DescTable] = {}
+        self.frag_token, self.frag_dgrad, self.frag_ok = None, False, False
+        self.pads_zeroed: set = set()
+        self.last_fwd_packed = True
+        self._first_bump: Optional[tuple] = None
         self.bn_layers = [s for s in self.order if s.bn]
         self._bn_idx = {s.name: i for i, s in enumerate(self.bn_layers)}
         self._n_enc_bn = sum(1 for s in self.bn_layers if s.name.startswith("encoder."))
@@ -333,6 +337,8 @@
             assert counters.dtype == torch.int64 and counters.is_contiguous() and counters.device == self.dev
         self._call(self.lib.hpfg_pack_weights_bump, dev, host, n, L.ptr(counters), counters.numel() if counters is not None else 0, L.ptr(self.seed_dev), int(seed_add),
                    None, 0, tag="pack_weights")
+        if self._b16:
+            self.pads_zeroed |= {"f", "d"} if with_dgrad else {"f"}
 
     def _finalize_bwd_all(self, lo: int, hi: int):
         if self.bwd_route != ACC or hi <= lo:
@@ -410,7 +416,14 @@
                 self.acc_all.zero_()
             self._acc_dirty = True
         pack_args = dict(with_dgrad=bool(train and needs_grad), counters=counters, seed_add=1 if seed_step == SEED_BUMP else 0)
-        if not (self.pack_overlap and train):
+        self._first_bump = None
+        self.last_fwd_packed = not (self._b16 and self.frag_ok and self.frag_token is not None and (self.frag_dgrad or not pack_args["with_dgrad"]))
+        self.frag_ok = False
+        if not self.last_fwd_packed:
+            if counters is not None or pack_args["seed_add"]:
+                self._first_bump = (counters, pack_args["seed_add"])
+            pack_args = None
+        elif not (self.pack_overlap and train):
             self.pack(**pack_args)
             pack_args = None
         if self.marks is not None:
@@ -426,7 +439,12 @@
         if s.idx == 0:
             a0, _ = self.input_acts(s.name)
             w, b = L.ptr(self.params[f"{s.name}.weight"]), L.ptr(self.params[f"{s.name}.bias"])
-            if acc:
+            if self._first_bump is not None:
+                (cnt, seed_add), self._first_bump = self._first_bump, None
+                self._call(self.lib.hpfg_conv3x3_first_fwd_bump, C.byref(a0), w, b, L.ptr(out), None if acc or not want_stats else L.ptr(self.partials),
+                           L.ptr(self.acc_of[s.name]) if acc else None, self.acc_shards[s.name], L.ptr(cnt), cnt.numel() if cnt is not None else 0,
+                           L.ptr(self.seed_dev), int(seed_add), self.N, s.h, s.w, s.cin, s.cout, tag="fwd:" + s.name)
+            elif acc:
                 self._call(self.lib.hpfg_conv3x3_first_fwd_acc, C.byref(a0), w, b, L.ptr(out), None, L.ptr(self.acc_of[s.name]), self.acc_shards[s.name],
                            self.N, s.h, s.w, s.cin, s.cout, tag="fwd:" + s.name)
             else:
diff --git a/hpfg_amd/model/unet.py b/hpfg_amd/model/unet.py
--- a/hpfg_amd/model/unet.py
+++ b/hpfg_amd/model/unet.py
@@ -7,6 +7,7 @@
 import torch.nn as nn
 
 import os
+import weakref
 
 from .. import _lib as L
 from .. import engine as E
@@ -58,11 +59,30 @@
     return m
 
 
+class _WatchedParameter(nn.Parameter):
+
+    @property
+    def data(self):
+        owner = self.__dict__.get("_hpfg_owner")
+        net = owner() if owner is not None else None
+        if net is not None:
+            net.mark_fragments_stale()
+        return torch.Tensor.data.__get__(self)
+
+    @data.setter
+    def data(self, value):
+        torch.Tensor.data.__set__(self, value)
+
+    def __reduce_ex__(self, proto):
+        return nn.Parameter(torch.Tensor.data.__get__(self), self.requires_grad).__reduce_ex__(proto)
+
+
 class _UNetFn(torch.autograd.Function):
 
     @staticmethod
     def forward(ctx, anchor: torch.Tensor, x: torch.Tensor, net: "UNet", want_feat: bool, needs_grad: bool):
         eng = net._acquire_engine(x)
+        net._last_engine = eng
         if getattr(net, "_bn_bump_pending", False):
             eng.bump_counters, net._bn_bump_pending = net._flat_long, False
         logits = eng.forward(x, train=net.training, track_running=True, seed_step=net._next_seed() if net.training else None, needs_grad=needs_grad)
@@ -139,6 +159,10 @@
                 k = p.numel()
                 p.data = flat[off:off + k].view(p.shape)
                 p.grad = None
+                if type(p) is nn.Parameter:
+                    p.__class__ = _WatchedParameter
+                if isinstance(p, _WatchedParameter):
+                    p.__dict__["_hpfg_owner"] = weakref.ref(self)
                 self._offsets[n] = (off, k)
                 off += k
             bs = self._float_buffers()
@@ -153,7 +177,7 @@
             for i, (n, b) in enumerate(ls):
                 b.data = fl[i]
         self._flat, self._flat_grad, self._flat_buf, self._flat_long = flat, flat_grad, fb, fl
-        self._engines = {}
+        self._engines, self._last_engine = {}, None
         self._anchor = torch.zeros(1, device=dev, requires_grad=True)
         self._backbone_numel = sum(p.numel() for n, p in ps if n.startswith("encoder.") or n.startswith("decoder."))
         self._encoder_numel = sum(p.numel() for n, p in ps if n.startswith("encoder."))
@@ -181,7 +205,7 @@
         nn.Module.__init__(new)
         import copy
         for k, v in self.__dict__.items():
-            if k in ("_flat", "_flat_grad", "_flat_buf", "_flat_long", "_engines", "_anchor", "dp"):
+            if k in ("_flat", "_flat_grad", "_flat_buf", "_flat_long", "_engines", "_last_engine", "_anchor", "dp"):
                 continue
             new.__dict__[k] = copy.deepcopy(v, memo)
         new.dp = self.dp
@@ -194,7 +218,16 @@
     def load_state_dict(self, *a, **k):
         out = super().load_state_dict(*a, **k)
         self._ensure_flat()
+        self.mark_fragments_stale()
         return out
+
+    def _weights_token(self) -> tuple:
+        return (self.math, self._flat.data_ptr(), self._flat._version, sum(p._version for p in self.parameters()))
+
+    def mark_fragments_stale(self):
+        for pool in self.__dict__.get("_engines", {}).values():
+            for e in pool:
+                e.frag_token = None
 
     @property
     def flat_params(self) -> torch.Tensor:
@@ -260,6 +293,9 @@
         rank = self.dp.rank if self.dp is not None else 0
         eng.base_seed = (self.dropout_seed + 0x632BE5AB * rank) & 0x7FFFFFFF
         eng.math = L.MATH_BF16X3 if self.math == "bf16x3" else L.MATH_F32
+        if eng.frag_token is not None and eng.frag_token != self._weights_token():
+            eng.frag_token = None
+        eng.frag_ok = eng.frag_token is not None
         eng.defer_wgrad = bool(getattr(self, "defer_wgrad", False))
         eng.pack_overlap = bool(getattr(self, "_alone", False))
         eng.after_layer = getattr(self, "_after_layer", None)
diff --git a/hpfg_amd/train.py b/hpfg_amd/train.py
--- a/hpfg_amd/train.py
+++ b/hpfg_amd/train.py
@@ -269,7 +269,7 @@
     def device_update(self):
         fs, ft = getattr(self.model, "flat_params", None), getattr(self.ema_model, "flat_params", None)
         if isinstance(self.optimizer, FusedSGD) and fs is not None and ft is not None and fs.numel() == ft.numel() and fs.is_cuda:
-            self.optimizer.step(push_lr=False, ema=(ft, fs.numel(), self.sc.view(S_ALPHA)))
+            self.optimizer.step(push_lr=False, ema=(ft, fs.numel(), self.sc.view(S_ALPHA), self.ema_model))
         else:
             self.optimizer.step(push_lr=False)
             update_ema_variables(self.model, self.ema_model, self.args.ema_decay, 0, alpha_dev=self.sc.view(S_ALPHA))
@@ -479,6 +479,8 @@
             model1.skip_necks = True
             if isinstance(self.optimizer1, (FusedSGD, FusedAdamW)):
                 self.optimizer1.active_numel = model1.backbone_numel()
+        if isinstance(self.optimizer2, FusedSGD):
+            self.optimizer2.pack_fragments = False
         self.dense_loss = Dense_Loss(args.batch_size + args.unlabel_batch_size, self.dev)
         self.dense_loss.dp = dp
         self.mask_generator = BoxMaskGenerator(prop_range=(0.25, 0.5), n_boxes=4, random_aspect_ratio=True, prop_by_area=True,
@@ -622,8 +624,13 @@
             raise GraphNotCapturable(f"GraphedStep: {type(step_obj).__name__} has no device_fwd_bwd / exchange / device_update split, so its gradient "
                                "exchange would be captured into the graph; run it eager under data parallel")
         self._freeze_seed_updates(True)
+        engines = [(m, e) for m in self.s.models for pool in getattr(m, "_engines", {}).values() for e in pool]
+        for _, e in engines:
+            e.last_fwd_packed = True
+        self._nopack = []
         try:
             self._capture(dp, mode_split=self.split)
+            self._nopack = [(m, e) for m, e in engines if not e.last_fwd_packed]
         finally:
             self._freeze_seed_updates(False)
             if dp is not None:
@@ -682,6 +689,12 @@
             else:
                 m._fwds_per_replay = getattr(m, "_graph_fwds", 0)
 
+    def _repack_stale(self):
+        for m, e in self._nopack:
+            if e.frag_token is None or e.frag_token != m._weights_token():
+                e.pack(with_dgrad=e.frag_dgrad)
+                e.frag_token = m._weights_token()
+
     def step(self, inputs, cur_itrs, **kw):
         for dst, src in zip(self.static, inputs):
             if dst is not src:
@@ -690,6 +703,7 @@
         self.s.sc.push()
         for m in self.s.models:
             m.bump_graph_seed()
+        self._repack_stale()
         if self.split:
             dp = self.s.dp
             for i, g in enumerate(self.graphs):
diff --git a/hpfg_amd/utils/optim.py b/hpfg_amd/utils/optim.py
--- a/hpfg_amd/utils/optim.py
+++ b/hpfg_amd/utils/optim.py
@@ -1,4 +1,6 @@
 from __future__ import annotations
+
+import ctypes as C
 
 import torch
 
@@ -17,6 +19,8 @@
         self._lr_dev = torch.zeros(1, dtype=torch.float32, device=flat.device)
         self.grad_scale = 1.0
         self.active_numel = None
+        self.pack_fragments = True
+        self._pack_plan = None
 
     def zero_grad(self, set_to_none: bool = False):
         if hasattr(self.model, "_hpfg_generic_flat"):
@@ -29,6 +33,49 @@
     def push_lr(self):
         self._lr_host[0] = float(self.param_groups[0]["lr"])
         self._lr_dev.copy_(self._lr_host, non_blocking=True)
+
+    def _update_pack_plan(self, n_sgd: int, teacher, n_ema: int):
+        from ..engine import DescTable
+        m = self.model
+        eng = getattr(m, "_last_engine", None)
+        if eng is None or getattr(m, "math", None) != "bf16x3" or eng.math != L.MATH_BF16X3 or not {"f", "d"} <= eng.pads_zeroed:
+            return None
+        if not any(eng is e for pool in m._engines.values() for e in pool):
+            return None
+        layers = sorted(eng.packed, key=lambda s: m._offsets[f"{s.name}.weight"][0])
+        end = max(sum(m._offsets[f"{s.name}.bias"]) for s in layers)
+        teng = getattr(teacher, "_last_engine", None) if teacher is not None else None
+        if teng is not None and (teacher.math != "bf16x3" or teng.math != L.MATH_BF16X3 or "f" not in teng.pads_zeroed or end > n_ema
+                                 or teacher._offsets != m._offsets or not any(teng is e for pool in teacher._engines.values() for e in pool)):
+            teng = None
+        key = (eng, teng, m._flat.data_ptr(), n_sgd, n_ema)
+        if self._pack_plan is not None and self._pack_plan[0][0] is eng and self._pack_plan[0][1] is teng and self._pack_plan[0][2:] == key[2:]:
+            return self._pack_plan[1], eng, teng
+        if torch.cuda.is_current_stream_capturing():
+            return None
+        descs =(L.UpdatePackDesc * len(layers))()
+        gaps, at = [], 0
+        for d, s in zip(descs, layers):
+            (wo, wn), (bo, bn) = m._offsets[f"{s.name}.weight"], m._offsets[f"{s.name}.bias"]
+            if not (at <= wo and wo + wn <= bo and bo + bn <= n_sgd):
+                return None
+            d.w_off, d.b_off = wo, bo
+            d.wpk16_fwd, d.wpk16_dgrad, d.bias_pad = L.ptr(eng.wpk16_f[s.name]), L.ptr(eng.wpk16_d[s.name]), L.ptr(eng.bias_pad[s.name])
+            if teng is not None:
+                d.t_wpk16_fwd, d.t_bias_pad = L.ptr(teng.wpk16_f[s.name]), L.ptr(teng.bias_pad[s.name])
+            d.Cout, d.Cin, d.CoutPad, d.CinPad, d.taps = s.cout, s.cin, s.cout_pad, s.cin_pad, s.taps
+            d.kc, d.kc_t = eng.kc[s.name], (teng or eng).kc[s.name]
+            for lo, hi in ((at, wo), (wo + wn, bo)):
+                if hi > lo:
+                    gaps.append((lo, hi))
+            at = bo + bn
+        if at < n_sgd:
+            gaps.append((at, n_sgd))
+        gh = (C.c_long * (2 * max(len(gaps), 1)))(*[v for g_ in gaps for v in g_])
+        gd = torch.tensor([v for g_ in gaps for v in g_] or [0, 0], dtype=torch.int64).to(m._flat.device)
+        plan = (DescTable(descs, m._flat.device), gh, gd, len(gaps))
+        self._pack_plan = (key, plan)
+        return plan, eng, teng
 
     @torch.no_grad()
     def step(self, closure=None, push_lr: bool = True, ema=None):
@@ -42,9 +89,28 @@
             self.push_lr()
         st = torch.cuda.current_stream(flat.device).cuda_stream
         n_sgd = flat.numel() if self.active_numel is None else int(self.active_numel)
+        lib = L.load()
+        teacher = ema[3] if ema is not None and len(ema) > 3 else None
+        for m in (self.model, teacher):
+            if hasattr(m, "mark_fragments_stale"):
+                m.mark_fragments_stale()
         if ema is not None:
-            t, n_ema, alpha_dev = ema
-            assert t.is_cuda and t.dtype == torch.float32 and t.numel() == flat.numel() and 0 <= n_ema <= n_sgd
+            assert ema[0].is_cuda and ema[0].dtype == torch.float32 and ema[0].numel() == flat.numel() and 0 <= ema[1] <= n_sgd
+        found = self._update_pack_plan(n_sgd, teacher, int(ema[1]) if ema is not None else 0) if (
+            self.pack_fragments and lib.hpfg_get_option(L.OPT_UPDATE_PACK) != 0 and hasattr(self.model, "_engines")) else None
+        if found is not None:
+            (table, gaps_host, gaps_dev, ngaps), eng, teng = found
+            dev, host, nl = table.sub(0, len(table.host))
+            t, n_ema, alpha_dev = (ema[0], int(ema[1]), ema[2]) if ema is not None else (None, 0, None)
+            L.check(lib.hpfg_sgd_ema_pack_step(L.ptr(flat), L.ptr(grad), L.ptr(self._mom), n_sgd, L.ptr(self._lr_dev), float(g["momentum"]),
+                                               float(g["weight_decay"]), float(self.grad_scale), L.ptr(t), n_ema, L.ptr(alpha_dev), dev, host, nl,
+                                               L.ptr(gaps_dev), gaps_host, ngaps, st), "sgd_ema_pack_step")
+            eng.frag_token, eng.frag_dgrad = self.model._weights_token(), True
+            if teng is not None:
+                teng.frag_token, teng.frag_dgrad = teacher._weights_token(), False
+            return
+        if ema is not None:
+            t, n_ema, alpha_dev = ema[:3]
             L.check(L.load().hpfg_sgd_ema_step(L.ptr(flat), L.ptr(grad), L.ptr(self._mom), n_sgd, L.ptr(self._lr_dev), float(g["momentum"]),
                                                float(g["weight_decay"]), float(self.grad_scale), L.ptr(t), int(n_ema), L.ptr(alpha_dev), st),
                     "sgd_ema_step")
@@ -137,6 +203,8 @@
         L.check(L.load().hpfg_adamw_step(L.ptr(flat), L.ptr(grad), L.ptr(self._m), L.ptr(self._v), n, L.ptr(self._lr_dev), L.ptr(self._step_dev),
                                          float(g["betas"][0]), float(g["betas"][1]), float(g["eps"]), float(g["weight_decay"]), float(self.grad_scale), st),
                 "adamw_step")
+        if hasattr(self.model, "mark_fragments_stale"):
+            self.model.mark_fragments_stale()
 
     def state_dict(self):
         d = super().state_dict()
diff --git a/hpfg_amd/utils/utils.py b/hpfg_amd/utils/utils.py
--- a/hpfg_amd/utils/utils.py
+++ b/hpfg_amd/utils/utils.py
@@ -101,6 +101,8 @@
     n = src.numel() if numel is None else numel
     a = alpha_dev if alpha_dev is not None else _alpha_dev(src.device, ema_alpha(global_step, alpha))
     L.check(L.load().hpfg_ema_update(L.ptr(dst), L.ptr(src), n, L.ptr(a), torch.cuda.current_stream(src.device).cuda_stream), "ema_update")
+    if hasattr(ema_model, "mark_fragments_stale"):
+        ema_model.mark_fragments_stale()
 
 
 def update_ema_variables_backbone(model, ema_model, alpha, global_step, alpha_dev: torch.Tensor = None):
diff --git a/include/hpfg_hip.h b/include/hpfg_hip.h
--- a/include/hpfg_hip.h
+++ b/include/hpfg_hip.h
@@ -7,7 +7,7 @@
 extern "C" {
 #endif
 
-#define HPFG_VERSION 139
+#define HPFG_VERSION 140
 enum { HPFG_MATH_F32 = 0, HPFG_MATH_BF16X3 = 1 };
 
 enum { HPFG_BN_MEAN = 0, HPFG_BN_RSTD = 1, HPFG_BN_SCALE = 2, HPFG_BN_SHIFT = 3,
@@ -113,7 +113,8 @@
 
 int hpfg_version(void);
 const char* hpfg_last_error(void);
-enum { HPFG_OPT_CONV_THIN = 0, HPFG_OPT_FIRST_MFMA = 1, HPFG_OPT_FIRST_WGRAD = 2, HPFG_OPT_NARROW_DEEP = 3, HPFG_OPT_COUNT = 4 };
+enum { HPFG_OPT_CONV_THIN = 0, HPFG_OPT_FIRST_MFMA = 1, HPFG_OPT_FIRST_WGRAD = 2, HPFG_OPT_NARROW_DEEP = 3, HPFG_OPT_UPDATE_PACK = 4, HPFG_OPT_COUNT = 5 };
+int hpfg_get_option(int which);
 int hpfg_set_option(int which, int value);
 
 int hpfg_conv3x3_first_fwd(const HpfgAct* x, const float* w_oihw, const float* bias, float* out, float* stat_partials,
@@ -156,6 +157,9 @@
 int hpfg_reduce_partials(const float* partials, int nblk, int C, double* sums, void* stream);
 int hpfg_bn_eval_table(const float* gamma, const float* beta, const float* running_mean, const float* running_var, float eps,
                        float* bn, int C, void* stream);
+int hpfg_conv3x3_first_fwd_bump(const HpfgAct* x, const float* w_oihw, const float* bias, float* out, float* stat_partials, long long* stat_acc,
+                                int stat_shards, long long* counters, int n_counters, int32_t* seed_word, int seed_add, int N, int H, int W, int Cin,
+                                int Cout, void* stream);
 int hpfg_conv_kc(int H, int W, int taps);
 long hpfg_wpk16_elems(int Kchannels, int NchannelsPad, int taps, int kc);
 int hpfg_pack_weights(const HpfgPackDesc* table_dev, const HpfgPackDesc* table_host, int nlayers, void* stream);
@@ -329,6 +333,21 @@
 int hpfg_sgd_ema_step(float* p, const float* g, float* mom, long n, const float* lr_dev, float momentum, float weight_decay, float grad_scale,
                       float* t, long n_ema, const float* alpha_dev, void* stream);
 
+typedef struct HpfgUpdatePackDesc {
+  long w_off, b_off;
+  void* wpk16_fwd;
+  void* wpk16_dgrad;
+  float* bias_pad;
+  void* t_wpk16_fwd;
+  float* t_bias_pad;
+  int32_t Cout, Cin, CoutPad, CinPad, taps;
+  int32_t kc, kc_t;
+  int32_t reserved;
+} HpfgUpdatePackDesc;
+int hpfg_sgd_ema_pack_step(float* p, const float* g, float* mom, long n, const float* lr_dev, float momentum, float weight_decay, float grad_scale,
+                           float* t, long n_ema, const float* alpha_dev, const HpfgUpdatePackDesc* table_dev, const HpfgUpdatePackDesc* table_host,
+                           int nlayers, const long* gaps_dev, const long* gaps_host, int ngaps, void* stream);
+
 int hpfg_attn_mfma_fwd(const float* q, const float* kv, float* out, int B, int N, int M, int heads, float scale, void* stream);
 int hpfg_attn_mfma_bwd(const float* q, const float* kv, const float* dout, float* dq, float* dkv, float* scratch, int B, int N, int M, int heads,
                        float scale, void* stream);
```
